# imuncle/TSCM_Calib

Measured on AMD Instinct MI355X. Metric: LM iterations/sec at 4 cams x 10k views (joint intrinsics+extrinsics, fp64), higher is better.
Workload: dtype f64

## Files before the change

include/tscm/tscm.h:

```cpp
#ifndef TSCM_H
#define TSCM_H

#include <stddef.h>

#ifdef __cplusplus
extern "C" {
#endif

#define TSCM_ABI_VERSION 6

enum {
    TSCM_OK = 0,
    TSCM_E_INVALID = -1,
    TSCM_E_NO_DEVICE = -2,
    TSCM_E_HIP = -3,
    TSCM_E_RCCL = -4,
    TSCM_E_UNSUPPORTED = -5,
    TSCM_E_NOMEM = -6,
    TSCM_E_PEER = -7
};

enum { TSCM_CONVERGENCE = 0, TSCM_NO_CONVERGENCE = 1, TSCM_FAILURE = 2 };

#define TSCM_MAX_ITERATIONS 255

typedef struct tscm_problem {
    int n_cameras;
    int n_boards;
    int n_points;
    int n_views;
    const double *board_xy;
    const int *view_camera;
    const int *view_board;
    const int *view_offset;
    const int *view_count;
    const double *obs_u;
    const double *obs_v;
    double *cam_rt;
    double *intr;
    double *board_rt;
    const unsigned char *cam_pose_constant;
    int mono;
    const unsigned char *board_pose_constant;
} tscm_problem;

typedef struct tscm_options {
    size_t struct_size;
    int max_num_iterations;
    double function_tolerance;
    double gradient_tolerance;
    double parameter_tolerance;
    double initial_trust_region_radius;
    double max_trust_region_radius;
    double min_trust_region_radius;
    double min_relative_decrease;
    double min_lm_diagonal;
    double max_lm_diagonal;
    int max_num_consecutive_invalid_steps;
    int jacobi_scaling;
    int check_every;
    int jacobian_fp32;
    int exec_flags;
} tscm_options;

enum {
    TSCM_EXEC_SEPARATE_T_REDUCE = 1,
    TSCM_EXEC_KEEP_SINGLE_RANK_COMM = 2,
    TSCM_EXEC_GRAM_16X16 = 4,
    TSCM_EXEC_SEPARATE_BACKSUB = 8,
    TSCM_EXEC_SEPARATE_CONTROL = 16,
    TSCM_EXEC_DENSE_REDUCED_ORDER = 32,
    TSCM_EXEC_GRAPH_REDUCED_ORDER = 64,
    TSCM_EXEC_SEPARATE_STATS = 128,
    TSCM_EXEC_ALL = 255
};

typedef struct tscm_iteration {
    int iteration;
    int step_is_valid;
    int step_is_successful;
    double cost;
    double cost_change;
    double gradient_max_norm;
    double gradient_norm;
    double step_norm;
    double relative_decrease;
    double trust_region_radius;
} tscm_iteration;

typedef struct tscm_summary {
    int termination_type;
    int num_iterations;
    int num_successful_steps;
    int num_unsuccessful_steps;
    double initial_cost;
    double final_cost;
    int n_residual_blocks;
    int lm_iterations;
    tscm_iteration iterations[TSCM_MAX_ITERATIONS + 1];
    char message[128];
    double seconds_solve;
    double seconds_total;
    double rmse;
} tscm_summary;

typedef struct tscm_solver tscm_solver;
typedef struct tscm_comm tscm_comm;

int tscm_abi_version(void);
const char *tscm_last_error(void);
int tscm_device_count(void);
int tscm_device_synchronize(int device);
int tscm_device_peak_fp64(int device, double *mfma_tflops, double *valu_tflops);
int tscm_device_peak_fp64_ex(int device, double peaks[3]);
int tscm_device_peak_fp32_mfma(int device, double *tflops);

void tscm_default_options(tscm_options *opt, int mono);

int tscm_solver_create(const tscm_problem *problem, int device, tscm_solver **out);
int tscm_solver_set_comm(tscm_solver *s, tscm_comm *comm);
int tscm_solver_debug_withhold_handoff(tscm_solver *s, int on);
int tscm_solver_reruns(const tscm_solver *s);
int tscm_solver_solve(tscm_solver *s, const tscm_options *opt, tscm_summary *summary);
int tscm_solver_upload_params(tscm_solver *s, const double *cam_rt, const double *intr, const double *board_rt);
int tscm_solver_solve_resident(tscm_solver *s, const tscm_options *opt, tscm_summary *summary, int reset);
int tscm_solver_download_params(tscm_solver *s, double *cam_rt, double *intr, double *board_rt);
void tscm_solver_destroy(tscm_solver *s);
int tscm_solver_kernel_time(tscm_solver *s, int enable, int *launches, double *total_ms);
int tscm_solver_exchange_time(tscm_solver *s, int *n_T, double *ms_T, int *n_H, double *ms_H);

int tscm_solve_multi(const tscm_problem *problem, const tscm_options *opt, tscm_summary *summary);
int tscm_solve_mono(const tscm_problem *problem, const tscm_options *opt, tscm_summary *summary);

int tscm_eval_functor(const tscm_problem *problem, int device, double *residuals,
                      double *J_cam, double *J_board, double *J_intr, double *cost);

int tscm_eval_normal_equations(const tscm_problem *problem, int device, double *board_gram,
                               double *board_grad, double *view_cross, double *cam_gram,
                               double *cam_grad, double *cost);

int tscm_eval_normal_equations_ex(const tscm_problem *problem, int device, const tscm_options *opt,
                                  double *board_gram, double *board_grad, double *view_cross,
                                  double *cam_gram, double *cam_grad, double *cost);

int tscm_eval_step_ex(const tscm_problem *problem, int device, const tscm_options *opt,
                      double *cam_rt, double *intr, double *board_rt, int *valid,
                      tscm_summary *summary);

enum { TSCM_LOSS_NONE = 0, TSCM_LOSS_HUBER = 1, TSCM_LOSS_SOFT_L1 = 2, TSCM_LOSS_CAUCHY = 3 };
int tscm_solver_set_loss(tscm_solver *s, int kind, double scale);
int tscm_solve_robust(const tscm_problem *problem, const tscm_options *opt, int kind, double scale, tscm_summary *summary);
int tscm_eval_normal_equations_robust(const tscm_problem *problem, int device, const tscm_options *opt, int kind, double scale,
                                      double *board_gram, double *board_grad, double *view_cross,
                                      double *cam_gram, double *cam_grad, double *cost);
int tscm_eval_step_robust(const tscm_problem *problem, int device, const tscm_options *opt, int kind, double scale,
                          double *cam_rt, double *intr, double *board_rt, int *valid, tscm_summary *summary);

enum {
    TSCM_FIX_FX = 1, TSCM_FIX_FY = 2, TSCM_FIX_CX = 4, TSCM_FIX_CY = 8, TSCM_FIX_XI = 16, TSCM_FIX_LAMBDA = 32,
    TSCM_FIX_ALPHA = 64, TSCM_FIX_B = 128, TSCM_FIX_C = 256,
    TSCM_FIX_INTRINSICS = 127, TSCM_FIX_ALL = 511,
    TSCM_MODEL_DS = TSCM_FIX_LAMBDA, TSCM_MODEL_UCM = TSCM_FIX_XI | TSCM_FIX_LAMBDA
};
int tscm_solver_set_fixed_intrinsics(tscm_solver *s, const unsigned short *fixed);
int tscm_solve_fixed(const tscm_problem *problem, const tscm_options *opt, const unsigned short *fixed, int kind, double scale,
                     tscm_summary *summary);
int tscm_eval_step_fixed(const tscm_problem *problem, int device, const tscm_options *opt, const unsigned short *fixed, int kind,
                         double scale, double *cam_rt, double *intr, double *board_rt, int *valid, tscm_summary *summary);

int tscm_solve_mono_batch(const tscm_problem *problems, int n_problems, int device, const tscm_options *opt,
                          const unsigned short *fixed , int loss_kind, double loss_scale,
                          tscm_summary *summaries );

int tscm_project_points(const double *intr9, const double *points, int n, int device, double *pixels);
int tscm_unproject_pixels(const double *intr9, const double *pixels, int n, int device, double *rays);
int tscm_reprojection_error(const tscm_problem *problem, int device, double *per_camera_mean,
                            double *global_mean, double *rmse);

#define TSCM_UNIQUE_ID_BYTES 128
int tscm_solver_create_sharded(const tscm_problem *problem, int device, int rank, int world, tscm_solver **out);
int tscm_comm_unique_id(unsigned char id[TSCM_UNIQUE_ID_BYTES]);
int tscm_comm_create(const unsigned char id[TSCM_UNIQUE_ID_BYTES], int rank, int world, int device, tscm_comm **out);
int tscm_comm_create_local(int world, int device, tscm_comm **out );
#define TSCM_IPC_HANDLE_BYTES 80
int tscm_comm_ipc_open(int rank, int world, int device, size_t max_doubles, tscm_comm **out, unsigned char handle[TSCM_IPC_HANDLE_BYTES]);
int tscm_comm_ipc_connect(tscm_comm *c, const unsigned char *handles );
void tscm_comm_destroy(tscm_comm *c);
int tscm_comm_info(const tscm_comm *c, int *rank, int *world, int *backend_ranks);
int tscm_solver_solve_group(tscm_solver **solvers, int n, const tscm_options *opt, tscm_summary *summaries, int reset);
int tscm_solver_gather_boards(tscm_solver *s, double *board_rt);
int tscm_shard_frames(const tscm_problem *problem, int world, int *owner);


typedef struct tscm_rig_input {
    int n_cameras, n_boards, n_points;
    const double *worlds;
    const double *intr;
    const unsigned char *has;
    const double *Rt;
    const double *pix_u, *pix_v;
} tscm_rig_input;

typedef struct tscm_rig_result {
    double *cam_R, *cam_t, *cam_rt;
    double *board_R, *board_t, *board_rt;
    unsigned char *board_initial;
    int *cam_choice;
    double *cam_min_error;
    double seconds_hypotheses;
    double seconds_total;
    long long n_projections;
} tscm_rig_result;

int tscm_rig_init(const tscm_rig_input *in, int device, tscm_rig_result *out);
int tscm_rig_stage_errors(const tscm_rig_input *in, int i, const double *Rp, const double *tp, int ksplit, int device,
                          double *Rs_out, double *ts_out, double *err_out, int *info_out);


int tscm_yaml_format(int n_cameras, const double *intr, const double *cam_R, const double *cam_t,
                     char *buf, size_t buf_size, size_t *needed);
int tscm_yaml_write(const char *path, int n_cameras, const double *intr, const double *cam_R,
                    const double *cam_t);
int tscm_yaml_parse(const char *text, int max_cameras, int *n_cameras, double *intr, double *Twc);
int tscm_yaml_read(const char *path, int max_cameras, int *n_cameras, double *intr, double *Twc);


typedef struct tscm_map_desc {
    double intr[9];
    double R[9];
    double fx, fy, cx, cy;
    double offset_x, offset_y;
    int width, height;
    int out_stride;
    int check_w2;
    long long out_offset;
    double w2;
} tscm_map_desc;

int tscm_build_maps(const tscm_map_desc *maps, int n_maps, int device, int exact, float *mapx,
                    float *mapy, size_t n_elems, double *seconds_kernel);

enum { TSCM_PROJ_PERSPECTIVE = 0, TSCM_PROJ_LONGLAT = 1, TSCM_PROJ_CYLINDRICAL = 2,
       TSCM_PROJ_STEREOGRAPHIC = 3, TSCM_PROJ_EQUIRECT = 4 };

int tscm_build_maps_ex(const tscm_map_desc *maps, const int *projection ,
                       int n_maps, int device, int exact, float *mapx, float *mapy, size_t n_elems,
                       double *seconds_kernel);

int tscm_build_sweep_maps(const tscm_map_desc *maps , const int *projection , int n_cameras,
                          const double *centers , const double *inv_distance , int D,
                          int device_index, int exact, float *mapx, float *mapy ,
                          size_t n_elems, double *seconds_kernel);

int tscm_rectify_points(const tscm_map_desc *map, int projection, const double *pixels ,
                        int n, int device, double *out , unsigned char *valid );


int tscm_estimate_focal(const double *pix_u, const double *pix_v, const int *count, int n_views,
                        int board_w, int board_h, double cx, double cy, int device, double *focal,
                        int *n_used);
int tscm_poses_from_r1r2t(const double *Rt, const unsigned char *has, int n, double *rt);
int tscm_estimate_extrinsic(const double *intr9, const double *pix_u, const double *pix_v, const int *count,
                            int n_views, const double *worlds, int n_points, int board_w, int device,
                            double *Rt, int *n_estimated);
#define TSCM_EXTRINSIC_NO_BOARD 1
#define TSCM_EXTRINSIC_DEGENERATE_BOARD 2
#define TSCM_EXTRINSIC_DLT_FAILED 3
#define TSCM_EXTRINSIC_ZERO_COLUMN 4
#define TSCM_EXTRINSIC_CONVERGED 5
#define TSCM_EXTRINSIC_ITERATION_CAP 6
#define TSCM_EXTRINSIC_GN_CHOLESKY 7
int tscm_estimate_focal_rows(const double *pix_u, const double *pix_v, const int *count, int n_views,
                             int board_w, int board_h, double cx, double cy, int device, double *gamma);
int tscm_estimate_extrinsic_stages(const double *intr9, const double *pix_u, const double *pix_v,
                                   const int *count, int n_views, const double *worlds, int n_points,
                                   int board_w, int device, double *Rt, int *n_estimated, double *T,
                                   double *H, double *pose0, double *pose, int *steps, int *exit_code);


typedef struct tscm_corner_set {
    int n_cameras, n_boards, board_cols, board_rows;
    double pitch;
    int image_width, image_height;
    unsigned char *has;
    double *pix_u, *pix_v;
} tscm_corner_set;

int tscm_corners_write(const char *path, const tscm_corner_set *set);
int tscm_corners_read(const char *path, tscm_corner_set *set);
void tscm_corners_free(tscm_corner_set *set);

int tscm_remap(const unsigned char *src, int width, int height, int stride, int channels, const float *mapx, const float *mapy, int map_width,
               int map_height, int map_stride, int to_gray, int device, unsigned char *dst, int dst_stride);

typedef struct tscm_corner_candidates {
    int n;
    int n_maxima;
    double *x, *y;
    double *v1, *v2;
    double *score;
    double *sub;
    double seconds;
} tscm_corner_candidates;

int tscm_detect_corners(const unsigned char *gray, int width, int height, int stride, int sigma, double min_score, int device,
                        tscm_corner_candidates *out);
int tscm_detect_corners_batch(const unsigned char *const *images, int n_images, int width, int height, int stride, int sigma, double min_score,
                              int device, tscm_corner_candidates *out);
void tscm_corner_candidates_free(tscm_corner_candidates *c);
// ... 222 lines not shown
```

tscm_calib_amd/api.py:

```python
from __future__ import annotations

import ctypes as C

import numpy as np

from . import lib as _l
from .problem import Problem


class Solver:

    def __init__(self, problem: Problem, device: int = 0, rank: int = 0, world: int = 1):
        self.problem = problem.normalised() if not _is_normalised(problem) else problem
        self.problem.validate()
        self._cp = _l.c_problem(self.problem)
        self._h = C.c_void_p()
        self.rank, self.world = rank, world
        _l.check(_l.lib().tscm_solver_create_sharded(C.byref(self._cp), device, rank, world, C.byref(self._h)))
        self._comm = None

    def close(self):
        if getattr(self, "_h", None) is not None and self._h.value:
            _l.lib().tscm_solver_destroy(self._h)
            self._h = C.c_void_p()
# ... 114 lines not shown
        _l.check(_l.lib().tscm_comm_unique_id(buf))
        return bytes(buf)

    def close(self):
        if getattr(self, "_h", None) is not None and self._h.value:
            _l.lib().tscm_comm_destroy(self._h)
            self._h = C.c_void_p()

    __del__ = close


class Group:

    def __init__(self, problem: Problem, world: int, device: int = 0, *, loss=None, fixed=None):
        self.problem = problem.normalised() if not _is_normalised(problem) else problem
        self.world = world
        self.comms = Comm.local_group(world, device)
        self.solvers = [Solver(self.problem, device, r, world) for r in range(world)]
        for s, c in zip(self.solvers, self.comms):
            s.set_comm(c)
        if loss is not None:
            k, a = _l.loss_args(loss)
            for s in self.solvers:
                _l.check(_l.lib().tscm_solver_set_loss(s._h, k, a))
        if fixed is not None:
            for s in self.solvers:
                s.set_fixed_intrinsics(fixed)

    def solve(self, **options) -> "list[dict]":
        for s in self.solvers:
            s.upload_params()
        out = self.solve_resident(reset=True, **options)
        p = self.problem
        cam, intr, _ = self.solvers[0].download_params()
        if not p.mono:
            p.cam_rt[:] = cam
        p.intr[:] = intr
        for s in self.solvers:
            _l.check(_l.lib().tscm_solver_download_params(s._h, None, None, _l.dptr(p.board_rt)))
        return out

    def solve_resident(self, reset: bool = True, **options) -> "list[dict]":
        o = _l.default_options(self.problem.mono, **options)
        hs = (C.c_void_p * self.world)(*[s._h for s in self.solvers])
        sums = (_l.CSummary * self.world)()
        _l.check(_l.lib().tscm_solver_solve_group(hs, self.world, C.byref(o), sums, 1 if reset else 0))
        return [_l.summary_dict(sums[r]) for r in range(self.world)]

    def close(self):
        for s in self.solvers:
            s.close()
        for c in self.comms:
            c.close()
        self.solvers, self.comms = [], []

    def __enter__(self):
        return self

    def __exit__(self, *a):
        self.close()


def _is_normalised(p: Problem) -> bool:
    ok = lambda a, dt: isinstance(a, np.ndarray) and a.dtype == dt and a.flags["C_CONTIGUOUS"]
    return (all(ok(getattr(p, n), np.float64) for n in ("board_xy", "obs_u", "obs_v", "cam_rt", "intr", "board_rt"))
            and all(ok(getattr(p, n), np.int32) for n in ("view_camera", "view_board", "view_offset", "view_count"))
            and ok(p.cam_pose_constant, np.uint8)
            and (p.board_pose_constant is None or ok(p.board_pose_constant, np.uint8)))


def calibrate(problem: Problem, device: int = 0, *, loss=None, fixed=None, **options) -> dict:
    if problem.mono:
        raise ValueError("calibrate() is the multi-camera solve; use refinement() for a mono problem")
    assert _is_normalised(problem), "use Problem.normalised()"
    o = _l.default_options(False, **options)
    s = _l.CSummary()
    cp = _l.c_problem(problem)
    _select(device)
    _solve_one_shot(cp, o, s, loss, fixed, problem.n_cameras, _l.lib().tscm_solve_multi)
    return _l.summary_dict(s)


def refinement(problem: Problem, device: int = 0, *, loss=None, fixed=None, **options):
    if not problem.mono:
        raise ValueError("refinement() is the mono solve")
    assert _is_normalised(problem), "use Problem.normalised()"
    o = _l.default_options(True, **options)
    s = _l.CSummary()
    cp = _l.c_problem(problem)
    _select(device)
    _solve_one_shot(cp, o, s, loss, fixed, problem.n_cameras, _l.lib().tscm_solve_mono)
    d = _l.summary_dict(s)
    return d["termination_type"] == 0, d


def refinement_batch(problems, device: int = 0, *, loss=None, fixed=None, **options):
    problems = list(problems)
    if not problems:
        raise ValueError("refinement_batch() needs at least one problem")
    for p in problems:
        if not p.mono:
            raise ValueError("refinement_batch() takes mono problems only")
        assert _is_normalised(p), "use Problem.normalised()"
    n = len(problems)
    o = _l.default_options(True, **options)
    cps = (_l.CProblem * n)(*[_l.c_problem(p) for p in problems])
    sums = (_l.CSummary * n)()
    if fixed is None:
        w = None
    else:
        if len(fixed) != n:
            raise ValueError("fixed: one mask per problem")
        w = np.array([_l.fixed_masks(f, 1)[0] for f in fixed], dtype=np.uint16)
    k, a = _l.loss_args(loss)
    _l.check(_l.lib().tscm_solve_mono_batch(cps, n, device, C.byref(o), _l.ushort_ptr(w) if w is not None else None, k, a, sums))
    out = []
    for i in range(n):
        d = _l.summary_dict(sums[i])
        out.append((d["termination_type"] == 0, d))
    return out


def _solve_one_shot(cp, o, s, loss, fixed, n_cameras, plain):
    if fixed is not None:
        w = _l.fixed_masks(fixed, n_cameras)
        k, a = _l.loss_args(loss)
        _l.check(_l.lib().tscm_solve_fixed(C.byref(cp), C.byref(o), _l.ushort_ptr(w), k, a, C.byref(s)))
    elif loss is None:
        _l.check(plain(C.byref(cp), C.byref(o), C.byref(s)))
    else:
        k, a = _l.loss_args(loss)
        _l.check(_l.lib().tscm_solve_robust(C.byref(cp), C.byref(o), k, a, C.byref(s)))


def _select(device: int):
    if device != 0:
        raise ValueError("one-shot calibrate()/refinement() use the current device; use Solver(problem, device)")


def evaluate_functor(problem: Problem, device: int = 0, jacobians: bool = True):
    assert _is_normalised(problem)
    N = problem.n_corners
    res = np.zeros((N, 2))
    cost = C.c_double(0.0)
    cp = _l.c_problem(problem)
    if jacobians:
        Jc, Jb, Ji = np.zeros((N, 2, 6)), np.zeros((N, 2, 6)), np.zeros((N, 2, 9))
        _l.check(_l.lib().tscm_eval_functor(C.byref(cp), device, _l.dptr(res), _l.dptr(Jc), _l.dptr(Jb), _l.dptr(Ji), C.byref(cost)))
        return cost.value, res, Jc, Jb, Ji
    _l.check(_l.lib().tscm_eval_functor(C.byref(cp), device, _l.dptr(res), None, None, None, C.byref(cost)))
    return cost.value, res


def normal_equations(problem: Problem, device: int = 0, *, jacobian_fp32: int = 0, exec_flags: int = 0, loss=None) -> dict:
    assert _is_normalised(problem)
    Cn, B, V = problem.n_cameras, problem.n_boards, problem.n_views
    out = dict(board_gram=np.zeros((B, 6, 6)), board_grad=np.zeros((B, 6)), view_cross=np.zeros((V, 6, 15)),
               cam_gram=np.zeros((Cn, 15, 15)), cam_grad=np.zeros((Cn, 15)))
    cost = C.c_double(0.0)
    cp = _l.c_problem(problem)
    o = _l.default_options(problem.mono, jacobian_fp32=jacobian_fp32, exec_flags=exec_flags)
    outs = (_l.dptr(out["board_gram"]), _l.dptr(out["board_grad"]), _l.dptr(out["view_cross"]),
            _l.dptr(out["cam_gram"]), _l.dptr(out["cam_grad"]), C.byref(cost))
    if loss is None:
        _l.check(_l.lib().tscm_eval_normal_equations_ex(C.byref(cp), device, C.byref(o), *outs))
    else:
        k, a = _l.loss_args(loss)
        _l.check(_l.lib().tscm_eval_normal_equations_robust(C.byref(cp), device, C.byref(o), k, a, *outs))
    out["cost"] = cost.value
    return out


def step(problem: Problem, device: int = 0, *, loss=None, fixed=None, **options) -> dict:
    assert _is_normalised(problem)
    cam, intr, board = np.zeros_like(problem.cam_rt), np.zeros_like(problem.intr), np.zeros_like(problem.board_rt)
    valid = C.c_int(0)
    s = _l.CSummary()
    cp = _l.c_problem(problem)
    o = _l.default_options(problem.mono, **options)
    outs = (_l.dptr(cam), _l.dptr(intr), _l.dptr(board), C.byref(valid), C.byref(s))
    if fixed is not None:
        w = _l.fixed_masks(fixed, problem.n_cameras)
        k, a = _l.loss_args(loss)
        _l.check(_l.lib().tscm_eval_step_fixed(C.byref(cp), device, C.byref(o), _l.ushort_ptr(w), k, a, *outs))
    elif loss is None:
        _l.check(_l.lib().tscm_eval_step_ex(C.byref(cp), device, C.byref(o), *outs))
    else:
        k, a = _l.loss_args(loss)
        _l.check(_l.lib().tscm_eval_step_robust(C.byref(cp), device, C.byref(o), k, a, *outs))
    return dict(cam_rt=cam, intr=intr, board_rt=board, valid=bool(valid.value), summary=_l.summary_dict(s))


def project(intr, points, device: int = 0) -> np.ndarray:
    intr = np.ascontiguousarray(intr, dtype=np.float64).reshape(9)
    pts = np.ascontiguousarray(points, dtype=np.float64).reshape(-1, 3)
    out = np.zeros((pts.shape[0], 2))
    _l.check(_l.lib().tscm_project_points(_l.dptr(intr), _l.dptr(pts), pts.shape[0], device, _l.dptr(out)))
    return out


def unproject(intr, pixels, device: int = 0) -> np.ndarray:
    intr = np.ascontiguousarray(intr, dtype=np.float64).reshape(9)
    px = np.ascontiguousarray(pixels, dtype=np.float64).reshape(-1, 2)
    out = np.zeros((px.shape[0], 3))
    _l.check(_l.lib().tscm_unproject_pixels(_l.dptr(intr), _l.dptr(px), px.shape[0], device, _l.dptr(out)))
    return out


def reprojection_error(problem: Problem, device: int = 0):
    assert _is_normalised(problem)
    per = np.zeros(problem.n_cameras)
    g, r = C.c_double(0.0), C.c_double(0.0)
    cp = _l.c_problem(problem)
    _l.check(_l.lib().tscm_reprojection_error(C.byref(cp), device, _l.dptr(per), C.byref(g), C.byref(r)))
    return per, g.value, r.value


def shard_owner(problem: Problem, world: int) -> np.ndarray:
    assert _is_normalised(problem)
    owner = np.zeros(problem.n_boards, dtype=np.int32)
    cp = _l.c_problem(problem)
    _l.check(_l.lib().tscm_shard_frames(C.byref(cp), world, owner.ctypes.data_as(C.POINTER(C.c_int))))
    return owner
```

tscm_calib_amd/csrc/tscm_dev.h:

```cpp
#pragma once

static_assert(kColFree == kFA && kColGrad == kFR, "tscm_columns.h plans the columns of tscm_math.h's camera tile");
constexpr int kWcolTc = 3;
constexpr int kFac = 56;
constexpr int kFacM = 0;
constexpr int kFacC = 15;
constexpr int kFacL = 21;
constexpr int kFacI = 36;
constexpr int kFacZ = 42;
constexpr int kFacD = 48;
constexpr int kTcols = 15;
constexpr int kTcWb = 0, kTcWc = 4, kTcF = 8, kTcOne = 9, kTcXi = 10, kTcLam = 12, kTcAl = 13, kTcR = 14;
__host__ __device__ constexpr int tc_tc(int j) { return 3 + 4 * j; }
constexpr int kVConst = 27;
constexpr int kCConst = 48;
constexpr int kCStride = 72;
constexpr int kCst = 80;
constexpr int kScal = 8;
constexpr int kStStride = 16;

constexpr int kVStride = 48;
constexpr int kVFloatOff = 32;

__device__ __forceinline__ void wave_lds_fence()
{
    __builtin_amdgcn_fence(__ATOMIC_RELEASE, "wavefront");
    __builtin_amdgcn_wave_barrier();
    __builtin_amdgcn_fence(__ATOMIC_ACQUIRE, "wavefront");
}

typedef int v2i __attribute__((ext_vector_type(2)));
__device__ __forceinline__ __amdgpu_buffer_rsrc_t make_rsrc(const void *p, size_t bytes)
{
    return __builtin_amdgcn_make_buffer_rsrc(const_cast<void *>(p), 0, (int)(bytes > 0xffffffffull ? 0xffffffffu : (unsigned)bytes), 0x00020000);
}
__device__ __forceinline__ double buf_load_f64(__amdgpu_buffer_rsrc_t r, unsigned voff, unsigned soff)
{
    return __builtin_bit_cast(double, __builtin_amdgcn_raw_buffer_load_b64(r, (int)voff, (int)soff, 0));
}
__device__ __forceinline__ void buf_store_f64(__amdgpu_buffer_rsrc_t r, unsigned voff, unsigned soff, double v)
{
    __builtin_amdgcn_raw_buffer_store_b64(__builtin_bit_cast(v2i, v), r, (int)voff, (int)soff, 0);
}

typedef double d4 __attribute__((ext_vector_type(4)));
typedef double d2 __attribute__((ext_vector_type(2)));
typedef int v4i __attribute__((ext_vector_type(4)));
__device__ __forceinline__ d2 buf_load_2f64(__amdgpu_buffer_rsrc_t r, unsigned voff, unsigned soff)
{
    return __builtin_bit_cast(d2, __builtin_amdgcn_raw_buffer_load_b128(r, (int)voff, (int)soff, 0));
}
__device__ __forceinline__ void buf_store_2f64(__amdgpu_buffer_rsrc_t r, unsigned voff, double a, double b)
{
    const d2 v = { a, b };
    __builtin_amdgcn_raw_buffer_store_b128(__builtin_bit_cast(v4i, v), r, (int)voff, 0, 0);
}

__device__ __forceinline__ void set_prio(int p)
{
    switch (p & 3) {
    case 0: __builtin_amdgcn_s_setprio(0); break;
    case 1: __builtin_amdgcn_s_setprio(1); break;
    case 2: __builtin_amdgcn_s_setprio(2); break;
    default: __builtin_amdgcn_s_setprio(3); break;
    }
}

__device__ __forceinline__ const double *rec_w(const double *rec, int slot) { return rec + (size_t)kRecW * slot; }
__device__ __forceinline__ const double *rec_e(const double *rec, int V, int slot) { return rec + (size_t)kRecW * V + (size_t)kRecE * slot; }
__device__ __forceinline__ const double *rec_g(const double *rec, int V, int slot) { return rec + (size_t)(kRecW + kRecE) * V + (size_t)kRecG * slot; }

struct Ctrl : CtrlHead {
    IterLog log[kMaxLog];
};

struct DevProblem {
    int C, B, n_points, V, N, n_pad;
    int n_chunks, n_pchunks, n_bids;
    int rp, half;
    int lds_wave;
    const double *board_xy;
    const int *view_cam, *view_board, *view_obs, *view_count;
    const double *obs_u, *obs_v;
    const int *chunk_vb, *chunk_ve, *chunk_cam, *cam_chunk_ptr;
    const int4 *chunk_desc;
    const int *bv_ptr;
    const int *view_slot, *slot_cam;
    const int *slot_view, *slot_board;
    const int *slow_boards;
    int n_slow;
    const int *pair_i, *pair_j;
    const int *pc_begin, *pc_end, *pc_tile;
    const int *bid_part_ptr;
    const int *pair_board;
    const int *bc_tile;
    const int4 *bc_desc;
    int n_bchunks, n_tiles;
    const unsigned char *col_ctl;
    const unsigned char *board_const;
    const unsigned char *col_active;
    const int *act_map;
    int n_act;
    int cam_pre[9];
    unsigned short cam_free[8];
    unsigned long long pair_mask;
    const int4 *solve_map;
    int cam_wg[9];
    int rank, world;
    const short *bid_lut;
    int bid_part_small[kSmallBids + 1];
    int g4_per;
};

struct DevState {
    double *cam_rt[2], *intr[2], *board_rt[2];
    double *board_pc, *cam_pc;
    double *vconst;
    double *cconst[2];
    double *rec[2];
    double *campart, *campart2;
    double *H[2], *H_stage;
    double *s_b, *s_c;
    double *fac;
    double *pairpart, *T;
    int *t_count;
    int *fac_fail;
    int *y_flag;
    double *yhat;
    double *Abig;
    double *bs_part, *st_part;
    int n_bs_blocks, n_st_blocks;
    Ctrl *ctrl;
    CtrlHead *ctrl_snap;
    int *stats_count, *stats_flag;
    struct CtlPub *ctl_pub;
};
struct CtlPub { int epoch, cur, done, pad; double radius; };

template <int CTRL>
__device__ __forceinline__ double dpp_f64(double v)
{
    const int lo = __builtin_amdgcn_update_dpp(0, __double2loint(v), CTRL, 0xF, 0xF, true);
    const int hi = __builtin_amdgcn_update_dpp(0, __double2hiint(v), CTRL, 0xF, 0xF, true);
    return __hiloint2double(hi, lo);
}
__device__ __forceinline__ double row16_allsum(double v)
{
    v += dpp_f64<0xB1>(v); v += dpp_f64<0x4E>(v); v += dpp_f64<0x141>(v); v += dpp_f64<0x140>(v);
    return v;
}
__device__ __forceinline__ double row16_allmax(double v)
{
    v = fmax(v, dpp_f64<0xB1>(v)); v = fmax(v, dpp_f64<0x4E>(v)); v = fmax(v, dpp_f64<0x141>(v)); v = fmax(v, dpp_f64<0x140>(v));
    return v;
}

#if defined(__HIP_DEVICE_COMPILE__) && !defined(__gfx950__) && !defined(__gfx942__)
#error "the in-launch hand-offs (handoff_store / handoff_load) rely on gfx942 / gfx950 sc1 write-through semantics: re-derive them for this target"
#endif
constexpr long long kHandoffTimeoutTicks = 50 * 1000 * 1000;
__device__ __forceinline__ void handoff_store(double *p, double v) { __hip_atomic_store(p, v, __ATOMIC_RELAXED, __HIP_MEMORY_SCOPE_AGENT); }
__device__ __forceinline__ double handoff_load(const double *p) { return __hip_atomic_load(p, __ATOMIC_RELAXED, __HIP_MEMORY_SCOPE_AGENT); }
```

tscm_calib_amd/csrc/tscm_eval_f32.h:

```cpp
#pragma once

template <int KS> struct F32Tile {
    static constexpr int KB = KS + (KS & 1);
    static constexpr int P2 = 4 * KB + 2;
    static constexpr int kDoubles = 16 * P2 > 512 ? 16 * P2 : 512;
    static_assert(4 * KB <= P2 && (2 * P2) % 8 == 4 && (KB * 8) % 16 == 0, "block starts are 16-byte aligned, columns 4 * odd dwords apart");
};

typedef float f2 __attribute__((ext_vector_type(2)));
typedef float f4 __attribute__((ext_vector_type(4)));

__host__ __device__ inline int eval_f32_lds_doubles(int n_points, int ks)
{
    const int kb = ks + (ks & 1), tile = 16 * (4 * kb + 2);
    return 4 * (tile > 512 ? tile : 512) + 2 * n_points;
}

template <int KS, bool MULTI, bool ROBUST = false>
__global__ __launch_bounds__(256, 4) void k_eval_gram_f32(DevProblem P, DevState S, int cand, LossArg L)
{
    static_assert(KS >= 1 && KS <= kG4MaxKS, "a pass holds at most 56 rows");
    const int ctrl_done = S.ctrl->done, ctrl_cur = S.ctrl->cur;
    extern __shared__ __attribute__((aligned(16))) double lds_all[];
    const int wave = __builtin_amdgcn_readfirstlane(threadIdx.x >> 6);
    constexpr int kP2 = F32Tile<KS>::P2, KB = F32Tile<KS>::KB, kTile32 = F32Tile<KS>::kDoubles;
    constexpr int lds_wave = kTile32;
    double *lds = lds_all + (size_t)wave * lds_wave;
    f2 *T2 = reinterpret_cast<f2 *>(lds);
    double *bxy = lds_all + 4 * kTile32;
    const int lane = threadIdx.x & 63;
    const int chunk = blockIdx.x * 4 + wave;
    const v4i cd = *(const v4i __attribute__((address_space(4))) *)(const void *)(P.chunk_desc + chunk);
    const int cam = cd[0], vb = cd[1], ve = cd[2];
    const int n2 = 2 * P.n_points;
    const double bx0 = P.board_xy[min(lane, n2 - 1)], bx1 = P.board_xy[min(lane + 64, n2 - 1)];
    typedef const float __attribute__((address_space(4))) *fptr4;
    double *const cc_buf[2] = { S.cconst[0], S.cconst[1] };
    double *const rec_buf[2] = { S.rec[0], S.rec[1] };
    const int col = lane & 15, kq = lane >> 4;
    d4 camU = { 0.0, 0.0, 0.0, 0.0 }, camV = { 0.0, 0.0, 0.0, 0.0 };
    double rr = 0.0;
    for (int i = lane; i < kTile32; i += 64) lds[i] = 0.0;
    int prev_nv = 0;
    double pf_u = 0.0, pf_v = 0.0;
    int warm = 0;
    constexpr int K = KS;
    const int per = MULTI ? P.g4_per : 4 * KS;
    f2 *fw = T2 + (KB == KS ? lane : KB * (lane / K) + lane % K);
    typedef const f4 __attribute__((address_space(3))) *lds_f4;
    const lds_f4 pB = (lds_f4)(T2 + col * kP2 + KB * kq);
    const lds_f4 pA = (lds_f4)(T2 + ((col >> 2) + 4 * (col & 3)) * kP2 + KB * kq);
    if (ctrl_done) return;
    const int tgt = cand ? (ctrl_cur ^ 1) : ctrl_cur;
    const __amdgpu_buffer_rsrc_t r_rec = make_rsrc(tgt ? rec_buf[1] : rec_buf[0], sizeof(double) * (size_t)kRec * P.V);
    const cptr4 cc = (cptr4)((tgt ? cc_buf[1] : cc_buf[0]) + kCStride * cam);
    const fptr4 cf = (fptr4)((tgt ? cc_buf[1] : cc_buf[0]) + kCStride * cam + kCConst);
    const RecLane rl = rec_lane(lane, (unsigned)P.V);
    const __amdgpu_buffer_rsrc_t r_vc = make_rsrc(S.vconst, sizeof(double) * (size_t)kVStride * P.V);
    const __amdgpu_buffer_rsrc_t r_u = make_rsrc(P.obs_u, sizeof(double) * (size_t)P.N), r_v = make_rsrc(P.obs_v, sizeof(double) * (size_t)P.N);
    int off_next = cd[3];
    int m_cnt0 = 0, m_slot0 = 0;
    if (vb + lane < min(ve, vb + 64)) { m_cnt0 = P.view_count[vb + lane]; m_slot0 = P.view_slot[vb + lane]; }
    if (vb < ve) { pf_u = buf_load_f64(r_u, 8u * lane, 8u * (unsigned)off_next); pf_v = buf_load_f64(r_v, 8u * lane, 8u * (unsigned)off_next); }
    {
        typedef const int __attribute__((address_space(4))) *cptr4i;
        const cptr4i v0 = (cptr4i)(S.vconst + (size_t)kVStride * min(vb, P.V - 1)), c0 = (cptr4i)cc;
        const int k0 = v0[0], k1 = v0[16], k2 = v0[32], k3 = v0[48], k4 = v0[64], k5 = v0[80], k6 = c0[16], k7 = c0[48], k8 = c0[80], k9 = c0[112], k10 = c0[128];
        asm volatile("" :: "s"(k0), "s"(k1), "s"(k2), "s"(k3), "s"(k4), "s"(k5), "s"(k6), "s"(k7), "s"(k8), "s"(k9), "s"(k10));
    }
    if (lane < n2) bxy[lane] = bx0;
    if (lane + 64 < n2) bxy[lane + 64] = bx1;
    for (int i = lane + 128; i < n2; i += 64) bxy[i] = P.board_xy[i];
    for (int vbase = vb; vbase < ve; vbase += 64) {
    const int vend = min(ve, vbase + 64);
    int m_cnt = 0, m_slot = 0;
    if (vbase == vb) { m_cnt = m_cnt0; m_slot = m_slot0; }
    else {
        if (vbase + lane < vend) { m_cnt = P.view_count[vbase + lane]; m_slot = P.view_slot[vbase + lane]; }
        pf_u = buf_load_f64(r_u, 8u * lane, 8u * (unsigned)off_next); pf_v = buf_load_f64(r_v, 8u * lane, 8u * (unsigned)off_next);
    }
    asm volatile("" : "+v"(m_cnt), "+v"(m_slot));
    for (int view = vbase; view < vend; ++view) {
        const int cnt = __builtin_amdgcn_readlane(m_cnt, view - vbase);
        const int off = off_next;
        off_next = off + cnt;
        wave_lds_fence();
        set_prio(3 - min(3, 8 * (view - vb) / max(1, ve - vb) % 4));
        const cptr4 cst = (cptr4)(S.vconst + (size_t)kVStride * view);
        const fptr4 cs = (fptr4)(S.vconst + (size_t)kVStride * view + kVFloatOff);
        d4 accU = { 0.0, 0.0, 0.0, 0.0 }, accV = { 0.0, 0.0, 0.0, 0.0 };
        for (int c0 = 0; c0 < cnt; c0 += per) {
            const int j = c0 + lane;
            const bool valid = lane < (MULTI ? min(per, cnt - c0) : cnt);
            float wf = 1.f;
            auto PUT = [&](int c, float u, float v) {
                if constexpr (ROBUST) { u *= wf; v *= wf; }
                fw[c * kP2] = f2{ u, v };
            };
            if (valid) {
                const double x = bxy[2 * j], y = bxy[2 * j + 1];
                const double ou = pf_u, ov = pf_v;
                const double X = fma(x, cst[0], fma(y, cst[3], cst[6]));
                const double Y = fma(x, cst[1], fma(y, cst[4], cst[7]));
                const double Z = fma(x, cst[2], fma(y, cst[5], cst[8]));
                const double rho2 = X * X + Y * Y;
                const double s1 = rho2 + Z * Z;
                const double id1 = fast_rsqrt(s1), d1 = s1 * id1;
                const double z1 = Z + cc[43] * d1;
                const double s2 = rho2 + z1 * z1;
                const double id2 = fast_rsqrt(s2), d2 = s2 * id2;
                const double z2 = z1 + cc[44] * d2;
                const double s3 = rho2 + z2 * z2;
                const double id3 = fast_rsqrt(s3), d3 = s3 * id3;
                const double ik = fast_rcp(z2 + cc[45] * d3);
                const double mx = X * ik, my = Y * ik;
                const double ru = ou - (cc[39] * mx + cc[41]);
                const double rv = ov - (cc[40] * my + cc[42]);
                double w = 1.0;
                if constexpr (ROBUST) {
                    double rho;
                    robust_rho(L, ru * ru + rv * rv, rho, w);
                    rr += rho;
                    wf = (float)w;
                } else {
                    rr += ru * ru + rv * rv;
                }
                const float xf = (float)x, yf = (float)y;
                const float Xf = (float)X, Yf = (float)Y, Zf = (float)Z, z1f = (float)z1, z2f = (float)z2;
                const float i1 = (float)id1, i2 = (float)id2, i3 = (float)id3, ikf = (float)ik;
                const float e1 = (float)d1, e2 = (float)d2, e3 = (float)d3;
                const float mxf = (float)mx, myf = (float)my;
                float Q0 = (float)(X - cc[9]), Q1 = (float)(Y - cc[10]), Q2 = (float)(Z - cc[11]);
                if (cc[24] != 0.0) {
                    const float w0 = cf[21], w1 = cf[22], w2 = cf[23];
                    const float s0 = w1 * Q2 - w2 * Q1, s1 = w2 * Q0 - w0 * Q2, s2 = w0 * Q1 - w1 * Q0;
                    Q0 -= s0; Q1 -= s1; Q2 -= s2;
                }
                const float xi = cf[43], lam = cf[44], beta = cf[45];
                const float c1 = 1.f + xi * Zf * i1;
                const float c2 = 1.f + lam * z1f * i2;
                const float c3 = 1.f + beta * z2f * i3;
                const float q = beta * i3 + c3 * (lam * i2 + c2 * xi * i1);
                const float kz = c1 * c2 * c3;
                const f2 fk = { cf[39] * ikf, cf[40] * ikf };
                const f2 HM = { fk.x * mxf, fk.y * myf };
                const f2 N0 = HM * (Xf * q) - (f2){ fk.x, 0.f };
                const f2 N1 = HM * (Yf * q) - (f2){ 0.f, fk.y };
                const f2 N2 = HM * kz;
                PUT(tc_tc(0), N0.x, N0.y);
                PUT(tc_tc(1), N1.x, N1.y);
                PUT(tc_tc(2), N2.x, N2.y);
#pragma unroll
                for (int kk = 0; kk < 3; ++kk) {
                    const float h0 = xf * cs[9 + 6 * kk] + yf * cs[12 + 6 * kk];
                    const float h1 = xf * cs[10 + 6 * kk] + yf * cs[13 + 6 * kk];
                    const float h2 = xf * cs[11 + 6 * kk] + yf * cs[14 + 6 * kk];
                    const f2 w = N0 * h0 + N1 * h1 + N2 * h2;
                    PUT((kTcWb + kk), w.x, w.y);
                }
                {
                    const f2 c0 = N2 * Q1 - N1 * Q2, c1 = N0 * Q2 - N2 * Q0, c2 = N1 * Q0 - N0 * Q1;
#pragma unroll
                    for (int kk = 0; kk < 3; ++kk) {
                        const f2 w = c0 * cf[12 + 3 * kk] + c1 * cf[13 + 3 * kk] + c2 * cf[14 + 3 * kk];
                        PUT((kTcWc + kk), w.x, w.y);
                    }
                }
                PUT(kTcF, -mxf, -myf);
                PUT(kTcOne, -1.f, -1.f);
                const float kxi = c3 * c2 * e1, klam = c3 * e2, kal = e3 * cf[46];
                const f2 a = HM * kxi, b = HM * klam, c = HM * kal;
                PUT(kTcXi, a.x, a.y);
                PUT(kTcLam, b.x, b.y);
                PUT(kTcAl, c.x, c.y);
                if constexpr (ROBUST) fw[kTcR * kP2] = f2{ (float)(w * ru), (float)(w * rv) };
                else PUT(kTcR, (float)ru, (float)rv);
            } else if (lane < prev_nv) {
#pragma unroll
                for (int c = 0; c < kTcols; ++c) PUT(c, 0.f, 0.f);
            }
            {
                const int vn = min(view + 1, vend - 1);
                const int cn = view + 1 < vend ? __builtin_amdgcn_readlane(m_cnt, vn - vbase) : 0;
                if (!MULTI || c0 == 0) warm = __builtin_amdgcn_raw_buffer_load_b32(r_vc, lane < 6 ? 64 * lane : (int)0xffffe000u, (int)(8u * (unsigned)kVStride * (unsigned)vn), 0);
                const bool more = MULTI && c0 + per < cnt;
                const int ncnt = MULTI ? (more ? min(per, cnt - c0 - per) : min(per, cn)) : cn;
// ... 57 lines not shown
```

tscm_calib_amd/csrc/tscm_eval_gram4.h:

```cpp
#pragma once

constexpr int kG4Stride = 68;
__host__ __device__ constexpr int g4_tile_doubles(int ks) { return ks * kG4Stride > 512 ? ks * kG4Stride : 512; }
__host__ __device__ inline int eval_gram4_lds_doubles(int n_points, int ks) { return g4_tile_doubles(ks) + 2 * n_points; }

constexpr int kG4Wb = 0, kG4R = 3, kG4Tc = 4, kG4Al = 7, kG4Wc = 8, kG4F = 11, kG4One = 12, kG4Xi = 13, kG4Lam = 14;
__device__ __forceinline__ constexpr int g4_old_col(int c)
{
    return c < 3 ? kTcWb + c : c == 3 ? kTcR : c < 7 ? tc_tc(c - 4) : c == 7 ? kTcAl : c < 11 ? kTcWc + (c - 8) : c == 11 ? kTcF
         : c == 12 ? kTcOne : c == 13 ? kTcXi : c == 14 ? kTcLam : 15;
}
__device__ __forceinline__ constexpr int g4_wcol(int c)
{
    return c < 3 ? -1 : c == 3 ? kFR : c < 7 ? kWcolTc + (c - 4) : c == 7 ? 12 : c < 11 ? c - 8 : c == 11 ? 6 : c == 12 ? 8 : c == 13 ? 10 : c == 14 ? 11 : -1;
}
__device__ __forceinline__ constexpr int g4_cgroup(int b, int q) { return q == 0 ? b : q == 1 ? ((b + 1) & 3) : (b == 0 ? 2 : b == 1 ? 3 : 1); }
__device__ __forceinline__ int g4_elem(int c, int k) { return 4 * c + (k ^ ((c >> 3) << 1)); }

template <int KS, int D, bool ACC, int T = 0>
__device__ __forceinline__ void gram4_steps(unsigned aN, unsigned aR, unsigned aB, double (&n)[KS], double (&r)[KS], double (&b)[KS], double (&acc)[3])
{
    if constexpr (T < KS) {
        if constexpr (T + D < KS) {
            n[T + D] = ds_read_f64<8 * kG4Stride * (T + D)>(aN);
            r[T + D] = ds_read_f64<8 * kG4Stride * (T + D)>(aR);
            b[T + D] = ds_read_f64<8 * kG4Stride * (T + D)>(aB);
        }
        constexpr int newer = 3 * (KS - 1 - T < D ? KS - 1 - T : D);
        lgkm_wait<newer + 2>(n[T]);
        if constexpr (T == 0 && !ACC) acc[0] = __builtin_amdgcn_mfma_f64_4x4x4f64(n[T], n[T], 0.0, 0, 0, 0);
        else acc[0] = __builtin_amdgcn_mfma_f64_4x4x4f64(n[T], n[T], acc[0], 0, 0, 0);
        lgkm_wait<newer + 1>(r[T]);
        if constexpr (T == 0 && !ACC) acc[1] = __builtin_amdgcn_mfma_f64_4x4x4f64(n[T], r[T], 0.0, 0, 0, 0);
        else acc[1] = __builtin_amdgcn_mfma_f64_4x4x4f64(n[T], r[T], acc[1], 0, 0, 0);
        lgkm_wait<newer>(b[T]);
        if constexpr (T == 0 && !ACC) acc[2] = __builtin_amdgcn_mfma_f64_4x4x4f64(n[T], b[T], 0.0, 0, 0, 0);
        else acc[2] = __builtin_amdgcn_mfma_f64_4x4x4f64(n[T], b[T], acc[2], 0, 0, 0);
        gram4_steps<KS, D, ACC, T + 1>(aN, aR, aB, n, r, b, acc);
    }
}
template <int KS, int D, int T = 0>
__device__ __forceinline__ void gram4_prime(unsigned aN, unsigned aR, unsigned aB, double (&n)[KS], double (&r)[KS], double (&b)[KS])
{
    if constexpr (T < D && T < KS) {
        n[T] = ds_read_f64<8 * kG4Stride * T>(aN);
        r[T] = ds_read_f64<8 * kG4Stride * T>(aR);
        b[T] = ds_read_f64<8 * kG4Stride * T>(aB);
        gram4_prime<KS, D, T + 1>(aN, aR, aB, n, r, b);
    }
}
template <int KS, bool ACC>
__device__ __forceinline__ void gram4_full(unsigned aN, unsigned aR, unsigned aB, double (&acc)[3])
{
    constexpr int D = KS < 2 ? KS : 2;
    double n[KS], r[KS], b[KS];
    gram4_prime<KS, D>(aN, aR, aB, n, r, b);
    gram4_steps<KS, D, ACC>(aN, aR, aB, n, r, b, acc);
}

__device__ __forceinline__ double quad_tb(double x, double c0, double c1, double c2)
{
    const double x0 = dpp_f64<0x00>(x), x1 = dpp_f64<0x55>(x), x2 = dpp_f64<0xAA>(x);
    return fma(c2, x2, fma(c0, x0, c1 * x1));
}

template <int ROW, int BANK>
__device__ __forceinline__ double lane_pick(double keep, double take)
{
    const int lo = __builtin_amdgcn_update_dpp(__double2loint(keep), __double2loint(take), 0xE4, ROW, BANK, false);
    const int hi = __builtin_amdgcn_update_dpp(__double2hiint(keep), __double2hiint(take), 0xE4, ROW, BANK, false);
    return __hiloint2double(hi, lo);
}

template <int KS, bool MULTI, bool ROBUST = false>
__global__ __launch_bounds__(256, 4) void k_eval_gram4(DevProblem P, DevState S, int cand, LossArg L)
{
    static_assert(KS >= 1 && KS <= kG4MaxKS, "a pass holds at most 56 rows");
    constexpr int kTile = g4_tile_doubles(KS);
    KTL(0);
    const int ctrl_done = S.ctrl->done, ctrl_cur = S.ctrl->cur;
#ifdef TSCM_WAVE_TIMELINE
    const long long tl_t0 = wall_clock64();
    const int tl_iter = S.ctrl->iteration;
    long long tl_ph[5] = { 0, 0, 0, 0, 0 };
    long long tl_w[4] = { 0, 0, 0, 0 };
    int tl_nv = 0;
#define TL_STAMP(var) const long long var = (long long)__builtin_readcyclecounter()
#define TL_ADD(k, a, b) tl_ph[k] += (b) - (a)
#else
#define TL_STAMP(var)
#define TL_ADD(k, a, b)
#endif
    extern __shared__ __attribute__((aligned(16))) double lds_all[];
    const int wave = __builtin_amdgcn_readfirstlane(threadIdx.x >> 6);
    const int lds_wave = eval_gram4_lds_doubles(P.n_points, KS);
    double *lds = lds_all + (size_t)wave * lds_wave;
    double *Fl = lds;
    double *bxy = lds + kTile;
    const int lane = threadIdx.x & 63;
    const int chunk = blockIdx.x * 4 + wave;
    const v4i cd = *(const v4i __attribute__((address_space(4))) *)(const void *)(P.chunk_desc + chunk);
    const int cam = cd[0], vb = cd[1], ve = cd[2];
    const d2 my_xy = *reinterpret_cast<const d2 *>(P.board_xy + 2 * min(lane, P.n_points - 1));
    double *const cc_buf[2] = { S.cconst[0], S.cconst[1] };
    double *const rec_buf[2] = { S.rec[0], S.rec[1] };
    double camU[3] = { 0.0, 0.0, 0.0 }, camV[3] = { 0.0, 0.0, 0.0 };
    for (int i = lane; i < KS * kG4Stride; i += 64) Fl[i] = 0.0;
    int prev_nv = 0;
    double pf_u = 0.0, pf_v = 0.0;
    int warm = 0;
    double rho_sum = 0.0;
    if (ctrl_done) return;
    const int tgt = cand ? (ctrl_cur ^ 1) : ctrl_cur;
    const __amdgpu_buffer_rsrc_t r_rec = make_rsrc(tgt ? rec_buf[1] : rec_buf[0], sizeof(double) * (size_t)kRec * P.V);
    const cptr4 ccs = (cptr4)((tgt ? cc_buf[1] : cc_buf[0]) + kCStride * cam);
    auto CC = [&](int k) { return ccs[k]; };
    const __amdgpu_buffer_rsrc_t r_vc = make_rsrc(S.vconst, sizeof(double) * (size_t)kVStride * P.V);
    const __amdgpu_buffer_rsrc_t r_u = make_rsrc(P.obs_u, sizeof(double) * (size_t)P.N), r_v = make_rsrc(P.obs_v, sizeof(double) * (size_t)P.N);
    int off_next = cd[3];
    int m_cnt0 = 0, m_slot0 = 0;
    if (vb + lane < min(ve, vb + 64)) { m_cnt0 = P.view_count[vb + lane]; m_slot0 = P.view_slot[vb + lane]; }
    if (vb < ve) { pf_u = buf_load_f64(r_u, 8u * ((unsigned)off_next + lane), 0); pf_v = buf_load_f64(r_v, 8u * ((unsigned)off_next + lane), 0); }
    typedef const int __attribute__((address_space(4))) *cptr4i;
    const cptr4i vc0 = (cptr4i)(S.vconst + (size_t)kVStride * min(vb, P.V - 1)), cc0 = (cptr4i)ccs;
    const int kw0 = vc0[0], kw1 = vc0[16], kw2 = vc0[32], kw3 = vc0[48], kw4 = cc0[16], kw5 = cc0[32], kw6 = cc0[48], kw7 = cc0[64], kw8 = cc0[80];
    double *fu_lo = Fl + (lane >> 2) * kG4Stride + (lane & 3), *fu_hi = Fl + (lane >> 2) * kG4Stride + ((lane & 3) ^ 2);
    const int li = lane >> 4, c16 = lane & 15, lb = c16 >> 2, lj = c16 & 3;
    const unsigned lds0 = lds_addr(Fl);
    const unsigned aN = lds0 + 8u * (unsigned)g4_elem(c16, li);
    const unsigned aR = lds0 + 8u * (unsigned)g4_elem((c16 + 4) & 15, li);
    const unsigned aB = lds0 + 8u * (unsigned)g4_elem(4 * g4_cgroup(lb, 2) + lj, li);
    const double rc0 = lj == 0 ? ccs[0] : lj == 1 ? ccs[1] : ccs[2];
    const double rc1 = lj == 0 ? ccs[3] : lj == 1 ? ccs[4] : ccs[5];
    const double rc2 = lj == 0 ? ccs[6] : lj == 1 ? ccs[7] : ccs[8];
    constexpr unsigned BAD = 0xffffe000u;
    unsigned o1e = BAD, o1w = BAD, o2 = BAD, o3e = BAD, o4 = BAD, o5 = BAD, o6 = BAD, o7a = BAD, o7b = BAD;
    {
        const int b = lb, j = lj, i = li;
        auto W = [](int wcol, int row) { return 8u * (unsigned)(6 * wcol + row); };
        const int f1 = g4_wcol(4 + i), f1j = g4_wcol(4 + j), f2 = g4_wcol(8 + i), f2j = g4_wcol(8 + j), f3 = g4_wcol(12 + i);
        if (b == 0 && j < 3 && i < 3) { o1e = 8u * (unsigned)(6 * j + i); o3e = 8u * (unsigned)(6 * i + 3 + j); }
        if (b == 0 && j == 3 && i < 3) { o1w = W(kFR, i); o7a = 8u * (unsigned)i; }
        if (b == 1 && j < 3) o1w = W(f1, 3 + j);
        if (b == 0 && i < 3) o2 = W(f1j, i);
        if (b == 0 && i == 3 && j < 3) { o2 = W(kFR, 3 + j); o7b = 8u * (unsigned)(3 + j); }
        if (b == 3 && j < 3 && i < 3) o2 = W(f3, j);
        if (b == 0 && i < 3) o4 = W(f2j, i);
        if (b == 2 && j < 3) o4 = W(f2, 3 + j);
        if (b == 3 && j < 3 && i < 3) o4 = W(f3, 3 + j);
        if (b == 3 && i == 0 && j < 3) { o5 = W(9, j); o6 = W(9, 3 + j); }
        if (b == 0 && j == 3 && i < 3) o6 = W(7, i);
        if (b == 2 && i == 3 && j < 3) o6 = W(7, 3 + j);
    }
    if (lane < P.n_points) *reinterpret_cast<d2 *>(bxy + 2 * lane) = my_xy;
    if constexpr (MULTI) {
        for (int j = lane + 64; j < P.n_points; j += 64) *reinterpret_cast<d2 *>(bxy + 2 * j) = *reinterpret_cast<const d2 *>(P.board_xy + 2 * j);
    }
    const int per = MULTI ? P.g4_per : 4 * KS;
    asm volatile("" :: "s"(kw0), "s"(kw1), "s"(kw2), "s"(kw3), "s"(kw4), "s"(kw5), "s"(kw6), "s"(kw7), "s"(kw8));
#ifdef TSCM_WAVE_TIMELINE
    tl_w[0] = wall_clock64();
    const bool tl_on = lane == 0 && tl_iter == 5 && cand && chunk < kTimelineWaves;
#endif
    const int prio_n = max(1, ve - vb);
    int prio_q = 0, prio_rem = 0;
    for (int vbase = vb; vbase < ve; vbase += 64) {
    const int vend = min(ve, vbase + 64);
    int m_cnt = 0, m_slot = 0;
    if (vbase == vb) { m_cnt = m_cnt0; m_slot = m_slot0; }
    else {
        if (vbase + lane < vend) { m_cnt = P.view_count[vbase + lane]; m_slot = P.view_slot[vbase + lane]; }
        pf_u = buf_load_f64(r_u, 8u * ((unsigned)off_next + lane), 0); pf_v = buf_load_f64(r_v, 8u * ((unsigned)off_next + lane), 0);
    }
    asm volatile("" : "+v"(m_cnt), "+v"(m_slot));
    for (int view = vbase; view < vend; ++view) {
        const int cnt = __builtin_amdgcn_readlane(m_cnt, view - vbase);
        const int off = off_next;
        off_next += cnt;
        wave_lds_fence();
        const int left = ve - 1 - view;
        const bool tail_steps = left <= 2 && ve - vb <= 16;
        set_prio(tail_steps ? left + 1 : 3 - (prio_q & 3));
        for (prio_rem += 8; prio_rem >= prio_n; prio_rem -= prio_n) { ++prio_q; asm volatile("" : "+s"(prio_q)); }
#ifdef TSCM_WAVE_TIMELINE
        if (tl_on && tl_nv < kTlViews) g_tlv[(size_t)(4 + kTlViews) * chunk + 4 + tl_nv] = wall_clock64();
        ++tl_nv;
#endif
        const cptr4 vcs = (cptr4)(S.vconst + (size_t)kVStride * view);
        auto VC = [&](int k) { return vcs[k]; };
        double accU[3] = { 0.0, 0.0, 0.0 }, accV[3] = { 0.0, 0.0, 0.0 };
        int pbv = 0;
        do {
        const int pb = MULTI ? pbv : 0;
        TL_STAMP(ts0);
        if constexpr (MULTI) { if (pb) wave_lds_fence(); }
        const int nv = MULTI ? min(per, cnt - pb) : cnt;
        const bool valid = lane < nv;
        double fv[16];
        auto PUT = [&](int c, double u, double v) { (c < 8 ? fu_lo : fu_hi)[4 * c] = u; fv[c] = v; };
        if (valid) {
            const double x = bxy[2 * (pb + lane)], y = bxy[2 * (pb + lane) + 1];
            constexpr int tcol[15] = { kG4Wb, kG4Wb + 1, kG4Wb + 2, kG4Tc, kG4Tc + 1, kG4Tc + 2, kG4Wc, kG4Wc + 1, kG4Wc + 2,
                                       kG4F, kG4One, kG4Xi, kG4Lam, kG4Al, kG4R };
            if constexpr (ROBUST) {
                double ru, rv, rho, w;
                corner_residual(x, y, pf_u, pf_v, VC, CC, ru, rv);
                robust_rho(L, ru * ru + rv * rv, rho, w);
                rho_sum += rho;
                corner_geometry(x, y, pf_u, pf_v, VC, CC, [&](int gc, double u, double v) { PUT(tcol[gc], w * u, w * v); });
            } else {
                corner_geometry(x, y, pf_u, pf_v, VC, CC, [&](int gc, double u, double v) { PUT(tcol[gc], u, v); });
            }
        }
        if (nv < prev_nv) {
            if (!valid && lane < prev_nv) {
#pragma unroll
                for (int c = 0; c < kTcols; ++c) (c < 8 ? fu_lo : fu_hi)[4 * c] = 0.0;
            }
        }
        {
            const int vn = min(view + 1, vend - 1);
            if (!MULTI || pb == 0) warm = __builtin_amdgcn_raw_buffer_load_b32(r_vc, lane < 4 ? 64 * lane : (int)0xffffe000u, (int)(8u * (unsigned)kVStride * (unsigned)vn), 0);
            const bool more = MULTI && pb + per < cnt;
            const unsigned noff = more ? (unsigned)(off + pb + per) : (unsigned)off_next;
            pf_u = buf_load_f64(r_u, 8u * (noff + lane), 0);
            pf_v = buf_load_f64(r_v, 8u * (noff + lane), 0);
        }
        prev_nv = MULTI ? min(per, max(cnt - pb, 0)) : cnt;
        wave_lds_fence();
        if (tail_steps && left == 0) set_prio(0);
        TL_STAMP(ts1);
#ifdef TSCM_WAVE_TIMELINE
        if (tl_nv == 1) tl_w[1] = wall_clock64();
#endif
        gram4_full<KS, MULTI>(aN, aR, aB, accU);
        wave_lds_fence();
        TL_STAMP(ts2);
        if (valid) {
#pragma unroll
            for (int c = 0; c < kTcols; ++c) (c < 8 ? fu_lo : fu_hi)[4 * c] = fv[c];
        }
        wave_lds_fence();
        TL_STAMP(ts3);
        gram4_full<KS, MULTI>(aN, aR, aB, accV);
        TL_STAMP(ts4);
        TL_ADD(0, ts0, ts1); TL_ADD(1, ts1, ts2); TL_ADD(2, ts2, ts3); TL_ADD(3, ts3, ts4);
        pbv += per;
        } while (MULTI && pbv < cnt);
        TL_STAMP(ts4e);
        asm volatile("" :: "v"(warm));
#pragma unroll
        for (int q = 0; q < 3; ++q) { camU[q] += accU[q]; camV[q] += accV[q]; }
        {
            const unsigned slot = (unsigned)__builtin_amdgcn_readlane(m_slot, view - vbase);
            const unsigned offW = 8u * (unsigned)kRecW * slot, offE = 8u * ((unsigned)kRecW * (unsigned)P.V + (unsigned)kRecE * slot);
            const double T0 = accU[0] + accV[0], T1 = accU[1] + accV[1], T2 = accU[2] + accV[2];
            const double X = lane_pick<0xF, 0x1>(lane_pick<0xF, 0x2>(T2, T0), T1);
            const double tbX = quad_tb(X, rc0, rc1, rc2), tbU2 = quad_tb(accU[2], rc0, rc1, rc2);
            const unsigned offG = 8u * ((unsigned)(kRecW + kRecE) * (unsigned)P.V + (unsigned)kRecG * slot);
            buf_store_f64(r_rec, o1e, offE, T0);
            buf_store_f64(r_rec, o7a, offG, T0);
            buf_store_f64(r_rec, o1w, offW, lane_pick<0xF, 0x2>(T0, tbX));
            buf_store_f64(r_rec, o5, offW, T1 - accU[1]);
            buf_store_f64(r_rec, o2, offW, lane_pick<0x1, 0x8>(lane_pick<0x8, 0xF>(T1, tbX), accU[1]));
            buf_store_f64(r_rec, o3e, offE, tbX);
            buf_store_f64(r_rec, o7b, offG, tbX);
            const double a4 = lane_pick<0xF, 0xE>(T2, tbX), u4 = lane_pick<0xF, 0x1>(tbU2, accU[2]);
            buf_store_f64(r_rec, o4, offW, (int)o6 >= 0 ? u4 : a4);
            buf_store_f64(r_rec, o6, offW, a4 - u4);
        }
#ifdef TSCM_WAVE_TIMELINE
        { TL_STAMP(ts5); TL_ADD(4, ts4e, ts5); }
        if (view + 1 == ve) tl_w[3] = wall_clock64();
#endif
    }
    }
#ifdef TSCM_WAVE_TIMELINE
    if (lane == 0 && tl_iter == 5 && cand && chunk < kTimelineWaves) {
        g_timeline[4 * chunk] = (long long)__builtin_amdgcn_s_getreg(63492);
        g_timeline[4 * chunk + 1] = (long long)__builtin_amdgcn_s_getreg(6164);
        g_timeline[4 * chunk + 2] = tl_t0;
        g_timeline[4 * chunk + 3] = wall_clock64();
        for (int k = 0; k < 5; ++k) g_phase[5 * chunk + k] = tl_ph[k];
        for (int k = 0; k < 4; ++k) g_tlv[(size_t)(4 + kTlViews) * chunk + k] = tl_w[k];
    }
#endif
    if constexpr (ROBUST) {
#pragma unroll
        for (int o = 32; o > 0; o >>= 1) rho_sum += __shfl_xor(rho_sum, o);
        if (lane == 16 * kG4R + kG4R) { camU[0] = rho_sum; camV[0] = 0.0; }
    }
    wave_lds_fence();
#pragma unroll
    for (int q = 0; q < 3; ++q) {
        const int r = g4_old_col(4 * lb + li), c = g4_old_col(4 * g4_cgroup(lb, q) + lj);
        lds[16 * r + c] = camU[q]; lds[16 * c + r] = camU[q];
        lds[256 + 16 * r + c] = camV[q]; lds[256 + 16 * c + r] = camV[q];
    }
    __syncthreads();
    {
        const int t = threadIdx.x;
        const size_t st = lds_wave;
        double *part = S.campart + (size_t)512 * blockIdx.x;
        part[t] = (lds_all[t] + lds_all[st + t]) + (lds_all[2 * st + t] + lds_all[3 * st + t]);
        part[256 + t] = (lds_all[256 + t] + lds_all[st + 256 + t]) + (lds_all[2 * st + 256 + t] + lds_all[3 * st + 256 + t]);
    }
#ifdef TSCM_WAVE_TIMELINE
    if (lane == 0 && tl_iter == 5 && cand && chunk < kTimelineWaves) g_tlv[(size_t)(4 + kTlViews) * chunk + 2] = wall_clock64();
#endif
}
```

tscm_calib_amd/csrc/tscm_exec_plan.h:

```cpp
#ifndef TSCM_EXEC_PLAN_H
#define TSCM_EXEC_PLAN_H

#include "tscm_layout.h"

#include <algorithm>
#include <string>

#ifdef __HIPCC__
#define TSCM_PLAN_FN __host__ __device__ inline
#else
#define TSCM_PLAN_FN inline
#endif

namespace tscm {

constexpr int kCamSl = 16;
constexpr int kTSlices = 16;
constexpr int kTEntries = 64;
constexpr int kFusedEntries = 256 / kTSlices;
constexpr int kVPrepThreads = 128;
constexpr int kDense4Cams = 4;

constexpr int kCtlOneGpu = 1;
constexpr int kCtlComm = 2;
constexpr int kCtlInit = 4;
constexpr int kCtlRide = 8;
constexpr int kCtlWithhold = 16;

enum CommKind { kCommNone, kCommOneRank, kCommShared };
inline bool uses_comm(int kind, int exec_flags) { return kind == kCommShared || (kind == kCommOneRank && (exec_flags & TSCM_EXEC_KEEP_SINGLE_RANK_COMM)); }

enum class Gram { G4, F32, G16, G16Pitch58 };
enum class EvalTail {
    ReduceControl,
    StatsThenHead,
    Ride,
    Exchange,
};
enum class Solver { Empty, Dense4, Nd, Big };

struct ExecDevice {
    int schur_resident[4] = {}, schur_resident_ride[4] = {};
    int dense4_resident = 0;
    int nd_resident[2] = {}, nd_tpt[2] = { 1, 1 };
};

struct ExecPlan {
    bool comm = false;
    Gram gram = Gram::G4;
    bool robust = false;
    EvalTail tail = EvalTail::ReduceControl;
    bool ctl_in_schur = false;
    bool stats_ride = false;
    bool t_in_solve = false;
    Solver solver = Solver::Empty;
    int nd = 0, tpt = 1;
    int n_prod = 0, n_bs = 0;
    int bs_threads = 0;
    bool f32() const { return gram == Gram::F32; }
};

inline int reduction_blocks(const Layout &L, int C) { return C * kCamSl + (L.B + 255) / 256; }

inline Gram plan_gram(int exec_flags, int jacobian_fp32, int rp)
{
    if (jacobian_fp32) return Gram::F32;
    if (!(exec_flags & TSCM_EXEC_GRAM_16X16)) return Gram::G4;
    return rp == 58 ? Gram::G16Pitch58 : Gram::G16;
}

constexpr int kG4MaxKS = 14;
struct G4Plan { int passes, per, ks; };
TSCM_PLAN_FN G4Plan g4_plan(int n_points)
{
    G4Plan g;
    g.passes = (n_points + 4 * kG4MaxKS - 1) / (4 * kG4MaxKS);
    if (g.passes < 1) g.passes = 1;
    g.ks = ((n_points + g.passes - 1) / g.passes + 3) / 4;
    if (g.ks < 1) g.ks = 1;
    g.per = 4 * g.ks;
    return g;
}

inline ExecPlan plan_exec(const Layout &L, int C, int n_act, int comm_kind, int exec_flags, int jacobian_fp32, int loss_kind, int rp,
                          const ExecDevice &dev)
{
    ExecPlan p;
    p.comm = uses_comm(comm_kind, exec_flags);
    p.gram = plan_gram(exec_flags, jacobian_fp32, rp);
    p.robust = loss_kind != TSCM_LOSS_NONE;
    const int n_variants = (L.nv_chunks[1] ? 1 : 0) + (L.nv_chunks[2] ? 1 : 0) + (L.nv_chunks[3] ? 1 : 0);
    const bool small = C <= kMaxCamLds;
    p.ctl_in_schur = (p.comm || small) && L.slow_boards.empty() && L.pc_begin.empty() && n_variants == 1 &&
                     !(exec_flags & TSCM_EXEC_SEPARATE_CONTROL);
    const int nv = L.nv_chunks[1] ? 1 : L.nv_chunks[2] ? 2 : 3;
    p.stats_ride = p.ctl_in_schur && !p.comm && small && !(exec_flags & TSCM_EXEC_SEPARATE_STATS) &&
                   std::max(reduction_blocks(L, C), L.nv_chunks[nv]) + 1 <= dev.schur_resident_ride[nv];
    p.tail = p.comm || !small ? EvalTail::Exchange : !p.ctl_in_schur ? EvalTail::ReduceControl : p.stats_ride ? EvalTail::Ride : EvalTail::StatsThenHead;
    p.t_in_solve = !(exec_flags & TSCM_EXEC_SEPARATE_T_REDUCE) && small && !p.comm && L.n_bids > 0 && L.n_bids <= kSmallBids && n_act > 0;
    p.n_prod = p.t_in_solve ? L.n_bids * (256 / kFusedEntries) : 0;
    p.nd = (exec_flags & TSCM_EXEC_DENSE_REDUCED_ORDER) ? 1 : 0;
    const bool graph_order = (exec_flags & TSCM_EXEC_GRAPH_REDUCED_ORDER) || p.nd;
    p.solver = n_act == 0 ? Solver::Empty : C <= kDense4Cams && !graph_order ? Solver::Dense4 : small ? Solver::Nd : Solver::Big;
    if (p.solver != Solver::Nd) p.nd = 0;
    p.tpt = p.solver == Solver::Nd ? dev.nd_tpt[p.nd] : 1;
    if (p.solver == Solver::Dense4 || p.solver == Solver::Nd) {
        const int resident = p.solver == Solver::Dense4 ? dev.dense4_resident : dev.nd_resident[p.nd];
        if (!(exec_flags & TSCM_EXEC_SEPARATE_BACKSUB) && L.bs_threads == 256 && L.n_bs_blocks <= resident - 1 - p.n_prod) p.n_bs = L.n_bs_blocks;
    }
    p.bs_threads = !p.n_bs && L.n_bs_blocks ? L.bs_threads : 0;
    return p;
}

inline int check_exec_options(const tscm_options &o, int loss_kind, std::string &err)
{
    if (o.max_num_iterations < 0 || o.max_num_iterations > TSCM_MAX_ITERATIONS) return layout_fail(err, TSCM_E_INVALID, "max_num_iterations must be in [0, 255]");
    if (o.exec_flags & ~TSCM_EXEC_ALL) return layout_fail(err, TSCM_E_INVALID, "unknown bits in tscm_options.exec_flags (an options struct of an older ABI?)");
    if (loss_kind != TSCM_LOSS_NONE && (o.exec_flags & TSCM_EXEC_GRAM_16X16)) return layout_fail(err, TSCM_E_UNSUPPORTED, "TSCM_EXEC_GRAM_16X16 has no robust-loss kernel");
    return 0;
}

}

#endif
```

tscm_calib_amd/csrc/tscm_geometry.h:

```cpp
#pragma once

__host__ __device__ __forceinline__ constexpr int f_tile(int f)
{
    return f < 3 ? kTcWc + f : f < 6 ? tc_tc(f - 3) : f < 8 ? kTcF : f < 10 ? kTcOne : f == 10 ? kTcXi : f == 11 ? kTcLam : f == 12 ? kTcAl : kTcR;
}
__device__ __forceinline__ int f_mask(int f) { return (f >= 6 && f < 10) ? (1 << ((f - 6) & 1)) : 3; }

typedef const double __attribute__((address_space(4))) *cptr4;

struct RecLane { unsigned off, stride, goff, gstride; };
__device__ __forceinline__ RecLane rec_lane(int lane, unsigned V)
{
    const int col = lane & 15, kq = lane >> 4;
    RecLane r;
    r.goff = col == kTcR ? 8u * ((unsigned)(kRecW + kRecE) * V + (unsigned)kq) : 0xffffe000u; r.gstride = col == kTcR ? 8u * kRecG : 0u;
    if (col < 3) { r.off = 8u * ((unsigned)kRecW * V + 6u * (unsigned)col + (unsigned)kq); r.stride = 8u * kRecE; }
    else if (col == 15) { r.off = 0xffffe000u; r.stride = 0u; }
    else {
        const int f = (col & 3) == 3 ? kWcolTc + (col >> 2) : col < 8 ? col - kTcWc : col == kTcF ? 6 : col == kTcOne ? 8 : col == kTcXi ? 10 : col - 1;
        r.off = 8u * (6u * (unsigned)f + (unsigned)kq); r.stride = 8u * kRecW;
    }
    return r;
}

template <typename PW, typename PR>
__host__ __device__ __forceinline__ double tb_tb(PW W, PR Rc, int l, int lp)
{
    double t = Rc[3 + lp] * W[6 * (kWcolTc + 1) + 3 + l];
    t = fma(Rc[lp], W[6 * kWcolTc + 3 + l], t);
    return fma(Rc[6 + lp], W[6 * (kWcolTc + 2) + 3 + l], t);
}

__device__ __forceinline__ void store_view_record(__amdgpu_buffer_rsrc_t r_rec, int lane, const d4 &accU, const d4 &accV, cptr4 cc, unsigned slot, RecLane rl)
{
    int le = lane;
    asm volatile("" : "+v"(le));
    const int col = le & 15;
    const bool k3 = le >= 48, split = col == kTcF || col == kTcOne;
    constexpr unsigned BAD = 0xffffe000u;
    const unsigned off = rl.off + __umul24(slot, rl.stride);
    const double t0 = accU[0] + accV[0], t1 = accU[1] + accV[1], t2 = accU[2] + accV[2];
    double tbT[3], tbU[3];
#pragma unroll
    for (int l = 0; l < 3; ++l) {
        tbT[l] = fma(cc[6 + l], t2, fma(cc[l], t0, cc[3 + l] * t1));
        tbU[l] = fma(cc[6 + l], accU[2], fma(cc[l], accU[0], cc[3 + l] * accU[1]));
    }
    const double selT = k3 ? tbT[0] : t0, selU = k3 ? tbU[0] : accU[0];
    buf_store_f64(r_rec, off, 0u, split ? selU : selT);
    buf_store_2f64(r_rec, (k3 ? off : BAD) + 8u, split ? tbU[1] : tbT[1], split ? tbU[2] : tbT[2]);
    buf_store_f64(r_rec, (split ? off : BAD) + 48u, 0u, selT - selU);
    buf_store_2f64(r_rec, (split && k3 ? off : BAD) + 56u, tbT[1] - tbU[1], tbT[2] - tbU[2]);
    const unsigned og = rl.goff + __umul24(slot, rl.gstride);
    buf_store_f64(r_rec, og, 0u, selT);
    buf_store_2f64(r_rec, (k3 ? og : BAD) + 8u, tbT[1], tbT[2]);
}

enum GCol { gcWb0 = 0, gcWb1, gcWb2, gcTc0, gcTc1, gcTc2, gcWc0, gcWc1, gcWc2, gcF, gcOne, gcXi, gcLam, gcAl, gcR };

template <typename FV, typename FC, typename FP>
__device__ __forceinline__ void corner_geometry(double x, double y, double ou, double ov, FV VC, FC CC, FP PUT)
{
    const double X = fma(x, VC(0), fma(y, VC(3), VC(6)));
    const double Y = fma(x, VC(1), fma(y, VC(4), VC(7)));
    const double Z = fma(x, VC(2), fma(y, VC(5), VC(8)));
    const double fx = CC(39), fy = CC(40), xi = CC(43), lam = CC(44), beta = CC(45);
    const double rho2 = X * X + Y * Y;
    double d1, id1, d2, id2, d3, id3;
    sqrt_and_inverse(rho2 + Z * Z, d1, id1);
    const double z1 = Z + xi * d1;
    sqrt_and_inverse(rho2 + z1 * z1, d2, id2);
    const double z2 = z1 + lam * d2;
    sqrt_and_inverse(rho2 + z2 * z2, d3, id3);
    const double k = z2 + beta * d3;
    const double ik = fast_rcp(k);
    const double mx = X * ik, my = Y * ik;
    const double c1 = 1.0 + xi * Z * id1;
    const double c2 = 1.0 + lam * z1 * id2;
    const double c3 = 1.0 + beta * z2 * id3;
    const double q = beta * id3 + c3 * (lam * id2 + c2 * xi * id1);
    const double kz = c1 * c2 * c3;
    const double fxk = fx * ik, fyk = fy * ik;
    const double n00 = -fxk * (1.0 - X * mx * q), n01 = fxk * mx * Y * q, n02 = fxk * mx * kz;
    const double n10 = fyk * my * X * q, n11 = -fyk * (1.0 - Y * my * q), n12 = fyk * my * kz;
    PUT(gcTc0, n00, n10);
    PUT(gcTc1, n01, n11);
    PUT(gcTc2, n02, n12);
#pragma unroll
    for (int kk = 0; kk < 3; ++kk) {
        const double h0 = x * VC(9 + 6 * kk) + y * VC(12 + 6 * kk);
        const double h1 = x * VC(10 + 6 * kk) + y * VC(13 + 6 * kk);
        const double h2 = x * VC(11 + 6 * kk) + y * VC(14 + 6 * kk);
        PUT(gcWb0 + kk, n00 * h0 + n01 * h1 + n02 * h2, n10 * h0 + n11 * h1 + n12 * h2);
    }
    {
        double Q0 = X - CC(9), Q1 = Y - CC(10), Q2 = Z - CC(11);
        if (CC(24) != 0.0) {
            const double w0 = CC(21), w1 = CC(22), w2 = CC(23);
            const double s0 = w1 * Q2 - w2 * Q1, s1 = w2 * Q0 - w0 * Q2, s2 = w0 * Q1 - w1 * Q0;
            Q0 -= s0; Q1 -= s1; Q2 -= s2;
        }
        const double cu0 = Q1 * n02 - Q2 * n01, cu1 = Q2 * n00 - Q0 * n02, cu2 = Q0 * n01 - Q1 * n00;
        const double cv0 = Q1 * n12 - Q2 * n11, cv1 = Q2 * n10 - Q0 * n12, cv2 = Q0 * n11 - Q1 * n10;
#pragma unroll
        for (int kk = 0; kk < 3; ++kk)
            PUT(gcWc0 + kk, CC(12 + 3 * kk) * cu0 + CC(13 + 3 * kk) * cu1 + CC(14 + 3 * kk) * cu2,
                            CC(12 + 3 * kk) * cv0 + CC(13 + 3 * kk) * cv1 + CC(14 + 3 * kk) * cv2);
    }
    PUT(gcF, -mx, -my);
    PUT(gcOne, -1.0, -1.0);
    const double hu = fxk * mx, hv = fyk * my;
    const double kxi = c3 * c2 * d1, klam = c3 * d2, kal = d3 * CC(46);
    PUT(gcXi, hu * kxi, hv * kxi);
    PUT(gcLam, hu * klam, hv * klam);
    PUT(gcAl, hu * kal, hv * kal);
    PUT(gcR, ou - (fx * mx + CC(41)), ov - (fy * my + CC(42)));
}

template <typename FV, typename FC>
__device__ __forceinline__ void corner_residual(double x, double y, double ou, double ov, FV VC, FC CC, double &ru, double &rv)
{
    const double X = fma(x, VC(0), fma(y, VC(3), VC(6)));
    const double Y = fma(x, VC(1), fma(y, VC(4), VC(7)));
    const double Z = fma(x, VC(2), fma(y, VC(5), VC(8)));
    const double xi = CC(43), lam = CC(44), beta = CC(45);
    const double rho2 = X * X + Y * Y;
    double d1, id1, d2, id2, d3, id3;
    sqrt_and_inverse(rho2 + Z * Z, d1, id1);
    const double z1 = Z + xi * d1;
    sqrt_and_inverse(rho2 + z1 * z1, d2, id2);
    const double z2 = z1 + lam * d2;
    sqrt_and_inverse(rho2 + z2 * z2, d3, id3);
    const double k = z2 + beta * d3;
    const double ik = fast_rcp(k);
    const double mx = X * ik, my = Y * ik;
    ru = ou - (CC(39) * mx + CC(41));
    rv = ov - (CC(40) * my + CC(42));
}

enum { kLossNone = 0, kLossHuber = 1, kLossSoftL1 = 2, kLossCauchy = 3 };
struct LossArg { double a, b, c; int kind, pad; };
__device__ __forceinline__ void robust_rho(const LossArg &L, double s, double &rho, double &w)
{
    constexpr double kMin = 2.2250738585072014e-308;
    double r1;
    if (L.kind == kLossHuber) {
        if (s > L.b) { const double r = sqrt(s); rho = 2.0 * L.a * r - L.b; r1 = fmax(kMin, L.a / r); }
        else { rho = s; r1 = 1.0; }
    } else if (L.kind == kLossSoftL1) {
        const double sum = 1.0 + s * L.c, tmp = sqrt(sum);
        rho = 2.0 * L.b * (tmp - 1.0); r1 = fmax(kMin, 1.0 / tmp);
    } else {
        const double sum = 1.0 + s * L.c, inv = 1.0 / sum;
        rho = L.b * log(sum); r1 = fmax(kMin, inv);
    }
    w = sqrt(r1);
}
```

tscm_calib_amd/csrc/tscm_solver.hip:

```cpp
#include "tscm/tscm.h"
#include "tscm_host.h"
#include "tscm_kernels.h"
#include "tscm_launch_seq.h"
#include "tscm_mono_batch.h"

#include <hip/hip_runtime.h>
#include <hip/hip_ext.h>
#include <rccl/rccl.h>

#include <algorithm>
#include <chrono>
#include <cstdio>
#include <cstdlib>
#include <cmath>
#include <cstring>
#include <memory>
#include <numeric>
#include <string>
#include <thread>
#include <vector>

using namespace tscm;

static thread_local std::string g_err;
static int fail(int code, const std::string &msg) { g_err = msg; return code; }
int tscm_set_error(int code, const std::string &msg) { return fail(code, msg); }

#define NCCL_TRY(expr)                                                                                 \
    do {                                                                                               \
        ncclResult_t r_ = (expr);                                                                      \
        if (r_ != ncclSuccess)                                                                         \
            return fail(TSCM_E_RCCL, std::string(#expr) + ": " + ncclGetErrorString(r_));             \
    } while (0)

static double wall() { return std::chrono::duration<double>(std::chrono::steady_clock::now().time_since_epoch()).count(); }

struct tscm_local_group {
    int world = 0, device = 0, refs = 0;
    hipStream_t stream = nullptr;
    double **d_ptrs = nullptr;
    DeviceMem mem;
    ~tscm_local_group() { if (stream) (void)hipStreamDestroy(stream); }
};
constexpr int kIpcMaxWorld = 16;
struct IpcPeers { double *base[kIpcMaxWorld]; };
struct tscm_ipc {
    int world = 0, rank = 0;
    size_t max_doubles = 0;
    DeviceMem mem;
    void *mapped[kIpcMaxWorld] = {};
    bool connected = false;
    long long count = 0;
    int *d_fault = nullptr;
    bool fine = false;
    bool dead = false;
    size_t slot_doubles() const { return max_doubles; }
    size_t flags_offset() const { return 2 * (size_t)world * max_doubles; }
    size_t total_bytes() const { return 8 * (flags_offset() + 2 * (size_t)world); }
};
struct tscm_comm {
    ncclComm_t comm = nullptr;
    tscm_local_group *group = nullptr;
    tscm_ipc *ipc = nullptr;
    int rank = 0, world = 1, device = 0;
};

typedef void (*EvalKernel)(DevProblem, DevState, int, LossArg);
template <bool ROBUST>
static EvalKernel g4_kernel_of(int ks, bool multi)
{
    static const EvalKernel single[kG4MaxKS] = {
        k_eval_gram4<1, false, ROBUST>, k_eval_gram4<2, false, ROBUST>, k_eval_gram4<3, false, ROBUST>, k_eval_gram4<4, false, ROBUST>,
        k_eval_gram4<5, false, ROBUST>, k_eval_gram4<6, false, ROBUST>, k_eval_gram4<7, false, ROBUST>, k_eval_gram4<8, false, ROBUST>,
        k_eval_gram4<9, false, ROBUST>, k_eval_gram4<10, false, ROBUST>, k_eval_gram4<11, false, ROBUST>, k_eval_gram4<12, false, ROBUST>,
        k_eval_gram4<13, false, ROBUST>, k_eval_gram4<14, false, ROBUST> };
    static const EvalKernel passes[kG4MaxKS] = {
        nullptr, nullptr, nullptr, nullptr, nullptr, nullptr, nullptr, k_eval_gram4<8, true, ROBUST>, k_eval_gram4<9, true, ROBUST>,
        k_eval_gram4<10, true, ROBUST>, k_eval_gram4<11, true, ROBUST>, k_eval_gram4<12, true, ROBUST>, k_eval_gram4<13, true, ROBUST>,
        k_eval_gram4<14, true, ROBUST> };
    return (multi ? passes : single)[ks - 1];
}
static EvalKernel g4_kernel(int ks, bool multi, bool robust) { return robust ? g4_kernel_of<true>(ks, multi) : g4_kernel_of<false>(ks, multi); }
template <bool ROBUST>
static EvalKernel f32_kernel_of(int ks, bool multi)
{
    static const EvalKernel single[kG4MaxKS] = {
        k_eval_gram_f32<1, false, ROBUST>, k_eval_gram_f32<2, false, ROBUST>, k_eval_gram_f32<3, false, ROBUST>, k_eval_gram_f32<4, false, ROBUST>,
        k_eval_gram_f32<5, false, ROBUST>, k_eval_gram_f32<6, false, ROBUST>, k_eval_gram_f32<7, false, ROBUST>, k_eval_gram_f32<8, false, ROBUST>,
        k_eval_gram_f32<9, false, ROBUST>, k_eval_gram_f32<10, false, ROBUST>, k_eval_gram_f32<11, false, ROBUST>, k_eval_gram_f32<12, false, ROBUST>,
        k_eval_gram_f32<13, false, ROBUST>, k_eval_gram_f32<14, false, ROBUST> };
    static const EvalKernel passes[kG4MaxKS] = {
        nullptr, nullptr, nullptr, nullptr, nullptr, nullptr, nullptr, k_eval_gram_f32<8, true, ROBUST>, k_eval_gram_f32<9, true, ROBUST>,
        k_eval_gram_f32<10, true, ROBUST>, k_eval_gram_f32<11, true, ROBUST>, k_eval_gram_f32<12, true, ROBUST>, k_eval_gram_f32<13, true, ROBUST>,
        k_eval_gram_f32<14, true, ROBUST> };
    return (multi ? passes : single)[ks - 1];
}
static EvalKernel f32_kernel(int ks, bool multi, bool robust) { return robust ? f32_kernel_of<true>(ks, multi) : f32_kernel_of<false>(ks, multi); }

struct tscm_solver {
    int device = 0;
    hipStream_t stream = nullptr;
    DevProblem P{};
    DevState S{};
    DeviceMem mem;
    tscm_comm *comm = nullptr;
    Layout L;
    int C = 0, B = 0, V = 0, N = 0, n_points = 0, n_pad = 0;
    int rank = 0, world = 1;
    hipStream_t own_stream = nullptr;
    bool mono = false;
    double *h_cam_rt = nullptr, *h_intr = nullptr, *h_board_rt = nullptr;
    double *d_init_cam = nullptr, *d_init_intr = nullptr, *d_init_board = nullptr;
    double *d_start_cam = nullptr, *d_start_intr = nullptr, *d_start_board = nullptr;
    bool have_init = false;
    Ctrl *h_ctrl = nullptr;
    Ctrl *d_h_ctrl = nullptr;
    size_t lds_eval = 0, lds_eval32 = 0, lds_solve = 0, lds_bs = 0;
    ExecDevice dev;
    ExecPlan xp;
    CtrlHead head;
    int withhold = 0, withhold_next = 0;
    int n_reruns = 0;
    bool no_rerun = false, no_rerun_next = false;
    tscm_comm *comm_reg = nullptr;
    NdPlan plan[2];
    const int4 *d_nd_map[2] = { nullptr, nullptr };
    const int *d_nd_tab[2] = { nullptr, nullptr }, *d_nd_bs[2] = { nullptr, nullptr };
    size_t lds_nd[2] = { 0, 0 }, lds_dense4 = 0;
    size_t lds_eval4 = 0;
    EvalKernel eval4 = nullptr, eval32 = nullptr;
    EvalKernel eval4r = nullptr, eval32r = nullptr;
    LossArg loss{};
    std::vector<unsigned short> fixed;
    int n_cu = 1;
    double *d_view_sq = nullptr;
    int timing = 0;
    unsigned ev_count[3] = { 0, 0, 0 };
    std::vector<std::pair<hipEvent_t, hipEvent_t>> ev;
    std::vector<int> ev_kind;
    size_t ev_used = 0;
    int t_launches[3] = { 0, 0, 0 };
    double t_ms[3] = { 0.0, 0.0, 0.0 };
};

struct SolverDelete { void operator()(tscm_solver *s) const { tscm_solver_destroy(s); } };
using SolverPtr = std::unique_ptr<tscm_solver, SolverDelete>;

static int create_scoped(const tscm_problem *p, int device, SolverPtr &sp)
{
    tscm_solver *s = nullptr;
    if (int rc = tscm_solver_create(p, device, &s)) return rc;
    sp.reset(s);
    return 0;
}

extern "C" int tscm_abi_version(void) { return TSCM_ABI_VERSION; }
extern "C" const char *tscm_last_error(void) { return g_err.c_str(); }

extern "C" int tscm_device_count(void)
{
    int n = 0;
    if (hipGetDeviceCount(&n) != hipSuccess) return 0;
    return n;
}

extern "C" int tscm_device_synchronize(int device)
{
    if (int rc = select_device(device, "tscm_device_synchronize")) return rc;
    HIP_TRY(hipDeviceSynchronize());
    return 0;
}

extern "C" void tscm_default_options(tscm_options *o, int mono)
{
    o->struct_size = sizeof(tscm_options);
    o->max_num_iterations = mono ? 100 : 50;
    o->function_tolerance = 1e-6;
    o->gradient_tolerance = 1e-10;
    o->parameter_tolerance = 1e-8;
    o->initial_trust_region_radius = 1e4;
    o->max_trust_region_radius = 1e16;
    o->min_trust_region_radius = 1e-32;
    o->min_relative_decrease = 1e-3;
    o->min_lm_diagonal = 1e-6;
    o->max_lm_diagonal = 1e32;
    o->max_num_consecutive_invalid_steps = 5;
    o->jacobi_scaling = 1;
    o->check_every = 4;
    o->jacobian_fp32 = 0;
    o->exec_flags = 0;
}

static int validate(const tscm_problem *p)
{
    std::string err;
    if (int rc = tscm::validate(p, err)) return fail(rc, err);
    return 0;
}

static int make_loss(int kind, double scale, LossArg &L)
{
    L = LossArg{};
    if (kind < TSCM_LOSS_NONE || kind > TSCM_LOSS_CAUCHY) return fail(TSCM_E_INVALID, "unknown loss kind");
    if (kind == TSCM_LOSS_NONE) return 0;
    if (!std::isfinite(scale) || !(scale > 0.0)) return fail(TSCM_E_INVALID, "the scale of a loss must be finite and > 0");
    L.kind = kind; L.a = scale; L.b = scale * scale; L.c = 1.0 / L.b;
    return 0;
}
static bool same_loss(const LossArg &x, const LossArg &y) { return x.kind == y.kind && (x.kind == TSCM_LOSS_NONE || x.a == y.a); }

extern "C" int tscm_solver_set_loss(tscm_solver *s, int kind, double scale)
{
    LossArg L;
    if (int rc = make_loss(kind, scale, L)) return rc;
    if (!s) return fail(TSCM_E_INVALID, "solver is NULL");
    s->loss = L;
    return 0;
}

extern "C" void tscm_solver_destroy(tscm_solver *s)
{
    if (!s) return;
    (void)hipSetDevice(s->device);
    s->stream = s->own_stream;
    if (s->stream) (void)hipStreamSynchronize(s->stream);
    for (auto &e : s->ev) { (void)hipEventDestroy(e.first); (void)hipEventDestroy(e.second); }
    if (s->h_ctrl) (void)hipHostFree(s->h_ctrl);
    if (s->stream) (void)hipStreamDestroy(s->stream);
    delete s;
}

static int apply_columns(tscm_solver *s, const ColumnPlan &c)
{
    DevProblem &P = s->P;
    HIP_TRY(hipSetDevice(s->device));
    HIP_TRY(hipStreamSynchronize(s->stream));
    HIP_TRY(hipMemcpy(const_cast<unsigned char *>(P.col_active), c.col_active.data(), c.col_active.size(), hipMemcpyHostToDevice));
    HIP_TRY(hipMemcpy(const_cast<unsigned char *>(P.col_ctl), c.col_ctl.data(), c.col_ctl.size(), hipMemcpyHostToDevice));
    HIP_TRY(hipMemcpy(const_cast<int *>(P.act_map), c.act_map.data(), sizeof(int) * c.act_map.size(), hipMemcpyHostToDevice));
    P.n_act = c.n_act;
    std::copy(std::begin(c.cam_pre), std::end(c.cam_pre), P.cam_pre);
    std::copy(std::begin(c.cam_free), std::end(c.cam_free), P.cam_free);
    static_assert(sizeof(Int4) == sizeof(int4), "the operand map is uploaded as it is");
    if (!c.solve_map.empty()) HIP_TRY(hipMemcpy(const_cast<int4 *>(P.solve_map), c.solve_map.data(), sizeof(Int4) * c.solve_map.size(), hipMemcpyHostToDevice));
    if (c.has_nd) {
        for (int v = 0; v < 2; ++v) {
            const NdPlan &pl = c.nd[v];
            s->mem.release(s->d_nd_map[v]); s->mem.release(s->d_nd_tab[v]); s->mem.release(s->d_nd_bs[v]);
            s->d_nd_map[v] = nullptr; s->d_nd_tab[v] = nullptr; s->d_nd_bs[v] = nullptr;
            HIP_TRY(s->mem.upload(&s->d_nd_map[v], reinterpret_cast<const int4 *>(pl.map.data()), pl.map.size() / 4));
            HIP_TRY(s->mem.upload(&s->d_nd_tab[v], pl.tab));
            HIP_TRY(s->mem.upload(&s->d_nd_bs[v], pl.bs_tab));
            s->lds_nd[v] = sizeof(double) * pl.lds_doubles;
            s->plan[v] = pl;
        }
        {
            const size_t lds_max = std::max(std::max(s->lds_nd[0], s->lds_nd[1]), s->lds_bs);
            if (lds_max > 64 * 1024)
                for (const void *k : { reinterpret_cast<const void *>(k_solve_nd<1, true>), reinterpret_cast<const void *>(k_solve_nd<2, true>),
                                       reinterpret_cast<const void *>(k_solve_nd<1, false>), reinterpret_cast<const void *>(k_solve_nd<2, false>) })
                    HIP_TRY(hipFuncSetAttribute(k, hipFuncAttributeMaxDynamicSharedMemorySize, (int)lds_max));
        }
        for (int v = 0; v < 2; ++v) {
            const size_t lds = std::max(s->lds_nd[v], s->lds_bs);
            int per_cu = 0;
            if (s->plan[v].tpt == 1) HIP_TRY(hipOccupancyMaxActiveBlocksPerMultiprocessor(&per_cu, reinterpret_cast<const void *>(k_solve_nd<1, true>), kNdThreads, lds));
            else HIP_TRY(hipOccupancyMaxActiveBlocksPerMultiprocessor(&per_cu, reinterpret_cast<const void *>(k_solve_nd<2, true>), kNdThreads, lds));
            s->dev.nd_resident[v] = per_cu * s->n_cu;
            s->dev.nd_tpt[v] = s->plan[v].tpt;
        }
        s->lds_solve = std::max(s->lds_nd[0], s->lds_nd[1]);
    }
    if (s->C > kMaxCamLds) s->lds_solve = solve_big_lds_bytes((c.n_act + 15) & ~15, s->n_pad);
    return 0;
}

static int check_fixed(const unsigned short *fixed, int C)
{
    if (fixed) for (int m = 0; m < C; ++m) if (fixed[m] & ~TSCM_FIX_ALL) return fail(TSCM_E_INVALID, "unknown bits in a fixed-intrinsics mask (bits 0-8 only)");
    return 0;
}

extern "C" int tscm_solver_set_fixed_intrinsics(tscm_solver *s, const unsigned short *fixed)
{
    if (!s) return fail(TSCM_E_INVALID, "solver is NULL");
    if (int rc = check_fixed(fixed, s->C)) return rc;
    std::vector<unsigned short> f(s->C, 0);
    if (fixed) f.assign(fixed, fixed + s->C);
    if (f == s->fixed) return 0;
    ColumnPlan c;
    std::string err;
    if (int rc = plan_columns(s->L, s->C, f.data(), c, err)) return fail(rc, err);
    if (int rc = apply_columns(s, c)) return rc;
    s->fixed = f;
    return 0;
}

extern "C" int tscm_solver_create_sharded(const tscm_problem *p, int device, int rank, int world, tscm_solver **out)
{
    if (!out) return fail(TSCM_E_INVALID, "out is NULL");
    *out = nullptr;
    if (int rc = validate(p)) return rc;
    if (world < 1 || rank < 0 || rank >= world) return fail(TSCM_E_INVALID, "rank / world out of range");
    if (int rc = select_device(device, "the TSCM solver")) return rc;

    SolverPtr sp(new tscm_solver);
    tscm_solver *s = sp.get();
    s->device = device;
    s->rank = rank; s->world = world;
    s->C = p->n_cameras; s->n_points = p->n_points; s->mono = p->mono != 0;
    s->n_pad = 16 * s->C;
    s->h_cam_rt = p->cam_rt; s->h_intr = p->intr; s->h_board_rt = p->board_rt;
    HIP_TRY(hipStreamCreateWithFlags(&s->stream, hipStreamNonBlocking));
    s->own_stream = s->stream;
    const int C = s->C;

    const int half_rows = 8 * ((std::min(64, p->n_points) + 7) / 8);
    const int rp = half_rows + 2;
    const size_t lds_eval_bytes = sizeof(double) * (std::max<size_t>((size_t)16 * rp, 512) + kCst + 2 * (size_t)p->n_points);
    if (4 * lds_eval_bytes > 64 * 1024) HIP_TRY(hipFuncSetAttribute(reinterpret_cast<const void *>(k_eval_gram<0>), hipFuncAttributeMaxDynamicSharedMemorySize, (int)(4 * lds_eval_bytes)));
    const G4Plan g4 = g4_plan(p->n_points);
    const EvalKernel eval4 = g4_kernel(g4.ks, g4.passes > 1, false), eval4r = g4_kernel(g4.ks, g4.passes > 1, true);
    const size_t lds_eval4 = 4 * sizeof(double) * (size_t)eval_gram4_lds_doubles(p->n_points, g4.ks);
    if (lds_eval4 > 160 * 1024) return fail(TSCM_E_UNSUPPORTED, "board with too many corners for the Gram kernel's LDS (more than about 2,000)");
    if (lds_eval4 > 64 * 1024)
        for (EvalKernel k : { eval4, eval4r }) HIP_TRY(hipFuncSetAttribute(reinterpret_cast<const void *>(k), hipFuncAttributeMaxDynamicSharedMemorySize, (int)lds_eval4));
    int wgs_per_cu = 0;
    HIP_TRY(hipOccupancyMaxActiveBlocksPerMultiprocessor(&wgs_per_cu, reinterpret_cast<const void *>(eval4), 256, lds_eval4));
    const int waves_per_cu = 4 * std::max(1, std::min(4, wgs_per_cu));
    hipDeviceProp_t prop;
    HIP_TRY(hipGetDeviceProperties(&prop, device));
    const void *schur[4][2] = { {}, { reinterpret_cast<const void *>(k_schur_gram<1>), reinterpret_cast<const void *>(k_schur_gram<1, true>) },
                                { reinterpret_cast<const void *>(k_schur_gram<2>), reinterpret_cast<const void *>(k_schur_gram<2, true>) },
                                { reinterpret_cast<const void *>(k_schur_gram<3>), reinterpret_cast<const void *>(k_schur_gram<3, true>) } };
    for (int nv = 1; nv <= 3; ++nv) {
        HIP_TRY(hipOccupancyMaxActiveBlocksPerMultiprocessor(&s->dev.schur_resident[nv], schur[nv][0], 256, 0));
        HIP_TRY(hipOccupancyMaxActiveBlocksPerMultiprocessor(&s->dev.schur_resident_ride[nv], schur[nv][1], 256, 0));
        s->dev.schur_resident[nv] *= prop.multiProcessorCount; s->dev.schur_resident_ride[nv] *= prop.multiProcessorCount;
    }
    s->n_cu = std::max(1, prop.multiProcessorCount);

    const Layout &L = s->L;
    {
        LayoutDevice dev;
        dev.n_cu = prop.multiProcessorCount; dev.waves_per_cu = waves_per_cu;
        std::string err;
        if (int rc = plan_layout(p, rank, world, dev, s->L, err)) return fail(rc, err);
    }
    s->B = L.B; s->V = L.V; s->N = L.N;
    const int B = L.B, V = L.V, N = L.N;
    s->lds_bs = sizeof(double) * (size_t)(L.bs_threads == 256 ? BsGeom<256>::kLds : BsGeom<128>::kLds);
    for (const void *k : { reinterpret_cast<const void *>(k_backsub_prep<128>), reinterpret_cast<const void *>(k_backsub_prep<256>) })
        HIP_TRY(hipFuncSetAttribute(k, hipFuncAttributeMaxDynamicSharedMemorySize, (int)s->lds_bs));

    std::vector<double> u((size_t)N), w((size_t)N);
    for (int i = 0; i < V; ++i) {
        const int v = L.dev2orig[i];
        std::memcpy(u.data() + L.view_obs[i], p->obs_u + p->view_offset[v], sizeof(double) * L.view_count[i]);
        std::memcpy(w.data() + L.view_obs[i], p->obs_v + p->view_offset[v], sizeof(double) * L.view_count[i]);
    }
    const std::vector<double> bxy(p->board_xy, p->board_xy + 2 * (size_t)p->n_points);
    auto int4s = [](const std::vector<Int4> &h) {
        std::vector<int4> d(h.size());
        for (size_t i = 0; i < h.size(); ++i) d[i] = make_int4(h[i].x, h[i].y, h[i].z, h[i].w);
        return d;
    };
    const std::vector<int4> chunk_desc = int4s(L.chunk_desc), bc_desc = int4s(L.bc_desc);
    const std::vector<short> bid_lut(L.bid_of.begin(), L.bid_of.end());
    DevProblem &P = s->P;
    DevState &S = s->S;
    P.C = C; P.B = B; P.n_points = p->n_points; P.V = V; P.N = N; P.n_pad = s->n_pad;
    P.rank = rank; P.world = world;
    P.rp = rp; P.half = half_rows; P.lds_wave = (int)(lds_eval_bytes / sizeof(double)); P.g4_per = g4.per;
    P.n_chunks = (int)L.chunk_vb.size(); P.n_pchunks = (int)L.pc_begin.size(); P.n_bids = L.n_bids;
    P.n_bchunks = (int)L.bc_desc.size(); P.n_tiles = L.n_tiles; P.n_slow = (int)L.slow_boards.size();
    std::copy(std::begin(L.cam_wg), std::end(L.cam_wg), P.cam_wg);
    std::copy(std::begin(L.bid_part_small), std::end(L.bid_part_small), P.bid_part_small);
    P.pair_mask = L.pair_mask;
    hipError_t he = hipSuccess;
    auto up = [&](auto **dst, const auto &h) { if (he == hipSuccess) he = s->mem.upload(dst, h); };
    auto al = [&](auto **dst, size_t n) { if (he == hipSuccess) he = s->mem.alloc(dst, n); };
    up(&P.board_xy, bxy);
    up(&P.view_cam, L.view_cam); up(&P.view_board, L.view_board); up(&P.view_obs, L.view_obs); up(&P.view_count, L.view_count);
    up(&P.obs_u, u); up(&P.obs_v, w);
    up(&P.chunk_vb, L.chunk_vb); up(&P.chunk_ve, L.chunk_ve); up(&P.chunk_cam, L.chunk_cam); up(&P.chunk_desc, chunk_desc);
    up(&P.cam_chunk_ptr, L.cam_chunk_ptr);
    up(&P.bv_ptr, L.bv_ptr); up(&P.view_slot, L.view_slot); up(&P.slot_cam, L.slot_cam); up(&P.slot_view, L.slot_view); up(&P.slot_board, L.slot_board);
    up(&P.slow_boards, L.slow_boards);
    up(&P.pair_i, L.pair_i); up(&P.pair_j, L.pair_j); up(&P.pc_begin, L.pc_begin); up(&P.pc_end, L.pc_end); up(&P.pc_tile, L.pc_tile);
    up(&P.bid_part_ptr, L.bid_part_ptr); up(&P.pair_board, L.pair_board); up(&P.bc_tile, L.bc_tile); up(&P.bc_desc, bc_desc);
    up(&P.bid_lut, bid_lut); up(&P.board_const, L.board_const);
    s->fixed.assign(C, 0);
    al(&P.col_active, s->n_pad); al(&P.col_ctl, (size_t)16 * kMaxCam); al(&P.act_map, s->n_pad);

    for (int k = 0; k < 2; ++k) {
        al(&S.cam_rt[k], 6 * (size_t)C); al(&S.intr[k], 9 * (size_t)C); al(&S.board_rt[k], 6 * (size_t)B);
        al(&S.rec[k], (size_t)kRec * V); al(&S.H[k], 256 * (size_t)C);
    }
    al(&s->d_init_cam, 6 * (size_t)C); al(&s->d_init_intr, 9 * (size_t)C); al(&s->d_init_board, 6 * (size_t)B);
    al(&s->d_start_cam, 6 * (size_t)C); al(&s->d_start_intr, 9 * (size_t)C); al(&s->d_start_board, 6 * (size_t)B);
    al(&S.board_pc, (size_t)kBoardConst * B); al(&S.cam_pc, (size_t)kCamConst * C); al(&S.vconst, (size_t)kVStride * V);
    al(&S.cconst[0], (size_t)kCStride * C); al(&S.cconst[1], (size_t)kCStride * C);
    al(&S.campart, 512 * (size_t)(P.n_chunks / 4)); al(&S.campart2, 512 * (size_t)C);
    al(&S.H_stage, 256 * (size_t)C + kScal + world);
    al(&S.s_b, 6 * (size_t)B); al(&S.s_c, s->n_pad); al(&S.fac, (size_t)kFac * B);
    al(&S.pairpart, 256 * (size_t)P.n_tiles); al(&S.T, 256 * (size_t)L.n_bids);
    al(&S.t_count, 1); al(&S.y_flag, 1); al(&S.fac_fail, 1);
    al(&S.yhat, s->n_pad);
    S.n_st_blocks = (B + 255) / 256;
    al(&S.bs_part, 2 * (size_t)((B + 15) / 16));
    al(&S.st_part, kStStride * (size_t)S.n_st_blocks);
    S.n_bs_blocks = L.n_bs_blocks;
    al(&S.ctrl, 1); al(&S.ctrl_snap, 1); al(&S.ctl_pub, 1);
    al(&S.stats_count, 64); al(&S.stats_flag, 64);
    HIP_TRY(he);
    for (int *flag : { S.t_count, S.y_flag, S.fac_fail }) HIP_TRY(hipMemset(flag, 0, sizeof(int)));
    HIP_TRY(hipMemset(S.stats_count, 0, 256)); HIP_TRY(hipMemset(S.stats_flag, 0, 256));
    HIP_TRY(hipMemset(S.ctl_pub, 0, sizeof(CtlPub)));
    HIP_TRY(hipMemset(S.T, 0, sizeof(double) * 256 * (size_t)L.n_bids));
    HIP_TRY(hipMemset(S.H_stage, 0, sizeof(double) * (256 * (size_t)C + kScal + world)));
    HIP_TRY(hipMemset(S.campart2, 0, sizeof(double) * 512 * (size_t)C));
    HIP_TRY(hipMemset(S.ctrl, 0, sizeof(Ctrl)));
    HIP_TRY(hipMemset(S.ctrl_snap, 0, sizeof(CtrlHead)));
    HIP_TRY(hipHostMalloc(reinterpret_cast<void **>(&s->h_ctrl), sizeof(Ctrl)));
    HIP_TRY(hipHostGetDevicePointer(reinterpret_cast<void **>(&s->d_h_ctrl), s->h_ctrl, 0));

    s->lds_eval = 4 * lds_eval_bytes;
    s->lds_eval32 = sizeof(double) * (size_t)eval_f32_lds_doubles(p->n_points, g4.ks);
    s->lds_eval4 = lds_eval4; s->eval4 = eval4; s->eval4r = eval4r;
    s->eval32 = f32_kernel(g4.ks, g4.passes > 1, false); s->eval32r = f32_kernel(g4.ks, g4.passes > 1, true);
    if (s->lds_eval32 > 64 * 1024)
        for (EvalKernel k : { s->eval32, s->eval32r }) HIP_TRY(hipFuncSetAttribute(reinterpret_cast<const void *>(k), hipFuncAttributeMaxDynamicSharedMemorySize, (int)s->lds_eval32));
    ColumnPlan cols;
    {
        std::string err;
        if (int rc = plan_columns(L, C, nullptr, cols, err)) return fail(rc, err);
    }
    if (C <= kDense4Cams) {
        int4 *map = nullptr;
        HIP_TRY(s->mem.alloc(&map, (size_t)(kSolveMapSlots / 4) * kSolveMapThreads));
        P.solve_map = map;
        const size_t NN = 64, TT = 4, NPD = 64;
        s->lds_dense4 = sizeof(double) * (NN * (NN + 2) + 2 * (NN / TT) * (TT * TT + 2) + 2 * NN + 3 * NPD);
        int per_cu = 0;
        HIP_TRY(hipOccupancyMaxActiveBlocksPerMultiprocessor(&per_cu, reinterpret_cast<const void *>(k_solve_reduced<4, 16, 64, true>), 256, std::max(s->lds_dense4, s->lds_bs)));
        s->dev.dense4_resident = per_cu * prop.multiProcessorCount;
    }
    if (C > kMaxCamLds) {
        const int NN = (cols.n_act + 15) & ~15;
        const size_t lds_max = solve_big_lds_bytes(NN, s->n_pad);
        HIP_TRY(s->mem.alloc(&S.Abig, (size_t)256 * (NN / 16 + 1) * (NN / 16 + 2) / 2));
        if (lds_max > 64 * 1024) HIP_TRY(hipFuncSetAttribute(reinterpret_cast<const void *>(k_solve_reduced_big), hipFuncAttributeMaxDynamicSharedMemorySize, (int)lds_max));
    }
    if (int rc = apply_columns(s, cols)) return rc;
    if (s->lds_eval > 160 * 1024) return fail(TSCM_E_UNSUPPORTED, "board has too many corners for the LDS board-point tile");
    HIP_TRY(hipDeviceSynchronize());
    *out = sp.release();
    return 0;
}

extern "C" int tscm_solver_create(const tscm_problem *p, int device, tscm_solver **out)
{
    return tscm_solver_create_sharded(p, device, 0, 1, out);
}

static CommKind comm_kind(const tscm_comm *c) { return !c ? kCommNone : c->world > 1 || c->group ? kCommShared : kCommOneRank; }

extern "C" int tscm_solver_debug_withhold_handoff(tscm_solver *s, int on)
{
    if (!s) return fail(TSCM_E_INVALID, "solver is NULL");
    s->withhold_next = on == 3 ? kWithholdStats : on ? kWithholdProducer : 0;
    s->no_rerun_next = on == 2;
    return 0;
}

extern "C" int tscm_solver_reruns(const tscm_solver *s)
{
    if (!s) return fail(TSCM_E_INVALID, "solver is NULL");
    return s->n_reruns;
}

extern "C" int tscm_solver_set_comm(tscm_solver *s, tscm_comm *comm)
{
    if (!s) return fail(TSCM_E_INVALID, "solver is NULL");
    if (comm && comm->device != s->device) return fail(TSCM_E_INVALID, "communicator and solver live on different devices");
    if (comm && (comm->world != s->world || comm->rank != s->rank))
        return fail(TSCM_E_INVALID, "communicator rank / world differ from the solver's shard (tscm_solver_create_sharded)");
    s->comm_reg = comm;
    s->comm = uses_comm(comm_kind(comm), 0) ? comm : nullptr;
    return 0;
}

extern "C" int tscm_solver_upload_params(tscm_solver *s, const double *cam_rt, const double *intr, const double *board_rt)
{
    if (!s || !intr || (!board_rt && s->L.B_total)) return fail(TSCM_E_INVALID, "NULL argument");
    HIP_TRY(hipSetDevice(s->device));
    std::vector<double> zero(6 * (size_t)s->C, 0.0);
    const double *c = (s->mono || !cam_rt) ? zero.data() : cam_rt;
    HIP_TRY(hipMemcpyAsync(s->d_init_cam, c, sizeof(double) * 6 * s->C, hipMemcpyHostToDevice, s->stream));
    HIP_TRY(hipMemcpyAsync(s->d_init_intr, intr, sizeof(double) * 9 * s->C, hipMemcpyHostToDevice, s->stream));
    std::vector<double> brd(6 * (size_t)s->B);
    for (int i = 0; i < s->B; ++i) std::memcpy(brd.data() + 6 * (size_t)i, board_rt + 6 * ((size_t)s->L.b0 + s->L.board_perm[i]), 6 * sizeof(double));
    if (s->B) HIP_TRY(hipMemcpyAsync(s->d_init_board, brd.data(), sizeof(double) * 6 * s->B, hipMemcpyHostToDevice, s->stream));
    HIP_TRY(hipStreamSynchronize(s->stream));
    s->have_init = true;
    return 0;
}

static int timed_pair(tscm_solver *s, int kind, hipEvent_t *e0, hipEvent_t *e1)
{
    *e0 = *e1 = nullptr;
    if (!(s->timing > 0 && (s->ev_count[kind]++ % (unsigned)s->timing) == 0)) return 0;
    if (s->ev_used == s->ev.size()) {
        hipEvent_t a, b;
        HIP_TRY(hipEventCreate(&a)); HIP_TRY(hipEventCreate(&b));
        s->ev.emplace_back(a, b);
        s->ev_kind.push_back(0);
    }
    s->ev_kind[s->ev_used] = kind;
    *e0 = s->ev[s->ev_used].first;
    *e1 = s->ev[s->ev_used].second;
    ++s->ev_used;
    return 0;
}

static int timed_begin(tscm_solver *s, int kind, hipStream_t stream, hipEvent_t *e1)
{
    hipEvent_t e0 = nullptr;
    if (int rc = timed_pair(s, kind, &e0, e1)) return rc;
    if (e0) HIP_TRY(hipEventRecord(e0, stream));
    return 0;
}

template <typename K, typename... A>
static void launch_eval_kernel(K kernel, dim3 grid, size_t lds, tscm_solver *s, hipEvent_t e0, hipEvent_t e1, int cand, A... extra)
{
    if (e0) hipExtLaunchKernelGGL(kernel, grid, dim3(256), (std::uint32_t)lds, s->stream, e0, e1, 0, s->P, s->S, cand, extra...);
    else hipLaunchKernelGGL(kernel, grid, dim3(256), lds, s->stream, s->P, s->S, cand, extra...);
}

static int launch_eval(tscm_solver *s, int cand)
{
    const DevProblem &P = s->P;
    if (P.n_chunks == 0) return 0;
    hipEvent_t e0 = nullptr, e1 = nullptr;
    if (int rc = timed_pair(s, 0, &e0, &e1)) return rc;
    const dim3 grid(P.n_chunks / 4);
    const bool robust = s->xp.robust;
    if (s->xp.gram == Gram::F32) launch_eval_kernel(robust ? s->eval32r : s->eval32, grid, s->lds_eval32, s, e0, e1, cand, s->loss);
    else if (s->xp.gram == Gram::G4) launch_eval_kernel(robust ? s->eval4r : s->eval4, grid, s->lds_eval4, s, e0, e1, cand, s->loss);
    else if (s->xp.gram == Gram::G16Pitch58) launch_eval_kernel(k_eval_gram<58>, grid, s->lds_eval, s, e0, e1, cand);
    else launch_eval_kernel(k_eval_gram<0>, grid, s->lds_eval, s, e0, e1, cand);
    return 0;
}

static int collect_timing(tscm_solver *s)
{
    for (size_t i = 0; i < s->ev_used; ++i) {
        float ms = 0.f;
        HIP_TRY(hipEventElapsedTime(&ms, s->ev[i].first, s->ev[i].second));
        const int k = s->ev_kind[i];
        s->t_ms[k] += ms; s->t_launches[k] += 1;
    }
    s->ev_used = 0;
    return 0;
}

extern "C" int tscm_solver_kernel_time(tscm_solver *s, int enable, int *launches, double *total_ms)
{
    if (!s) return fail(TSCM_E_INVALID, "solver is NULL");
    if (launches) *launches = s->t_launches[0];
    if (total_ms) *total_ms = s->t_ms[0];
    s->t_launches[0] = 0; s->t_ms[0] = 0.0;
    s->timing = enable < 0 ? 0 : enable;
    s->ev_count[0] = s->ev_count[1] = s->ev_count[2] = 0;
    return 0;
}

extern "C" int tscm_solver_exchange_time(tscm_solver *s, int *n_T, double *ms_T, int *n_H, double *ms_H)
{
    if (!s) return fail(TSCM_E_INVALID, "solver is NULL");
    if (n_T) *n_T = s->t_launches[1];
    if (ms_T) *ms_T = s->t_ms[1];
    if (n_H) *n_H = s->t_launches[2];
    if (ms_H) *ms_H = s->t_ms[2];
    s->t_launches[1] = s->t_launches[2] = 0; s->t_ms[1] = s->t_ms[2] = 0.0;
    return 0;
}

__global__ void k_xchg_sum(double *const *bufs, int world, size_t n)
{
    const size_t i = (size_t)blockIdx.x * blockDim.x + threadIdx.x;
    if (i >= n) return;
    double a = 0.0;
    for (int r = 0; r < world; ++r) a += bufs[r][i];
    for (int r = 0; r < world; ++r) bufs[r][i] = a;
}

constexpr long long kIpcTimeoutTicks = 1000000000;
__global__ __launch_bounds__(1024) void k_ipc_allreduce(double *buf, size_t n, IpcPeers peers, int rank, int world, size_t max_doubles, long long epoch, int *fault)
{
    if (__hip_atomic_load(fault, __ATOMIC_RELAXED, __HIP_MEMORY_SCOPE_AGENT)) return;
    const int parity = (int)(epoch & 1);
    const size_t slot = ((size_t)parity * world + rank) * max_doubles, flags = 2 * (size_t)world * max_doubles;
    for (int p = 0; p < world; ++p) {
        double *dst = peers.base[p] + slot;
        for (size_t i = threadIdx.x; i < n; i += 1024) __builtin_nontemporal_store(buf[i], dst + i);
    }
    __builtin_amdgcn_fence(__ATOMIC_RELEASE, "");
    __syncthreads();
    if ((int)threadIdx.x < world) {
        long long *f = reinterpret_cast<long long *>(peers.base[threadIdx.x] + flags) + (size_t)parity * world + rank;
        __hip_atomic_store(f, epoch, __ATOMIC_RELEASE, __HIP_MEMORY_SCOPE_SYSTEM);
    }
    __shared__ int s_late;
    if (threadIdx.x == 0) s_late = 0;
    __syncthreads();
    if ((int)threadIdx.x < world) {
        const long long *f = reinterpret_cast<const long long *>(peers.base[rank] + flags) + (size_t)parity * world + threadIdx.x;
        const long long t0 = wall_clock64();
        while (__hip_atomic_load(f, __ATOMIC_ACQUIRE, __HIP_MEMORY_SCOPE_SYSTEM) < epoch) {
            __builtin_amdgcn_s_sleep(8);
            if (wall_clock64() - t0 > kIpcTimeoutTicks) { s_late = 1; break; }
        }
    }
    __syncthreads();
    __builtin_amdgcn_fence(__ATOMIC_ACQUIRE, "");
    if (s_late) { if (threadIdx.x == 0) __hip_atomic_store(fault, 1, __ATOMIC_RELAXED, __HIP_MEMORY_SCOPE_SYSTEM); return; }
    const double *mine = peers.base[rank] + (size_t)parity * world * max_doubles;
    for (size_t i = threadIdx.x; i < n; i += 1024) {
        double a = 0.0;
        for (int r = 0; r < world; ++r) a += __builtin_nontemporal_load(mine + (size_t)r * max_doubles + i);
        buf[i] = a;
    }
}

static int comm_allreduce(tscm_comm *c, double *buf, size_t n, hipStream_t stream)
{
    if (c->ipc) {
        tscm_ipc *x = c->ipc;
        if (!x->connected) return fail(TSCM_E_INVALID, "tscm_comm_ipc_connect has not been called");
        if (x->dead) return fail(TSCM_E_PEER, "the IPC communicator is unusable after an earlier failure (a peer that did not arrive, or a failed solve)");
        IpcPeers peers{};
        for (int r = 0; r < x->world; ++r) peers.base[r] = static_cast<double *>(x->mapped[r]);
        for (size_t off = 0; off < n; off += x->max_doubles) {
            const size_t m = std::min(x->max_doubles, n - off);
            hipLaunchKernelGGL(k_ipc_allreduce, dim3(1), dim3(1024), 0, stream, buf + off, m, peers, x->rank, x->world, x->max_doubles, ++x->count, x->d_fault);
        }
        return 0;
    }
    NCCL_TRY(ncclAllReduce(buf, buf, n, ncclDouble, ncclSum, c->comm, stream));
    return 0;
}
static int comm_check(tscm_comm *c)
{
    if (!c || !c->ipc) return 0;
    int f = 0;
    HIP_TRY(hipMemcpy(&f, c->ipc->d_fault, sizeof(int), hipMemcpyDeviceToHost));
    if (f) { c->ipc->dead = true; return fail(TSCM_E_PEER, "IPC exchange: a peer rank did not arrive within the bound (failed or gone); the communicator is unusable from here on"); }
    return 0;
}

struct LmSeq {
    SeqState st;
    LaunchList todo;
    int at = 0;
};
struct LmRun {
    std::vector<tscm_solver *> m;
    std::vector<LmSeq> seq;
};

static int exchange(LmRun &run, bool t_buffer)
{
    tscm_solver *s0 = run.m[0];
    if (!s0->comm) return 0;
    const size_t n = t_buffer ? 256 * (size_t)s0->P.n_bids : 256 * (size_t)s0->P.C + kScal + s0->P.world;
    if (n == 0) return 0;
    hipEvent_t e1 = nullptr;
    if (s0->comm->group) {
        tscm_local_group *g = s0->comm->group;
        if (int rc = timed_begin(s0, t_buffer ? 1 : 2, g->stream, &e1)) return rc;
        hipLaunchKernelGGL(k_xchg_sum, dim3((unsigned)((n + 255) / 256)), dim3(256), 0, g->stream, g->d_ptrs + (t_buffer ? 0 : g->world), g->world, n);
        if (e1) HIP_TRY(hipEventRecord(e1, g->stream));
        return 0;
    }
    double *buf = t_buffer ? s0->S.T : s0->S.H_stage;
    if (int rc = timed_begin(s0, t_buffer ? 1 : 2, s0->stream, &e1)) return rc;
    if (int rc = comm_allreduce(s0->comm, buf, n, s0->stream)) return rc;
    if (e1) HIP_TRY(hipEventRecord(e1, s0->stream));
    return 0;
}

static int enqueue(tscm_solver *s, const Launch &l)
{
    const DevProblem &P = s->P;
    const DevState &S = s->S;
    hipStream_t st = s->stream;
    const dim3 grid(l.grid);
    auto schur = [&](auto kernel) { hipLaunchKernelGGL(kernel, grid, dim3(256), 0, st, P, S, l.chunk0, l.ctl, l.first_round, l.ce, l.target, l.n_chunks); };
    auto nd = [&](auto kernel) {
        const int v = l.nd;
        hipLaunchKernelGGL(kernel, grid, dim3(kNdThreads), std::max(s->lds_nd[v], l.n_bs ? s->lds_bs : (size_t)0), st, P, S, s->d_nd_map[v], s->d_nd_tab[v], s->d_nd_bs[v],
// ... 363 lines not shown
    sp->loss = loss;
    if (fixed) if (int rc = tscm_solver_set_fixed_intrinsics(sp.get(), fixed)) return rc;
    return tscm_solver_solve(sp.get(), opt, sum);
}

extern "C" int tscm_solve_multi(const tscm_problem *p, const tscm_options *opt, tscm_summary *sum)
{
    if (p && p->mono) return fail(TSCM_E_INVALID, "tscm_solve_multi called with a mono problem");
    return solve_once(p, opt, sum);
}

extern "C" int tscm_solve_mono(const tscm_problem *p, const tscm_options *opt, tscm_summary *sum)
{
    if (p && !p->mono) return fail(TSCM_E_INVALID, "tscm_solve_mono called with a multi-camera problem");
    return solve_once(p, opt, sum);
}

extern "C" int tscm_solve_robust(const tscm_problem *p, const tscm_options *opt, int kind, double scale, tscm_summary *sum)
{
    LossArg L;
    if (int rc = make_loss(kind, scale, L)) return rc;
    if (!p || !sum) return fail(TSCM_E_INVALID, "NULL argument");
    tscm_options o;
    if (int rc = read_options(opt, p->mono, o)) return rc;
    if (int rc = check_options(o, L.kind)) return rc;
    return solve_once(p, opt, sum, L);
}

extern "C" int tscm_solve_fixed(const tscm_problem *p, const tscm_options *opt, const unsigned short *fixed, int kind, double scale, tscm_summary *sum)
{
    LossArg L;
    if (int rc = make_loss(kind, scale, L)) return rc;
    if (!p || !sum) return fail(TSCM_E_INVALID, "NULL argument");
    if (int rc = check_fixed(fixed, p->n_cameras)) return rc;
    tscm_options o;
    if (int rc = read_options(opt, p->mono, o)) return rc;
    if (int rc = check_options(o, L.kind)) return rc;
    return solve_once(p, opt, sum, L, fixed);
}

static int eval_step(const tscm_problem *p, int device, const tscm_options *opt_in, const LossArg &loss, double *cam_rt, double *intr,
                     double *board_rt, int *valid, tscm_summary *summary, const unsigned short *fixed = nullptr)
{
    tscm_options opt;
    int rc = read_options(opt_in, p ? p->mono : 0, opt);
    if (rc) return rc;
    opt.max_num_iterations = 1;
    opt.function_tolerance = opt.gradient_tolerance = opt.parameter_tolerance = 0.0;
    if ((rc = check_options(opt, loss.kind))) return rc;
    if (!p || !intr || !valid || (!cam_rt && !p->mono) || (!board_rt && p->n_boards)) return fail(TSCM_E_INVALID, "NULL argument");
    SolverPtr sp;
    if ((rc = create_scoped(p, device, sp))) return rc;
    tscm_solver *s = sp.get();
    s->loss = loss;
    if (fixed && (rc = tscm_solver_set_fixed_intrinsics(s, fixed))) return rc;
    if ((rc = tscm_solver_upload_params(s, p->cam_rt, p->intr, p->board_rt))) return rc;
    tscm_summary sum;
    if ((rc = tscm_solver_solve_resident(s, &opt, &sum, 1))) return rc;
    if (cam_rt) { if (p->cam_rt) std::memcpy(cam_rt, p->cam_rt, sizeof(double) * 6 * p->n_cameras); else std::memset(cam_rt, 0, sizeof(double) * 6 * p->n_cameras); }
    if (p->n_boards) std::memcpy(board_rt, p->board_rt, sizeof(double) * 6 * p->n_boards);
    if ((rc = download_buffer(s, 1, cam_rt, intr, board_rt))) return rc;
    *valid = sum.num_iterations > 1 && sum.iterations[1].step_is_valid ? 1 : 0;
    if (summary) *summary = sum;
    return 0;
}

extern "C" int tscm_eval_step_ex(const tscm_problem *p, int device, const tscm_options *opt, double *cam_rt, double *intr,
                                 double *board_rt, int *valid, tscm_summary *summary)
{
    return eval_step(p, device, opt, LossArg{}, cam_rt, intr, board_rt, valid, summary);
}

extern "C" int tscm_eval_step_robust(const tscm_problem *p, int device, const tscm_options *opt, int kind, double scale, double *cam_rt,
                                     double *intr, double *board_rt, int *valid, tscm_summary *summary)
{
    LossArg L;
    if (int rc = make_loss(kind, scale, L)) return rc;
    return eval_step(p, device, opt, L, cam_rt, intr, board_rt, valid, summary);
}

extern "C" int tscm_eval_step_fixed(const tscm_problem *p, int device, const tscm_options *opt, const unsigned short *fixed, int kind, double scale,
                                    double *cam_rt, double *intr, double *board_rt, int *valid, tscm_summary *summary)
{
    LossArg L;
    if (int rc = make_loss(kind, scale, L)) return rc;
    if (!p) return fail(TSCM_E_INVALID, "NULL argument");
    if (int rc = check_fixed(fixed, p->n_cameras)) return rc;
    return eval_step(p, device, opt, L, cam_rt, intr, board_rt, valid, summary, fixed);
}

static int prepare_eval(tscm_solver *s, int with_floats = 0)
{
    int rc;
    if ((rc = tscm_solver_upload_params(s, s->h_cam_rt, s->h_intr, s->h_board_rt))) return rc;
    DevState &S = s->S;
    HIP_TRY(hipMemset(S.ctrl, 0, sizeof(Ctrl)));
    HIP_TRY(hipMemcpy(S.cam_rt[0], s->d_init_cam, sizeof(double) * 6 * s->C, hipMemcpyDeviceToDevice));
    HIP_TRY(hipMemcpy(S.intr[0], s->d_init_intr, sizeof(double) * 9 * s->C, hipMemcpyDeviceToDevice));
    if (s->B) HIP_TRY(hipMemcpy(S.board_rt[0], s->d_init_board, sizeof(double) * 6 * s->B, hipMemcpyDeviceToDevice));
    hipLaunchKernelGGL(k_pose_prep, dim3((s->P.B + s->P.C + 255) / 256), dim3(256), 0, s->stream, s->P, S, 0);
    hipLaunchKernelGGL(k_view_prep, dim3((s->P.V + s->P.C + kVPrepThreads - 1) / kVPrepThreads), dim3(kVPrepThreads), 0, s->stream, s->P, S, 0, with_floats);
    HIP_TRY(hipStreamSynchronize(s->stream));
    return 0;
}

extern "C" int tscm_eval_functor(const tscm_problem *p, int device, double *residuals, double *J_cam,
                                 double *J_board, double *J_intr, double *cost)
{
    SolverPtr sp;
    int rc = create_scoped(p, device, sp);
    if (rc) return rc;
    tscm_solver *s = sp.get();
    if ((rc = prepare_eval(s))) return rc;
    const size_t N = (size_t)s->N;
    std::vector<int> corner_view(N);
    for (int v = 0; v < s->V; ++v) for (int j = 0; j < s->L.view_count[v]; ++j) corner_view[s->L.view_obs[v] + j] = v;
    const int *d_cv = nullptr;
    double *d_res = nullptr, *d_Jc = nullptr, *d_Jb = nullptr, *d_Ji = nullptr;
    HIP_TRY(s->mem.upload(&d_cv, corner_view));
    HIP_TRY(s->mem.alloc(&d_res, 2 * N));
    if (J_cam) HIP_TRY(s->mem.alloc(&d_Jc, 12 * N));
    if (J_board) HIP_TRY(s->mem.alloc(&d_Jb, 12 * N));
    if (J_intr) HIP_TRY(s->mem.alloc(&d_Ji, 18 * N));
    if (N) hipLaunchKernelGGL(k_eval_functor, dim3((unsigned)((N + 255) / 256)), dim3(256), 0, s->stream, s->P, s->S, d_cv, d_res, d_Jc, d_Jb, d_Ji);
    HIP_TRY(hipStreamSynchronize(s->stream));
    HIP_TRY(hipGetLastError());
    std::vector<double> h_res(2 * N), h_Jc(d_Jc ? 12 * N : 0), h_Jb(d_Jb ? 12 * N : 0), h_Ji(d_Ji ? 18 * N : 0);
    if (N) HIP_TRY(hipMemcpy(h_res.data(), d_res, sizeof(double) * 2 * N, hipMemcpyDeviceToHost));
    if (d_Jc && N) HIP_TRY(hipMemcpy(h_Jc.data(), d_Jc, sizeof(double) * 12 * N, hipMemcpyDeviceToHost));
    if (d_Jb && N) HIP_TRY(hipMemcpy(h_Jb.data(), d_Jb, sizeof(double) * 12 * N, hipMemcpyDeviceToHost));
    if (d_Ji && N) HIP_TRY(hipMemcpy(h_Ji.data(), d_Ji, sizeof(double) * 18 * N, hipMemcpyDeviceToHost));
    std::vector<long> orig_row(p->n_views, 0);
    { long k = 0; for (int v = 0; v < p->n_views; ++v) { orig_row[v] = k; k += p->view_count[v]; } }
    double c = 0.0;
    for (int dv = 0; dv < s->V; ++dv) {
        const long dst = orig_row[s->L.dev2orig[dv]], src = s->L.view_obs[dv];
        const int cnt = s->L.view_count[dv];
        if (residuals) std::memcpy(residuals + 2 * dst, h_res.data() + 2 * src, sizeof(double) * 2 * cnt);
        if (J_cam) std::memcpy(J_cam + 12 * dst, h_Jc.data() + 12 * src, sizeof(double) * 12 * cnt);
        if (J_board) std::memcpy(J_board + 12 * dst, h_Jb.data() + 12 * src, sizeof(double) * 12 * cnt);
        if (J_intr) std::memcpy(J_intr + 18 * dst, h_Ji.data() + 18 * src, sizeof(double) * 18 * cnt);
    }
    for (size_t k = 0; k < N; ++k) c += 0.5 * (h_res[2 * k] * h_res[2 * k] + h_res[2 * k + 1] * h_res[2 * k + 1]);
    if (cost) *cost = c;
    return 0;
}

extern "C" int tscm_eval_normal_equations(const tscm_problem *p, int device, double *board_gram, double *board_grad,
                                          double *view_cross, double *cam_gram, double *cam_grad, double *cost)
{
    return tscm_eval_normal_equations_ex(p, device, nullptr, board_gram, board_grad, view_cross, cam_gram, cam_grad, cost);
}

static int eval_normal_equations(const tscm_problem *p, int device, const tscm_options *opt_in, const LossArg &loss, double *board_gram,
                                 double *board_grad, double *view_cross, double *cam_gram, double *cam_grad, double *cost)
{
    tscm_options opt;
    int rc = read_options(opt_in, p ? p->mono : 0, opt);
    if (rc) return rc;
    opt.max_num_iterations = 0;
    if ((rc = check_options(opt, loss.kind))) return rc;
    SolverPtr sp;
    if ((rc = create_scoped(p, device, sp))) return rc;
    tscm_solver *s = sp.get();
    s->loss = loss;
    s->xp = plan_exec(s->L, s->C, s->P.n_act, kCommNone, opt.exec_flags, opt.jacobian_fp32, loss.kind, s->P.rp, s->dev);
    if ((rc = prepare_eval(s, s->xp.f32() ? 1 : 0))) return rc;
    const DevProblem &P = s->P;
    DevState &S = s->S;
    if ((rc = launch_eval(s, 0))) return rc;
    hipLaunchKernelGGL(k_reduce_stats, dim3(P.C * kCamSl), dim3(256), 0, s->stream, P, S, 0, 0);
    hipLaunchKernelGGL(k_finalize_eval, dim3(P.C), dim3(256), 0, s->stream, P, S, 0);
    HIP_TRY(hipStreamSynchronize(s->stream));
    HIP_TRY(hipGetLastError());
    std::vector<double> rec((size_t)kRec * s->V), H(256 * (size_t)s->C), cc((size_t)kCStride * s->C);
    if (s->V) HIP_TRY(hipMemcpy(rec.data(), S.rec[0], sizeof(double) * rec.size(), hipMemcpyDeviceToHost));
    HIP_TRY(hipMemcpy(H.data(), S.H_stage, sizeof(double) * H.size(), hipMemcpyDeviceToHost));
    HIP_TRY(hipMemcpy(cc.data(), S.cconst[0], sizeof(double) * cc.size(), hipMemcpyDeviceToHost));
    if (board_gram) std::memset(board_gram, 0, sizeof(double) * 36 * (size_t)s->B);
    if (board_grad) std::memset(board_grad, 0, sizeof(double) * 6 * (size_t)s->B);
    if (view_cross) std::memset(view_cross, 0, sizeof(double) * 90 * (size_t)p->n_views);
    for (int dv = 0; dv < s->V; ++dv) {
        const double *rw = rec.data() + (size_t)kRecW * s->L.view_slot[dv];
        const double *re = rec.data() + (size_t)kRecW * s->V + (size_t)kRecE * s->L.view_slot[dv];
        const double *Rc = cc.data() + (size_t)kCStride * s->L.view_cam[dv];
        const int b = s->L.b0 + s->L.board_perm[s->L.view_board[dv]], ov = s->L.dev2orig[dv];
        for (int i = 0; i < 6; ++i) {
            if (board_gram)
                for (int j = 0; j < 6; ++j) {
                    const int hi = std::max(i, j), lo = std::min(i, j);
                    board_gram[36 * (size_t)b + 6 * i + j] += lo < 3 ? re[6 * lo + hi] : tb_tb(rw, Rc, hi - 3, lo - 3);
                }
            if (board_grad) board_grad[6 * (size_t)b + i] += rw[6 * kFR + i];
            if (view_cross) {
                for (int j = 0; j < 13; ++j) view_cross[90 * (size_t)ov + 15 * i + j] = rw[6 * j + i];
            }
        }
    }
    double c = 0.0;
    for (int m = 0; m < s->C; ++m) {
        const double *h = H.data() + 256 * (size_t)m;
        if (cam_gram) { std::memset(cam_gram + 225 * (size_t)m, 0, sizeof(double) * 225); for (int i = 0; i < 13; ++i) for (int j = 0; j < 13; ++j) cam_gram[225 * (size_t)m + 15 * i + j] = h[16 * i + j]; }
        if (cam_grad) { std::memset(cam_grad + 15 * (size_t)m, 0, sizeof(double) * 15); for (int i = 0; i < 13; ++i) cam_grad[15 * (size_t)m + i] = h[16 * i + kFR]; }
        c += 0.5 * h[16 * kFR + kFR];
    }
    if (cost) *cost = c;
    return 0;
}

extern "C" int tscm_eval_normal_equations_ex(const tscm_problem *p, int device, const tscm_options *opt, double *board_gram,
                                             double *board_grad, double *view_cross, double *cam_gram, double *cam_grad, double *cost)
{
    return eval_normal_equations(p, device, opt, LossArg{}, board_gram, board_grad, view_cross, cam_gram, cam_grad, cost);
}

extern "C" int tscm_eval_normal_equations_robust(const tscm_problem *p, int device, const tscm_options *opt, int kind, double scale,
                                                 double *board_gram, double *board_grad, double *view_cross, double *cam_gram,
                                                 double *cam_grad, double *cost)
{
    LossArg L;
    if (int rc = make_loss(kind, scale, L)) return rc;
    return eval_normal_equations(p, device, opt, L, board_gram, board_grad, view_cross, cam_gram, cam_grad, cost);
}


static int map_rows(void (*kernel)(const double *, const double *, int, double *), const char *who, const double *intr9, const double *in, int w_in,
                    int n, int device, double *out, int w_out)
{
    if (!intr9 || (n > 0 && (!in || !out)) || n < 0) return fail(TSCM_E_INVALID, "NULL argument");
    if (int rc = select_device(device, who)) return rc;
    if (n == 0) return 0;
    DeviceMem mem;
    const double *d_i = nullptr, *d_p = nullptr;
    double *d_o = nullptr;
    HIP_TRY(mem.upload(&d_i, intr9, 9));
    HIP_TRY(mem.upload(&d_p, in, w_in * (size_t)n));
    HIP_TRY(mem.alloc(&d_o, w_out * (size_t)n));
    hipLaunchKernelGGL(kernel, dim3((n + 255) / 256), dim3(256), 0, 0, d_i, d_p, n, d_o);
    HIP_TRY(hipMemcpy(out, d_o, w_out * (size_t)n * sizeof(double), hipMemcpyDeviceToHost));
    return 0;
}

extern "C" int tscm_project_points(const double *intr9, const double *points, int n, int device, double *pixels)
{
    return map_rows(k_project, "tscm_project_points", intr9, points, 3, n, device, pixels, 2);
}

extern "C" int tscm_unproject_pixels(const double *intr9, const double *pixels, int n, int device, double *rays)
{
    return map_rows(k_unproject, "tscm_unproject_pixels", intr9, pixels, 2, n, device, rays, 3);
}

extern "C" int tscm_reprojection_error(const tscm_problem *p, int device, double *per_camera_mean, double *global_mean, double *rmse)
{
    SolverPtr sp;
    int rc = create_scoped(p, device, sp);
    if (rc) return rc;
    tscm_solver *s = sp.get();
    if ((rc = tscm_solver_upload_params(s, s->h_cam_rt, s->h_intr, s->h_board_rt))) return rc;
    double *d_e = nullptr, *d_q = nullptr;
    HIP_TRY(s->mem.alloc(&d_e, (size_t)s->V));
    HIP_TRY(s->mem.alloc(&d_q, (size_t)s->V));
    if (s->V) hipLaunchKernelGGL(k_reproj_error, dim3(s->V), dim3(64), 0, s->stream, s->P, s->d_init_cam, s->d_init_intr, s->d_init_board, d_e, d_q);
    HIP_TRY(hipStreamSynchronize(s->stream));
    HIP_TRY(hipGetLastError());
    std::vector<double> e(s->V), q(s->V);
    if (s->V) { HIP_TRY(hipMemcpy(e.data(), d_e, sizeof(double) * s->V, hipMemcpyDeviceToHost)); HIP_TRY(hipMemcpy(q.data(), d_q, sizeof(double) * s->V, hipMemcpyDeviceToHost)); }
    std::vector<double> err(s->C, 0.0);
    std::vector<long> cnt(s->C, 0);
    double sq = 0.0;
    for (int v = 0; v < s->V; ++v) { err[s->L.view_cam[v]] += e[v]; cnt[s->L.view_cam[v]] += s->L.view_count[v]; sq += q[v]; }
    double tot = 0.0; long n = 0;
    for (int m = 0; m < s->C; ++m) { tot += err[m]; n += cnt[m]; if (per_camera_mean) per_camera_mean[m] = cnt[m] ? err[m] / (double)cnt[m] : 0.0; }
    if (global_mean) *global_mean = n ? tot / (double)n : 0.0;
    if (rmse) *rmse = n ? std::sqrt(sq / (double)n) : 0.0;
    return 0;
}

struct MbStream {
    hipStream_t s = nullptr;
    hipEvent_t e0 = nullptr, e1 = nullptr;
    ~MbStream() { if (e0) (void)hipEventDestroy(e0); if (e1) (void)hipEventDestroy(e1); if (s) (void)hipStreamDestroy(s); }
};

static double mb_pixel_rmse(const tscm_problem &p)
{
    ViewConst vc;
    mono_view_const(p.intr, vc);
    double sq = 0.0;
    long n = 0;
    for (int v = 0; v < p.n_views; ++v) {
        if (p.view_count[v] <= 0) continue;
        const double *rt = p.board_rt + 6 * (size_t)p.view_board[v];
        double bc[kBoardConst];
        board_constants(rt, bc);
        for (int q = 0; q < 3; ++q) { vc.r1[q] = bc[q]; vc.r2[q] = bc[3 + q]; vc.tb[q] = rt[3 + q]; }
        for (int kk = 0; kk < 3; ++kk) for (int q = 0; q < 6; ++q) vc.db[kk][q] = bc[6 + 6 * kk + q];
        for (int j = 0; j < p.view_count[v]; ++j) {
            double r[2], JE[2][kE], JF[2][kFA];
            const int o = p.view_offset[v] + j;
            corner_residual_jacobian(vc, p.board_xy[2 * j], p.board_xy[2 * j + 1], p.obs_u[o], p.obs_v[o], r, JE, JF);
            sq += r[0] * r[0] + r[1] * r[1];
        }
        n += p.view_count[v];
    }
    return n ? std::sqrt(sq / (double)n) : 0.0;
}

extern "C" int tscm_solve_mono_batch(const tscm_problem *problems, int n_problems, int device, const tscm_options *opt_in,
                                     const unsigned short *fixed, int loss_kind, double loss_scale, tscm_summary *summaries)
{
    const double t_call = wall();
    if (!summaries) return fail(TSCM_E_INVALID, "summaries is NULL");
    tscm_options opt;
    if (int rc = read_options(opt_in, 1, opt)) return rc;
    BatchPlan bp;
    {
        std::string err;
        if (int rc = plan_batch(problems, n_problems, opt, fixed, loss_kind, loss_scale, bp, err)) return fail(rc, err);
    }
    LossArg loss;
    if (int rc = make_loss(loss_kind, loss_scale, loss)) return rc;
    if (int rc = select_device(device, "tscm_solve_mono_batch")) return rc;
    for (int i = 0; i < n_problems; ++i) std::memset(&summaries[i], 0, sizeof(tscm_summary));

    const int K = bp.K, nc = (int)bp.chunk.size(), ns = (int)bp.slot_prob.size(), B = bp.B;
    double seconds_solve = 0.0;
    if (K > 0) {
        std::vector<double> ou((size_t)bp.N), ov((size_t)bp.N), intr((size_t)9 * K), board((size_t)6 * B, 0.0);
        for (int s = 0; s < ns; ++s) {
            const tscm_problem &p = problems[bp.dev_prob[bp.slot_prob[s]]];
            const int v = bp.slot_view[s];
            for (int j = 0; j < bp.slot_count[s]; ++j) { ou[bp.slot_obs[s] + j] = p.obs_u[p.view_offset[v] + j]; ov[bp.slot_obs[s] + j] = p.obs_v[p.view_offset[v] + j]; }
        }
        for (int k = 0; k < K; ++k) {
            const tscm_problem &p = problems[bp.dev_prob[k]];
            std::memcpy(&intr[9 * (size_t)k], p.intr, 9 * sizeof(double));
            if (p.n_boards) std::memcpy(&board[6 * (size_t)bp.board_ptr[k]], p.board_rt, 6 * sizeof(double) * p.n_boards);
        }
        std::vector<int4> chunk(nc);
        for (int c = 0; c < nc; ++c) chunk[c] = make_int4(bp.chunk[c].x, bp.chunk[c].y, bp.chunk[c].z, 0);

        DeviceMem A;
        MbDev D{};
        D.K = K; D.n_points = bp.n_points; D.n_chunks = nc; D.n_slots = ns; D.loss = loss;
        char *d_ctrl = nullptr;
        const size_t ctrl_bytes = sizeof(CtrlHead) * (size_t)K + sizeof(IterLog) * (size_t)kMaxLog * K;
        HIP_TRY(A.upload(&D.board_xy, problems[0].board_xy, 2 * (size_t)bp.n_points));
        HIP_TRY(A.upload(&D.obs_u, ou)); HIP_TRY(A.upload(&D.obs_v, ov));
        HIP_TRY(A.upload(&D.chunk, chunk));
        HIP_TRY(A.upload(&D.chunk_ptr, bp.chunk_ptr)); HIP_TRY(A.upload(&D.board_ptr, bp.board_ptr));
        HIP_TRY(A.upload(&D.slot_board, bp.slot_board)); HIP_TRY(A.upload(&D.slot_obs, bp.slot_obs));
        HIP_TRY(A.upload(&D.slot_count, bp.slot_count)); HIP_TRY(A.upload(&D.slot_active, bp.slot_active));
        HIP_TRY(A.upload(&D.mask, bp.mask));
        for (int b = 0; b < 2; ++b) {
            HIP_TRY(A.upload(&D.intr[b], intr)); HIP_TRY(A.upload(&D.board[b], board));
            HIP_TRY(A.alloc(&D.rec[b], (size_t)kMbRec * ns)); HIP_TRY(A.alloc(&D.part[b], (size_t)kMbPart * nc)); HIP_TRY(A.alloc(&D.tot[b], (size_t)kMbTot * K));
        }
        HIP_TRY(A.alloc(&D.schur, (size_t)kMbSp * nc)); HIP_TRY(A.alloc(&D.solvep, 4 * (size_t)nc)); HIP_TRY(A.alloc(&D.cam_mp, 4 * (size_t)K));
        HIP_TRY(A.alloc(&D.s_b, 6 * (size_t)ns)); HIP_TRY(A.alloc(&D.s_f, 7 * (size_t)K));
// ... 282 lines not shown
```

tscm_calib_amd/lib.py:

```python
from __future__ import annotations

import ctypes as C
import os
import subprocess

import numpy as np

_HERE = os.path.dirname(os.path.abspath(__file__))
CSRC = os.path.join(_HERE, "csrc")
LIB_PATH = os.path.join(CSRC, "libtscm_hip.so")
UNIQUE_ID_BYTES = 128
IPC_HANDLE_BYTES = 80
MAX_ITERATIONS = 255
EXEC_SEPARATE_T_REDUCE = 1
EXEC_KEEP_SINGLE_RANK_COMM = 2
EXEC_GRAM_16X16 = 4
EXEC_SEPARATE_BACKSUB = 8
EXEC_SEPARATE_CONTROL = 16
EXEC_DENSE_REDUCED_ORDER = 32
EXEC_GRAPH_REDUCED_ORDER = 64
EXEC_SEPARATE_STATS = 128
LOSS_NONE, LOSS_HUBER, LOSS_SOFT_L1, LOSS_CAUCHY = 0, 1, 2, 3
LOSS_KINDS = {None: LOSS_NONE, "none": LOSS_NONE, "huber": LOSS_HUBER, "soft_l1": LOSS_SOFT_L1, "cauchy": LOSS_CAUCHY}
PROJ_PERSPECTIVE, PROJ_LONGLAT, PROJ_CYLINDRICAL, PROJ_STEREOGRAPHIC, PROJ_EQUIRECT = 0, 1, 2, 3, 4
PROJ_KINDS = {"perspective": PROJ_PERSPECTIVE, "longlat": PROJ_LONGLAT, "cylindrical": PROJ_CYLINDRICAL,
              "stereographic": PROJ_STEREOGRAPHIC, "equirect": PROJ_EQUIRECT}
PANO_SEAM, PANO_FEATHER, PANO_MULTIBAND = 0, 1, 2
FILL_LOWEST, FILL_SECOND_LOWEST, FILL_MEDIAN = 0, 1, 2
PANO_MODES = {"seam": PANO_SEAM, "feather": PANO_FEATHER, "multiband": PANO_MULTIBAND}
INTRINSIC_NAMES = ("fx", "fy", "cx", "cy", "xi", "lambda", "alpha", "b", "c")
FIX = {name: 1 << k for k, name in enumerate(INTRINSIC_NAMES)}
FIX_INTRINSICS, FIX_ALL = 127, 511
MODEL_DS = FIX["lambda"]
MODEL_UCM = FIX["xi"] | FIX["lambda"]

E_NAMES = {0: "TSCM_OK", -1: "TSCM_E_INVALID", -2: "TSCM_E_NO_DEVICE", -3: "TSCM_E_HIP",
           -4: "TSCM_E_RCCL", -5: "TSCM_E_UNSUPPORTED", -6: "TSCM_E_NOMEM", -7: "TSCM_E_PEER"}
TERMINATION = {0: "CONVERGENCE", 1: "NO_CONVERGENCE", 2: "FAILURE"}


class TscmError(RuntimeError):
    def __init__(self, code: int, message: str):
        super().__init__(f"{E_NAMES.get(code, code)}: {message}")
        self.code = code


class CProblem(C.Structure):
    _fields_ = [
        ("n_cameras", C.c_int), ("n_boards", C.c_int), ("n_points", C.c_int), ("n_views", C.c_int),
        ("board_xy", C.c_void_p), ("view_camera", C.c_void_p), ("view_board", C.c_void_p),
        ("view_offset", C.c_void_p), ("view_count", C.c_void_p), ("obs_u", C.c_void_p), ("obs_v", C.c_void_p),
        ("cam_rt", C.c_void_p), ("intr", C.c_void_p), ("board_rt", C.c_void_p),
        ("cam_pose_constant", C.c_void_p), ("mono", C.c_int), ("board_pose_constant", C.c_void_p),
    ]


class COptions(C.Structure):
    _fields_ = [
        ("struct_size", C.c_size_t), ("max_num_iterations", C.c_int), ("function_tolerance", C.c_double), ("gradient_tolerance", C.c_double),
        ("parameter_tolerance", C.c_double), ("initial_trust_region_radius", C.c_double),
        ("max_trust_region_radius", C.c_double), ("min_trust_region_radius", C.c_double),
        ("min_relative_decrease", C.c_double), ("min_lm_diagonal", C.c_double), ("max_lm_diagonal", C.c_double),
        ("max_num_consecutive_invalid_steps", C.c_int), ("jacobi_scaling", C.c_int), ("check_every", C.c_int),
        ("jacobian_fp32", C.c_int), ("exec_flags", C.c_int),
    ]


class CIteration(C.Structure):
    _fields_ = [
        ("iteration", C.c_int), ("step_is_valid", C.c_int), ("step_is_successful", C.c_int),
        ("cost", C.c_double), ("cost_change", C.c_double), ("gradient_max_norm", C.c_double),
        ("gradient_norm", C.c_double), ("step_norm", C.c_double), ("relative_decrease", C.c_double),
        ("trust_region_radius", C.c_double),
    ]


class CSummary(C.Structure):
    _fields_ = [
        ("termination_type", C.c_int), ("num_iterations", C.c_int), ("num_successful_steps", C.c_int),
        ("num_unsuccessful_steps", C.c_int), ("initial_cost", C.c_double), ("final_cost", C.c_double),
        ("n_residual_blocks", C.c_int), ("lm_iterations", C.c_int),
        ("iterations", CIteration * (MAX_ITERATIONS + 1)), ("message", C.c_char * 128),
        ("seconds_solve", C.c_double), ("seconds_total", C.c_double), ("rmse", C.c_double),
    ]


class CRigInput(C.Structure):
    _fields_ = [
        ("n_cameras", C.c_int), ("n_boards", C.c_int), ("n_points", C.c_int),
        ("worlds", C.c_void_p), ("intr", C.c_void_p), ("has", C.c_void_p), ("Rt", C.c_void_p),
        ("pix_u", C.c_void_p), ("pix_v", C.c_void_p),
    ]


class CRigResult(C.Structure):
    _fields_ = [
        ("cam_R", C.c_void_p), ("cam_t", C.c_void_p), ("cam_rt", C.c_void_p),
        ("board_R", C.c_void_p), ("board_t", C.c_void_p), ("board_rt", C.c_void_p),
        ("board_initial", C.c_void_p), ("cam_choice", C.c_void_p), ("cam_min_error", C.c_void_p),
        ("seconds_hypotheses", C.c_double), ("seconds_total", C.c_double), ("n_projections", C.c_longlong),
    ]


class CMapDesc(C.Structure):
    _fields_ = [
        ("intr", C.c_double * 9), ("R", C.c_double * 9), ("fx", C.c_double), ("fy", C.c_double), ("cx", C.c_double),
        ("cy", C.c_double), ("offset_x", C.c_double), ("offset_y", C.c_double), ("width", C.c_int), ("height", C.c_int),
        ("out_stride", C.c_int), ("check_w2", C.c_int), ("out_offset", C.c_longlong), ("w2", C.c_double),
    ]


class CStereoParams(C.Structure):
    _fields_ = [("struct_size", C.c_int), ("min_disparity", C.c_int), ("num_disparities", C.c_int), ("p1", C.c_int), ("p2", C.c_int),
                ("paths", C.c_int), ("uniqueness_ratio", C.c_int), ("disp12_max_diff", C.c_int)]


class CStereoFilterParams(C.Structure):
    _fields_ = [("struct_size", C.c_int), ("min_disparity", C.c_int), ("speckle_window_size", C.c_int), ("speckle_range", C.c_int),
                ("median", C.c_int)]


class CStereoFillParams(C.Structure):
    _fields_ = [("struct_size", C.c_int), ("min_disparity", C.c_int), ("rule", C.c_int), ("paths", C.c_int), ("max_distance", C.c_int),
                ("min_directions", C.c_int), ("wrap_x", C.c_int)]


class CStereoRefineParams(C.Structure):
    _fields_ = [("struct_size", C.c_int), ("min_disparity", C.c_int), ("radius", C.c_int), ("iterations", C.c_int), ("fill_invalid", C.c_int),
                ("wrap_x", C.c_int)]


class CPanoramaParams(C.Structure):
    _fields_ = [("struct_size", C.c_int), ("mode", C.c_int), ("levels", C.c_int), ("wrap_x", C.c_int)]


class CSweepParams(C.Structure):
    _fields_ = [("struct_size", C.c_int), ("num_hypotheses", C.c_int), ("p1", C.c_int), ("p2", C.c_int), ("paths", C.c_int),
                ("uniqueness_ratio", C.c_int), ("wrap_x", C.c_int)]


class CSweepComposeParams(C.Structure):
    _fields_ = [("struct_size", C.c_int), ("mode", C.c_int), ("levels", C.c_int), ("wrap_x", C.c_int), ("fallback_index", C.c_int)]


class CSweepVisibilityParams(C.Structure):
    _fields_ = [("struct_size", C.c_int), ("cell_shift", C.c_int), ("tolerance", C.c_int), ("dilate", C.c_int), ("near_is_high", C.c_int)]


class CCornerSet(C.Structure):
    _fields_ = [
        ("n_cameras", C.c_int), ("n_boards", C.c_int), ("board_cols", C.c_int), ("board_rows", C.c_int), ("pitch", C.c_double),
        ("image_width", C.c_int), ("image_height", C.c_int), ("has", C.c_void_p), ("pix_u", C.c_void_p), ("pix_v", C.c_void_p),
    ]


EXPORTS = [
    "tscm_abi_version", "tscm_last_error", "tscm_device_count", "tscm_device_synchronize", "tscm_device_peak_fp64", "tscm_device_peak_fp64_ex", "tscm_device_peak_fp32_mfma", "tscm_default_options",
    "tscm_solver_create", "tscm_solver_set_comm", "tscm_solver_debug_withhold_handoff", "tscm_solver_reruns", "tscm_solver_solve", "tscm_solver_upload_params",
    "tscm_solver_solve_resident", "tscm_solver_download_params", "tscm_solver_destroy",
    "tscm_solver_kernel_time", "tscm_solver_exchange_time", "tscm_solve_multi", "tscm_solve_mono", "tscm_eval_functor",
    "tscm_eval_normal_equations", "tscm_eval_normal_equations_ex", "tscm_eval_step_ex", "tscm_project_points", "tscm_unproject_pixels",
    "tscm_reprojection_error", "tscm_comm_unique_id", "tscm_comm_create", "tscm_comm_destroy",
    "tscm_shard_frames", "tscm_solver_create_sharded", "tscm_comm_create_local", "tscm_comm_ipc_open", "tscm_comm_ipc_connect", "tscm_solver_solve_group",
    "tscm_solver_gather_boards", "tscm_comm_info", "tscm_rig_init", "tscm_rig_stage_errors", "tscm_yaml_format", "tscm_yaml_write", "tscm_yaml_parse",
    "tscm_yaml_read", "tscm_build_maps", "tscm_estimate_focal", "tscm_poses_from_r1r2t",
    "tscm_estimate_extrinsic", "tscm_estimate_focal_rows", "tscm_estimate_extrinsic_stages", "tscm_corners_write", "tscm_corners_read", "tscm_corners_free",
    "tscm_detect_corners", "tscm_detect_corners_batch", "tscm_corner_planes_batch", "tscm_corner_candidates_free", "tscm_chessboards_from_corners", "tscm_chessboards_free", "tscm_remap",
    "tscm_solver_set_loss", "tscm_solve_robust", "tscm_eval_normal_equations_robust", "tscm_eval_step_robust",
    "tscm_solver_set_fixed_intrinsics", "tscm_solve_fixed", "tscm_eval_step_fixed", "tscm_solve_mono_batch",
    "tscm_build_maps_ex", "tscm_rectify_points",
    "tscm_stereo_default_params", "tscm_stereo_match", "tscm_stereo_stages", "tscm_stereo_stage_times", "tscm_stereo_points",
    "tscm_stereo_filter_default_params", "tscm_stereo_filter", "tscm_stereo_filter_stages",
    "tscm_stereo_fill_default_params", "tscm_stereo_fill", "tscm_stereo_fill_stages",
    "tscm_stereo_refine_default_params", "tscm_stereo_refine_weights", "tscm_stereo_refine", "tscm_stereo_refine_stages",
    "tscm_panorama_default_params", "tscm_panorama_create", "tscm_panorama_compose", "tscm_panorama_stages", "tscm_panorama_overlap", "tscm_panorama_destroy",
    "tscm_build_sweep_maps",
    "tscm_sweep_default_params", "tscm_sweep_create", "tscm_sweep_depth", "tscm_sweep_stages", "tscm_sweep_stage_times", "tscm_sweep_points", "tscm_sweep_destroy",
    "tscm_sweep_compose_default_params", "tscm_sweep_compose", "tscm_sweep_compose_stages",
    "tscm_sweep_visibility_default_params", "tscm_sweep_visibility", "tscm_sweep_visibility_stages", "tscm_sweep_compose_visible", "tscm_sweep_compose_visible_stages",
]


def build(force: bool = False) -> str:
    import glob
    srcs = [f for pat in ("*.hip", "*.cpp", "*.h") for f in glob.glob(os.path.join(CSRC, pat))]
    srcs.append(os.path.join(_HERE, "..", "include", "tscm", "tscm.h"))
    stale = (not os.path.exists(LIB_PATH)) or any(os.path.getmtime(f) > os.path.getmtime(LIB_PATH) for f in srcs)
    if force or stale:
        subprocess.check_call(["make", "-C", CSRC] + (["-B"] if force else []))
    return LIB_PATH


_lib = None


def lib():
    global _lib
    if _lib is not None:
        return _lib
    if not os.path.exists(LIB_PATH):
        raise TscmError(-2, f"{LIB_PATH} is missing: run `python -c 'import __graft_entry__ as g; g.build()'` "
                            "(there is no CPU fallback)")
    L = C.CDLL(LIB_PATH)
    dp, ip, vp = C.POINTER(C.c_double), C.POINTER(C.c_int), C.c_void_p
    L.tscm_abi_version.restype = C.c_int
    L.tscm_last_error.restype = C.c_char_p
    L.tscm_device_count.restype = C.c_int
    L.tscm_device_synchronize.argtypes = [C.c_int]
    L.tscm_device_peak_fp64.argtypes = [C.c_int, dp, dp]
    L.tscm_device_peak_fp64_ex.argtypes = [C.c_int, dp]
    L.tscm_device_peak_fp32_mfma.argtypes = [C.c_int, dp]
    L.tscm_default_options.argtypes = [C.POINTER(COptions), C.c_int]
    L.tscm_default_options.restype = None
    L.tscm_solver_create.argtypes = [C.POINTER(CProblem), C.c_int, C.POINTER(vp)]
    L.tscm_solver_create_sharded.argtypes = [C.POINTER(CProblem), C.c_int, C.c_int, C.c_int, C.POINTER(vp)]
    L.tscm_comm_create_local.argtypes = [C.c_int, C.c_int, C.POINTER(vp)]
    L.tscm_comm_ipc_open.argtypes = [C.c_int, C.c_int, C.c_int, C.c_size_t, C.POINTER(vp), C.POINTER(C.c_ubyte)]
    L.tscm_comm_ipc_connect.argtypes = [vp, C.POINTER(C.c_ubyte)]
    L.tscm_solver_solve_group.argtypes = [C.POINTER(vp), C.c_int, C.POINTER(COptions), C.POINTER(CSummary), C.c_int]
    L.tscm_solver_gather_boards.argtypes = [vp, dp]
    L.tscm_comm_info.argtypes = [vp, ip, ip, ip]
    L.tscm_solver_set_comm.argtypes = [vp, vp]
    L.tscm_solver_debug_withhold_handoff.argtypes = [vp, C.c_int]
    L.tscm_solver_reruns.argtypes = [vp]
    L.tscm_solver_solve.argtypes = [vp, C.POINTER(COptions), C.POINTER(CSummary)]
    L.tscm_solver_upload_params.argtypes = [vp, dp, dp, dp]
    L.tscm_solver_solve_resident.argtypes = [vp, C.POINTER(COptions), C.POINTER(CSummary), C.c_int]
    L.tscm_solver_download_params.argtypes = [vp, dp, dp, dp]
    L.tscm_solver_destroy.argtypes = [vp]
    L.tscm_solver_destroy.restype = None
    L.tscm_solver_kernel_time.argtypes = [vp, C.c_int, ip, dp]
    L.tscm_solver_exchange_time.argtypes = [vp, ip, dp, ip, dp]
    L.tscm_solve_multi.argtypes = [C.POINTER(CProblem), C.POINTER(COptions), C.POINTER(CSummary)]
    L.tscm_solve_mono.argtypes = [C.POINTER(CProblem), C.POINTER(COptions), C.POINTER(CSummary)]
    L.tscm_eval_functor.argtypes = [C.POINTER(CProblem), C.c_int, dp, dp, dp, dp, dp]
    L.tscm_eval_normal_equations.argtypes = [C.POINTER(CProblem), C.c_int, dp, dp, dp, dp, dp, dp]
    L.tscm_eval_normal_equations_ex.argtypes = [C.POINTER(CProblem), C.c_int, C.POINTER(COptions), dp, dp, dp, dp, dp, dp]
    L.tscm_eval_step_ex.argtypes = [C.POINTER(CProblem), C.c_int, C.POINTER(COptions), dp, dp, dp, ip, C.POINTER(CSummary)]
    L.tscm_solver_set_loss.argtypes = [vp, C.c_int, C.c_double]
    L.tscm_solve_robust.argtypes = [C.POINTER(CProblem), C.POINTER(COptions), C.c_int, C.c_double, C.POINTER(CSummary)]
    L.tscm_eval_normal_equations_robust.argtypes = [C.POINTER(CProblem), C.c_int, C.POINTER(COptions), C.c_int, C.c_double, dp, dp, dp, dp, dp, dp]
    L.tscm_eval_step_robust.argtypes = [C.POINTER(CProblem), C.c_int, C.POINTER(COptions), C.c_int, C.c_double, dp, dp, dp, ip, C.POINTER(CSummary)]
    usp = C.POINTER(C.c_ushort)
    L.tscm_solver_set_fixed_intrinsics.argtypes = [vp, usp]
    L.tscm_solve_fixed.argtypes = [C.POINTER(CProblem), C.POINTER(COptions), usp, C.c_int, C.c_double, C.POINTER(CSummary)]
    L.tscm_solve_mono_batch.argtypes = [C.POINTER(CProblem), C.c_int, C.c_int, C.POINTER(COptions), usp, C.c_int, C.c_double,
                                        C.POINTER(CSummary)]
    L.tscm_eval_step_fixed.argtypes = [C.POINTER(CProblem), C.c_int, C.POINTER(COptions), usp, C.c_int, C.c_double, dp, dp, dp, ip, C.POINTER(CSummary)]
    L.tscm_project_points.argtypes = [dp, dp, C.c_int, C.c_int, dp]
    L.tscm_unproject_pixels.argtypes = [dp, dp, C.c_int, C.c_int, dp]
    L.tscm_reprojection_error.argtypes = [C.POINTER(CProblem), C.c_int, dp, dp, dp]
    L.tscm_comm_unique_id.argtypes = [C.POINTER(C.c_ubyte)]
    L.tscm_comm_create.argtypes = [C.POINTER(C.c_ubyte), C.c_int, C.c_int, C.c_int, C.POINTER(vp)]
    L.tscm_comm_destroy.argtypes = [vp]
    L.tscm_comm_destroy.restype = None
    L.tscm_shard_frames.argtypes = [C.POINTER(CProblem), C.c_int, ip]
    L.tscm_rig_init.argtypes = [C.POINTER(CRigInput), C.c_int, C.POINTER(CRigResult)]
    L.tscm_rig_stage_errors.argtypes = [C.POINTER(CRigInput), C.c_int, dp, dp, C.c_int, C.c_int, dp, dp, dp, ip]
    L.tscm_build_maps.argtypes = [C.POINTER(CMapDesc), C.c_int, C.c_int, C.c_int, C.POINTER(C.c_float), C.POINTER(C.c_float),
                                  C.c_size_t, dp]
    L.tscm_build_maps_ex.argtypes = [C.POINTER(CMapDesc), ip, C.c_int, C.c_int, C.c_int, C.POINTER(C.c_float), C.POINTER(C.c_float),
                                     C.c_size_t, dp]
    L.tscm_rectify_points.argtypes = [C.POINTER(CMapDesc), C.c_int, dp, C.c_int, C.c_int, dp, C.POINTER(C.c_ubyte)]
    ubp = C.POINTER(C.c_ubyte)
    L.tscm_stereo_default_params.argtypes = [C.POINTER(CStereoParams)]
    L.tscm_stereo_default_params.restype = None
    L.tscm_stereo_match.argtypes = [ubp, ubp, C.c_int, C.c_int, C.c_int, C.POINTER(CStereoParams), C.c_int, C.POINTER(C.c_short), C.c_int, dp]
    L.tscm_stereo_stages.argtypes = [ubp, ubp, C.c_int, C.c_int, C.c_int, C.POINTER(CStereoParams), C.c_int, C.POINTER(C.c_ulonglong),
                                     C.POINTER(C.c_ulonglong), ubp, usp]
    L.tscm_stereo_stage_times.argtypes = [dp]
    L.tscm_stereo_points.argtypes = [C.POINTER(C.c_short), C.c_int, C.c_int, C.c_int, C.c_int, C.POINTER(CMapDesc), C.c_int, C.c_double, C.c_int,
                                     dp, ubp]
    L.tscm_stereo_filter_default_params.argtypes = [C.POINTER(CStereoFilterParams)]
    L.tscm_stereo_filter_default_params.restype = None
    L.tscm_stereo_filter.argtypes = [C.POINTER(C.c_short), C.c_int, C.c_int, C.c_int, C.POINTER(CStereoFilterParams), C.c_int, C.POINTER(C.c_short), C.c_int, dp]
    L.tscm_stereo_filter_stages.argtypes = [C.POINTER(C.c_short), C.c_int, C.c_int, C.c_int, C.POINTER(CStereoFilterParams), C.c_int, C.POINTER(C.c_int),
                                            C.POINTER(C.c_int), C.POINTER(C.c_short)]
    L.tscm_stereo_fill_default_params.argtypes = [C.POINTER(CStereoFillParams)]
    L.tscm_stereo_fill_default_params.restype = None
    L.tscm_stereo_fill.argtypes = [C.POINTER(C.c_short), C.c_int, C.c_int, C.c_int, C.POINTER(CStereoFillParams), C.c_int, C.POINTER(C.c_short), C.c_int, ubp, dp]
    L.tscm_stereo_fill_stages.argtypes = [C.POINTER(C.c_short), C.c_int, C.c_int, C.c_int, C.POINTER(CStereoFillParams), C.c_int, C.POINTER(C.c_short),
                                          C.POINTER(C.c_short)]
    L.tscm_stereo_refine_default_params.argtypes = [C.POINTER(CStereoRefineParams)]
    L.tscm_stereo_refine_default_params.restype = None
    L.tscm_stereo_refine_weights.argtypes = [C.c_double, ubp]
    L.tscm_stereo_refine_weights.restype = None
    L.tscm_stereo_refine.argtypes = [C.POINTER(C.c_short), C.c_int, C.c_int, C.c_int, ubp, C.c_int, ubp, C.POINTER(CStereoRefineParams), C.c_int,
                                     C.POINTER(C.c_short), C.c_int, dp]
    L.tscm_stereo_refine_stages.argtypes = [C.POINTER(C.c_short), C.c_int, C.c_int, C.c_int, ubp, C.c_int, ubp, C.POINTER(CStereoRefineParams), C.c_int,
                                            C.POINTER(C.c_int), ubp, C.POINTER(C.c_short)]
    fp, shp, llp, vpp = C.POINTER(C.c_float), C.POINTER(C.c_short), C.POINTER(C.c_longlong), C.POINTER(vp)
    L.tscm_panorama_default_params.argtypes = [C.POINTER(CPanoramaParams)]
    L.tscm_panorama_default_params.restype = None
    L.tscm_panorama_create.argtypes = [C.c_int, C.c_int, C.c_int, C.c_int, vpp, fp, fp, C.c_int, C.c_int, C.POINTER(CPanoramaParams), C.c_int, vpp]
    L.tscm_panorama_compose.argtypes = [vp, vpp, C.c_int, usp, ubp, C.c_int, ubp, dp]
    L.tscm_panorama_stages.argtypes = [vp, vpp, C.c_int, usp, ubp, ubp, ubp, ubp, shp, shp]
    L.tscm_panorama_overlap.argtypes = [vp, vpp, C.c_int, llp, llp]
    L.tscm_panorama_destroy.argtypes = [vp]
    L.tscm_panorama_destroy.restype = None
    L.tscm_build_sweep_maps.argtypes = [C.POINTER(CMapDesc), ip, C.c_int, dp, dp, C.c_int, C.c_int, C.c_int, fp, fp, C.c_size_t, dp]
    L.tscm_sweep_default_params.argtypes = [C.POINTER(CSweepParams)]
    L.tscm_sweep_default_params.restype = None
    L.tscm_sweep_create.argtypes = [C.c_int, C.c_int, C.c_int, vpp, fp, fp, C.c_int, C.c_int, C.POINTER(CSweepParams), C.c_int, vpp]
    L.tscm_sweep_depth.argtypes = [vp, vpp, C.c_int, shp, C.c_int, dp]
    L.tscm_sweep_stages.argtypes = [vp, vpp, C.c_int, ubp, ubp, C.POINTER(C.c_ulonglong), ubp, usp]
    L.tscm_sweep_stage_times.argtypes = [dp]
    L.tscm_sweep_points.argtypes = [shp, C.c_int, C.c_int, C.c_int, C.POINTER(CMapDesc), C.c_int, dp, C.c_int, C.c_int, dp, ubp]
    L.tscm_sweep_compose_default_params.argtypes = [C.POINTER(CSweepComposeParams)]
    L.tscm_sweep_compose_default_params.restype = None
    L.tscm_sweep_compose.argtypes = [vp, vpp, C.c_int, C.c_int, shp, C.c_int, C.POINTER(CSweepComposeParams), usp, ubp, C.c_int, ubp, dp]
    L.tscm_sweep_compose_stages.argtypes = [vp, vpp, C.c_int, C.c_int, shp, C.c_int, C.POINTER(CSweepComposeParams), usp, ubp, ubp, ubp, ubp, ubp, shp, shp]
    vis = C.POINTER(CSweepVisibilityParams)
    L.tscm_sweep_visibility_default_params.argtypes = [vis]
    L.tscm_sweep_visibility_default_params.restype = None
    L.tscm_sweep_visibility.argtypes = [vp, shp, C.c_int, vis, ubp, ubp, dp]
    L.tscm_sweep_visibility_stages.argtypes = [vp, shp, C.c_int, vis, ubp, usp, ip, ubp, ubp, ubp]
    L.tscm_sweep_compose_visible.argtypes = [vp, vpp, C.c_int, C.c_int, shp, C.c_int, C.POINTER(CSweepComposeParams), vis, usp, ubp, C.c_int, ubp, dp]
    L.tscm_sweep_compose_visible_stages.argtypes = [vp, vpp, C.c_int, C.c_int, shp, C.c_int, C.POINTER(CSweepComposeParams), vis, usp, ubp, ubp, ubp, ubp, ubp, shp, shp,
                                                    ubp, ubp]
    L.tscm_sweep_destroy.argtypes = [vp]
    L.tscm_sweep_destroy.restype = None
    L.tscm_estimate_focal.argtypes = [dp, dp, ip, C.c_int, C.c_int, C.c_int, C.c_double, C.c_double, C.c_int, dp, ip]
    L.tscm_poses_from_r1r2t.argtypes = [dp, C.c_void_p, C.c_int, dp]
    L.tscm_estimate_extrinsic.argtypes = [dp, dp, dp, ip, C.c_int, dp, C.c_int, C.c_int, C.c_int, dp, ip]
    L.tscm_estimate_focal_rows.argtypes = [dp, dp, ip, C.c_int, C.c_int, C.c_int, C.c_double, C.c_double, C.c_int, dp]
    L.tscm_estimate_extrinsic_stages.argtypes = [dp, dp, dp, ip, C.c_int, dp, C.c_int, C.c_int, C.c_int, dp, ip, dp, dp, dp, dp, ip, ip]
    L.tscm_corners_write.argtypes = [C.c_char_p, C.POINTER(CCornerSet)]
    L.tscm_corners_read.argtypes = [C.c_char_p, C.POINTER(CCornerSet)]
    L.tscm_corners_free.argtypes = [C.POINTER(CCornerSet)]
    L.tscm_corners_free.restype = None
    L.tscm_yaml_format.argtypes = [C.c_int, dp, dp, dp, C.c_char_p, C.c_size_t, C.POINTER(C.c_size_t)]
    L.tscm_yaml_write.argtypes = [C.c_char_p, C.c_int, dp, dp, dp]
    L.tscm_yaml_parse.argtypes = [C.c_char_p, C.c_int, ip, dp, dp]
    L.tscm_yaml_read.argtypes = [C.c_char_p, C.c_int, ip, dp, dp]
    _lib = L
    return L


def loss_args(loss) -> tuple:
    if loss is None:
        return LOSS_NONE, 0.0
    if isinstance(loss, str):
        kind, scale = loss, 1.0
    else:
        kind, scale = loss
    if kind not in LOSS_KINDS:
        raise ValueError(f"unknown loss {kind!r}: one of 'huber', 'soft_l1', 'cauchy' or None")
    return LOSS_KINDS[kind], float(scale)


def fixed_masks(fixed, n_cameras: int) -> np.ndarray:
    C_ = int(n_cameras)
    if fixed is None:
        return np.zeros(C_, np.uint16)
    if isinstance(fixed, str):
        fixed = (fixed,)
    if isinstance(fixed, (int, np.integer)) and not isinstance(fixed, bool):
        words = np.full(C_, int(fixed), np.int64)
    elif isinstance(fixed, (tuple, list)) and all(isinstance(x, str) for x in fixed):
        w = 0
        for name in fixed:
            if name not in FIX:
                raise ValueError(f"unknown intrinsic {name!r}: one of {', '.join(INTRINSIC_NAMES)}")
            w |= FIX[name]
        words = np.full(C_, w, np.int64)
    else:
        a = np.asarray(fixed)
        if a.dtype == np.bool_:
            if a.shape != (C_, 9):
                raise ValueError(f"a bool mask has shape [{C_}, 9], not {list(a.shape)}")
            words = (a.astype(np.int64) << np.arange(9, dtype=np.int64)).sum(axis=1)
        elif np.issubdtype(a.dtype, np.integer):
            if a.shape != (C_,):
                raise ValueError(f"an integer mask has shape [{C_}], not {list(a.shape)}")
            words = a.astype(np.int64)
        else:
            raise ValueError(f"fixed must be None, names, a [C] int array or a [C, 9] bool array, not {a.dtype}")
    if np.any(words < 0) or np.any(words & ~FIX_ALL):
        raise ValueError("unknown bits in a fixed-intrinsics mask (bits 0-8: fx fy cx cy xi lambda alpha b c)")
    return words.astype(np.uint16)


def ushort_ptr(a: np.ndarray):
    assert a.dtype == np.uint16 and a.flags.c_contiguous
    return a.ctypes.data_as(C.POINTER(C.c_ushort))


def check(rc: int) -> None:
    if rc != 0:
        raise TscmError(rc, lib().tscm_last_error().decode(errors="replace"))


def dptr(a):
    return None if a is None else a.ctypes.data_as(C.POINTER(C.c_double))

# ... 54 lines not shown
```

Before: 8911.

## Skip constant camera-pose columns in gram4 eval for fixed-pose cameras

Chunks belonging to cameras whose pose is constant (for example the reference camera) are tagged in the chunk descriptor. The gram4 eval kernel can then take a reduced path that leaves out the camera-pose Jacobian columns and one of the three MFMA accumulations per step, storing a rearranged record layout. A solver-level normal-equations entry point is added so the solved-path output can be checked against the full path. The gain depends on how many chunks have constant pose, and the new layout risks mismatched record indexing.

```diff
diff --git a/include/tscm/tscm.h b/include/tscm/tscm.h
--- a/include/tscm/tscm.h
+++ b/include/tscm/tscm.h
@@ -155,6 +155,9 @@
                                       double *cam_gram, double *cam_grad, double *cost);
 int tscm_eval_step_robust(const tscm_problem *problem, int device, const tscm_options *opt, int kind, double scale,
                           double *cam_rt, double *intr, double *board_rt, int *valid, tscm_summary *summary);
+int tscm_solver_eval_normal_equations(tscm_solver *s, const tscm_options *opt, int as_solved,
+                                      double *board_gram, double *board_grad, double *view_cross,
+                                      double *cam_gram, double *cam_grad, double *cost);
 
 enum {
     TSCM_FIX_FX = 1, TSCM_FIX_FY = 2, TSCM_FIX_CX = 4, TSCM_FIX_CY = 8, TSCM_FIX_XI = 16, TSCM_FIX_LAMBDA = 32,
diff --git a/tscm_calib_amd/api.py b/tscm_calib_amd/api.py
--- a/tscm_calib_amd/api.py
+++ b/tscm_calib_amd/api.py
@@ -290,7 +290,8 @@
     return cost.value, res
 
 
-def normal_equations(problem: Problem, device: int = 0, *, jacobian_fp32: int = 0, exec_flags: int = 0, loss=None) -> dict:
+def normal_equations(problem: Problem, device: int = 0, *, jacobian_fp32: int = 0, exec_flags: int = 0, loss=None,
+                     as_solved: bool = False) -> dict:
     assert _is_normalised(problem)
     Cn, B, V = problem.n_cameras, problem.n_boards, problem.n_views
     out = dict(board_gram=np.zeros((B, 6, 6)), board_grad=np.zeros((B, 6)), view_cross=np.zeros((V, 6, 15)),
@@ -300,7 +301,12 @@
     o = _l.default_options(problem.mono, jacobian_fp32=jacobian_fp32, exec_flags=exec_flags)
     outs = (_l.dptr(out["board_gram"]), _l.dptr(out["board_grad"]), _l.dptr(out["view_cross"]),
             _l.dptr(out["cam_gram"]), _l.dptr(out["cam_grad"]), C.byref(cost))
-    if loss is None:
+    if as_solved:
+        with Solver(problem, device) as s:
+            if loss is not None:
+                s.set_loss(*((loss,) if isinstance(loss, str) else loss))
+            _l.check(_l.lib().tscm_solver_eval_normal_equations(s._h, C.byref(o), 1, *outs))
+    elif loss is None:
         _l.check(_l.lib().tscm_eval_normal_equations_ex(C.byref(cp), device, C.byref(o), *outs))
     else:
         k, a = _l.loss_args(loss)
diff --git a/tscm_calib_amd/csrc/tscm_dev.h b/tscm_calib_amd/csrc/tscm_dev.h
--- a/tscm_calib_amd/csrc/tscm_dev.h
+++ b/tscm_calib_amd/csrc/tscm_dev.h
@@ -12,6 +12,8 @@
 constexpr int kTcols = 15;
 constexpr int kTcWb = 0, kTcWc = 4, kTcF = 8, kTcOne = 9, kTcXi = 10, kTcLam = 12, kTcAl = 13, kTcR = 14;
 __host__ __device__ constexpr int tc_tc(int j) { return 3 + 4 * j; }
+constexpr int kChunkConstPose = 1 << 30, kChunkCamMask = kChunkConstPose - 1;
+constexpr int kEvalCand = 1, kEvalSkipConst = 2;
 constexpr int kVConst = 27;
 constexpr int kCConst = 48;
 constexpr int kCStride = 72;
diff --git a/tscm_calib_amd/csrc/tscm_eval_f32.h b/tscm_calib_amd/csrc/tscm_eval_f32.h
--- a/tscm_calib_amd/csrc/tscm_eval_f32.h
+++ b/tscm_calib_amd/csrc/tscm_eval_f32.h
@@ -31,7 +31,7 @@
     const int lane = threadIdx.x & 63;
     const int chunk = blockIdx.x * 4 + wave;
     const v4i cd = *(const v4i __attribute__((address_space(4))) *)(const void *)(P.chunk_desc + chunk);
-    const int cam = cd[0], vb = cd[1], ve = cd[2];
+    const int cam = cd[0] & kChunkCamMask, vb = cd[1], ve = cd[2];
     const int n2 = 2 * P.n_points;
     const double bx0 = P.board_xy[min(lane, n2 - 1)], bx1 = P.board_xy[min(lane + 64, n2 - 1)];
     typedef const float __attribute__((address_space(4))) *fptr4;
diff --git a/tscm_calib_amd/csrc/tscm_eval_gram4.h b/tscm_calib_amd/csrc/tscm_eval_gram4.h
--- a/tscm_calib_amd/csrc/tscm_eval_gram4.h
+++ b/tscm_calib_amd/csrc/tscm_eval_gram4.h
@@ -17,8 +17,13 @@
 __device__ __forceinline__ constexpr int g4_cgroup(int b, int q) { return q == 0 ? b : q == 1 ? ((b + 1) & 3) : (b == 0 ? 2 : b == 1 ? 3 : 1); }
 __device__ __forceinline__ int g4_elem(int c, int k) { return 4 * c + (k ^ ((c >> 3) << 1)); }
 
-template <int KS, int D, bool ACC, int T = 0>
-__device__ __forceinline__ void gram4_steps(unsigned aN, unsigned aR, unsigned aB, double (&n)[KS], double (&r)[KS], double (&b)[KS], double (&acc)[3])
+constexpr int kG4FCp = 15;
+template <bool CP> __device__ __forceinline__ constexpr bool g4_live(int c) { return CP ? (c < 8 || c >= 12) : c < kTcols; }
+template <bool CP> __device__ __forceinline__ constexpr int g4_old_col_of(int c) { return CP && c == kG4FCp ? kTcF : g4_old_col(c); }
+__device__ __forceinline__ constexpr int g4_wcol_cp(int i) { return i == 0 ? 8 : i == 1 ? 10 : i == 2 ? 11 : 6; }
+
+template <int KS, int D, bool ACC, int NQ, int T = 0>
+__device__ __forceinline__ void gram4_steps(unsigned aN, unsigned aR, unsigned aB, double (&n)[KS], double (&r)[KS], double (&b)[KS], double (&acc)[NQ])
 {
     if constexpr (T < KS) {
         if constexpr (T + D < KS) {
@@ -28,15 +33,17 @@
         }
         constexpr int newer = 3 * (KS - 1 - T < D ? KS - 1 - T : D);
         lgkm_wait<newer + 2>(n[T]);
-        if constexpr (T == 0 && !ACC) acc[0] = __builtin_amdgcn_mfma_f64_4x4x4f64(n[T], n[T], 0.0, 0, 0, 0);
-        else acc[0] = __builtin_amdgcn_mfma_f64_4x4x4f64(n[T], n[T], acc[0], 0, 0, 0);
+        if constexpr (NQ == 3) {
+            if constexpr (T == 0 && !ACC) acc[0] = __builtin_amdgcn_mfma_f64_4x4x4f64(n[T], n[T], 0.0, 0, 0, 0);
+            else acc[0] = __builtin_amdgcn_mfma_f64_4x4x4f64(n[T], n[T], acc[0], 0, 0, 0);
+        }
         lgkm_wait<newer + 1>(r[T]);
-        if constexpr (T == 0 && !ACC) acc[1] = __builtin_amdgcn_mfma_f64_4x4x4f64(n[T], r[T], 0.0, 0, 0, 0);
-        else acc[1] = __builtin_amdgcn_mfma_f64_4x4x4f64(n[T], r[T], acc[1], 0, 0, 0);
+        if constexpr (T == 0 && !ACC) acc[NQ - 2] = __builtin_amdgcn_mfma_f64_4x4x4f64(n[T], r[T], 0.0, 0, 0, 0);
+        else acc[NQ - 2] = __builtin_amdgcn_mfma_f64_4x4x4f64(n[T], r[T], acc[NQ - 2], 0, 0, 0);
         lgkm_wait<newer>(b[T]);
-        if constexpr (T == 0 && !ACC) acc[2] = __builtin_amdgcn_mfma_f64_4x4x4f64(n[T], b[T], 0.0, 0, 0, 0);
-        else acc[2] = __builtin_amdgcn_mfma_f64_4x4x4f64(n[T], b[T], acc[2], 0, 0, 0);
-        gram4_steps<KS, D, ACC, T + 1>(aN, aR, aB, n, r, b, acc);
+        if constexpr (T == 0 && !ACC) acc[NQ - 1] = __builtin_amdgcn_mfma_f64_4x4x4f64(n[T], b[T], 0.0, 0, 0, 0);
+        else acc[NQ - 1] = __builtin_amdgcn_mfma_f64_4x4x4f64(n[T], b[T], acc[NQ - 1], 0, 0, 0);
+        gram4_steps<KS, D, ACC, NQ, T + 1>(aN, aR, aB, n, r, b, acc);
     }
 }
 template <int KS, int D, int T = 0>
@@ -49,13 +56,13 @@
         gram4_prime<KS, D, T + 1>(aN, aR, aB, n, r, b);
     }
 }
-template <int KS, bool ACC>
-__device__ __forceinline__ void gram4_full(unsigned aN, unsigned aR, unsigned aB, double (&acc)[3])
+template <int KS, bool ACC, int NQ>
+__device__ __forceinline__ void gram4_full(unsigned aN, unsigned aR, unsigned aB, double (&acc)[NQ])
 {
     constexpr int D = KS < 2 ? KS : 2;
     double n[KS], r[KS], b[KS];
     gram4_prime<KS, D>(aN, aR, aB, n, r, b);
-    gram4_steps<KS, D, ACC>(aN, aR, aB, n, r, b, acc);
+    gram4_steps<KS, D, ACC, NQ>(aN, aR, aB, n, r, b, acc);
 }
 
 __device__ __forceinline__ double quad_tb(double x, double c0, double c1, double c2)
@@ -72,13 +79,13 @@
     return __hiloint2double(hi, lo);
 }
 
-template <int KS, bool MULTI, bool ROBUST = false>
-__global__ __launch_bounds__(256, 4) void k_eval_gram4(DevProblem P, DevState S, int cand, LossArg L)
+template <int KS, bool MULTI, bool ROBUST, bool CP>
+__device__ __forceinline__ void eval_gram4_wave(const DevProblem &P, const DevState &S, const int cand, const LossArg &L, const v4i cd,
+                                                const int ctrl_done, const int ctrl_cur, const d2 my_xy)
 {
     static_assert(KS >= 1 && KS <= kG4MaxKS, "a pass holds at most 56 rows");
     constexpr int kTile = g4_tile_doubles(KS);
-    KTL(0);
-    const int ctrl_done = S.ctrl->done, ctrl_cur = S.ctrl->cur;
+    constexpr int NQ = CP ? 2 : 3;
 #ifdef TSCM_WAVE_TIMELINE
     const long long tl_t0 = wall_clock64();
     const int tl_iter = S.ctrl->iteration;
@@ -98,13 +105,13 @@
     double *Fl = lds;
     double *bxy = lds + kTile;
     const int lane = threadIdx.x & 63;
+#ifdef TSCM_WAVE_TIMELINE
     const int chunk = blockIdx.x * 4 + wave;
-    const v4i cd = *(const v4i __attribute__((address_space(4))) *)(const void *)(P.chunk_desc + chunk);
-    const int cam = cd[0], vb = cd[1], ve = cd[2];
-    const d2 my_xy = *reinterpret_cast<const d2 *>(P.board_xy + 2 * min(lane, P.n_points - 1));
+#endif
+    const int cam = cd[0] & kChunkCamMask, vb = cd[1], ve = cd[2];
     double *const cc_buf[2] = { S.cconst[0], S.cconst[1] };
     double *const rec_buf[2] = { S.rec[0], S.rec[1] };
-    double camU[3] = { 0.0, 0.0, 0.0 }, camV[3] = { 0.0, 0.0, 0.0 };
+    double camU[NQ] = {}, camV[NQ] = {};
     for (int i = lane; i < KS * kG4Stride; i += 64) Fl[i] = 0.0;
     int prev_nv = 0;
     double pf_u = 0.0, pf_v = 0.0;
@@ -127,9 +134,9 @@
     double *fu_lo = Fl + (lane >> 2) * kG4Stride + (lane & 3), *fu_hi = Fl + (lane >> 2) * kG4Stride + ((lane & 3) ^ 2);
     const int li = lane >> 4, c16 = lane & 15, lb = c16 >> 2, lj = c16 & 3;
     const unsigned lds0 = lds_addr(Fl);
-    const unsigned aN = lds0 + 8u * (unsigned)g4_elem(c16, li);
-    const unsigned aR = lds0 + 8u * (unsigned)g4_elem((c16 + 4) & 15, li);
-    const unsigned aB = lds0 + 8u * (unsigned)g4_elem(4 * g4_cgroup(lb, 2) + lj, li);
+    const unsigned aN = lds0 + 8u * (unsigned)g4_elem(CP && lb == 2 ? 12 + lj : c16, li);
+    const unsigned aR = lds0 + 8u * (unsigned)g4_elem(CP ? (lb == 2 ? lj : c16) : (c16 + 4) & 15, li);
+    const unsigned aB = lds0 + 8u * (unsigned)g4_elem(CP ? 4 + lj : 4 * g4_cgroup(lb, 2) + lj, li);
     const double rc0 = lj == 0 ? ccs[0] : lj == 1 ? ccs[1] : ccs[2];
     const double rc1 = lj == 0 ? ccs[3] : lj == 1 ? ccs[4] : ccs[5];
     const double rc2 = lj == 0 ? ccs[6] : lj == 1 ? ccs[7] : ccs[8];
@@ -144,6 +151,13 @@
         if (b == 1 && j < 3) o1w = W(f1, 3 + j);
         if (b == 0 && i < 3) o2 = W(f1j, i);
         if (b == 0 && i == 3 && j < 3) { o2 = W(kFR, 3 + j); o7b = 8u * (unsigned)(3 + j); }
+        if constexpr (CP) {
+            const int f3c = g4_wcol_cp(i);
+            if (b == 2 && j < 3) o2 = W(f3c, j);
+            if (b == 3 && j < 3) o2 = W(f3c, 3 + j);
+            if (b == 2 && j < 3 && (i == 0 || i == 3)) o4 = W(f3c + 1, j);
+            if (b == 3 && j < 3 && (i == 0 || i == 3)) o4 = W(f3c + 1, 3 + j);
+        } else {
         if (b == 3 && j < 3 && i < 3) o2 = W(f3, j);
         if (b == 0 && i < 3) o4 = W(f2j, i);
         if (b == 2 && j < 3) o4 = W(f2, 3 + j);
@@ -151,6 +165,13 @@
         if (b == 3 && i == 0 && j < 3) { o5 = W(9, j); o6 = W(9, 3 + j); }
         if (b == 0 && j == 3 && i < 3) o6 = W(7, i);
         if (b == 2 && i == 3 && j < 3) o6 = W(7, 3 + j);
+        }
+    }
+    {
+        const unsigned baseE = 8u * (unsigned)kRecW * (unsigned)P.V, baseG = 8u * (unsigned)(kRecW + kRecE) * (unsigned)P.V;
+        if (o1e != BAD) { o1e += baseE; o3e += baseE; }
+        if (o7a != BAD) o7a += baseG;
+        if (o7b != BAD) o7b += baseG;
     }
     if (lane < P.n_points) *reinterpret_cast<d2 *>(bxy + 2 * lane) = my_xy;
     if constexpr (MULTI) {
@@ -188,7 +209,7 @@
 #endif
         const cptr4 vcs = (cptr4)(S.vconst + (size_t)kVStride * view);
         auto VC = [&](int k) { return vcs[k]; };
-        double accU[3] = { 0.0, 0.0, 0.0 }, accV[3] = { 0.0, 0.0, 0.0 };
+        double accU[NQ] = {}, accV[NQ] = {};
         int pbv = 0;
         do {
         const int pb = MULTI ? pbv : 0;
@@ -201,21 +222,21 @@
         if (valid) {
             const double x = bxy[2 * (pb + lane)], y = bxy[2 * (pb + lane) + 1];
             constexpr int tcol[15] = { kG4Wb, kG4Wb + 1, kG4Wb + 2, kG4Tc, kG4Tc + 1, kG4Tc + 2, kG4Wc, kG4Wc + 1, kG4Wc + 2,
-                                       kG4F, kG4One, kG4Xi, kG4Lam, kG4Al, kG4R };
+                                       CP ? kG4FCp : kG4F, kG4One, kG4Xi, kG4Lam, kG4Al, kG4R };
             if constexpr (ROBUST) {
                 double ru, rv, rho, w;
                 corner_residual(x, y, pf_u, pf_v, VC, CC, ru, rv);
                 robust_rho(L, ru * ru + rv * rv, rho, w);
                 rho_sum += rho;
-                corner_geometry(x, y, pf_u, pf_v, VC, CC, [&](int gc, double u, double v) { PUT(tcol[gc], w * u, w * v); });
+                corner_geometry<!CP>(x, y, pf_u, pf_v, VC, CC, [&](int gc, double u, double v) { PUT(tcol[gc], w * u, w * v); });
             } else {
-                corner_geometry(x, y, pf_u, pf_v, VC, CC, [&](int gc, double u, double v) { PUT(tcol[gc], u, v); });
+                corner_geometry<!CP>(x, y, pf_u, pf_v, VC, CC, [&](int gc, double u, double v) { PUT(tcol[gc], u, v); });
             }
         }
         if (nv < prev_nv) {
             if (!valid && lane < prev_nv) {
 #pragma unroll
-                for (int c = 0; c < kTcols; ++c) (c < 8 ? fu_lo : fu_hi)[4 * c] = 0.0;
+                for (int c = 0; c < 16; ++c) if (g4_live<CP>(c)) (c < 8 ? fu_lo : fu_hi)[4 * c] = 0.0;
             }
         }
         {
@@ -233,16 +254,16 @@
 #ifdef TSCM_WAVE_TIMELINE
         if (tl_nv == 1) tl_w[1] = wall_clock64();
 #endif
-        gram4_full<KS, MULTI>(aN, aR, aB, accU);
+        gram4_full<KS, MULTI, NQ>(aN, aR, aB, accU);
         wave_lds_fence();
         TL_STAMP(ts2);
         if (valid) {
 #pragma unroll
-            for (int c = 0; c < kTcols; ++c) (c < 8 ? fu_lo : fu_hi)[4 * c] = fv[c];
+            for (int c = 0; c < 16; ++c) if (g4_live<CP>(c)) (c < 8 ? fu_lo : fu_hi)[4 * c] = fv[c];
         }
         wave_lds_fence();
         TL_STAMP(ts3);
-        gram4_full<KS, MULTI>(aN, aR, aB, accV);
+        gram4_full<KS, MULTI, NQ>(aN, aR, aB, accV);
         TL_STAMP(ts4);
         TL_ADD(0, ts0, ts1); TL_ADD(1, ts1, ts2); TL_ADD(2, ts2, ts3); TL_ADD(3, ts3, ts4);
         pbv += per;
@@ -250,14 +271,26 @@
         TL_STAMP(ts4e);
         asm volatile("" :: "v"(warm));
 #pragma unroll
-        for (int q = 0; q < 3; ++q) { camU[q] += accU[q]; camV[q] += accV[q]; }
+        for (int q = 0; q < NQ; ++q) { camU[q] += accU[q]; camV[q] += accV[q]; }
         {
             const unsigned slot = (unsigned)__builtin_amdgcn_readlane(m_slot, view - vbase);
-            const unsigned offW = 8u * (unsigned)kRecW * slot, offE = 8u * ((unsigned)kRecW * (unsigned)P.V + (unsigned)kRecE * slot);
-            const double T0 = accU[0] + accV[0], T1 = accU[1] + accV[1], T2 = accU[2] + accV[2];
+            const unsigned offW = 8u * (unsigned)kRecW * slot, offE = 8u * (unsigned)kRecE * slot, offG = 8u * (unsigned)kRecG * slot;
+            if constexpr (CP) {
+            const double T0 = accU[0] + accV[0], T1 = accU[1] + accV[1];
+            const double X = lane_pick<0xF, 0x2>(T1, T0);
+            const double tbX = quad_tb(X, rc0, rc1, rc2), tbU1 = quad_tb(accU[1], rc0, rc1, rc2);
+            buf_store_f64(r_rec, o1e, offE, T0);
+            buf_store_f64(r_rec, o7a, offG, T0);
+            const double Z = lane_pick<0xF, 0x9>(T0, tbX), ZU = lane_pick<0xF, 0x8>(accU[0], tbU1);
+            buf_store_f64(r_rec, o4, offW, Z - ZU);
+            buf_store_f64(r_rec, o1w, offW, lane_pick<0xF, 0x2>(T0, tbX));
+            buf_store_f64(r_rec, o2, offW, lane_pick<0x9, 0xC>(lane_pick<0x7, 0x1>(Z, T1), ZU));
+            buf_store_f64(r_rec, o3e, offE, tbX);
+            buf_store_f64(r_rec, o7b, offG, tbX);
+            } else {
+            const double T0 = accU[0] + accV[0], T1 = accU[1] + accV[1], T2 = accU[NQ - 1] + accV[NQ - 1];
             const double X = lane_pick<0xF, 0x1>(lane_pick<0xF, 0x2>(T2, T0), T1);
-            const double tbX = quad_tb(X, rc0, rc1, rc2), tbU2 = quad_tb(accU[2], rc0, rc1, rc2);
-            const unsigned offG = 8u * ((unsigned)(kRecW + kRecE) * (unsigned)P.V + (unsigned)kRecG * slot);
+            const double tbX = quad_tb(X, rc0, rc1, rc2), tbU2 = quad_tb(accU[NQ - 1], rc0, rc1, rc2);
             buf_store_f64(r_rec, o1e, offE, T0);
             buf_store_f64(r_rec, o7a, offG, T0);
             buf_store_f64(r_rec, o1w, offW, lane_pick<0xF, 0x2>(T0, tbX));
@@ -265,9 +298,10 @@
             buf_store_f64(r_rec, o2, offW, lane_pick<0x1, 0x8>(lane_pick<0x8, 0xF>(T1, tbX), accU[1]));
             buf_store_f64(r_rec, o3e, offE, tbX);
             buf_store_f64(r_rec, o7b, offG, tbX);
-            const double a4 = lane_pick<0xF, 0xE>(T2, tbX), u4 = lane_pick<0xF, 0x1>(tbU2, accU[2]);
+            const double a4 = lane_pick<0xF, 0xE>(T2, tbX), u4 = lane_pick<0xF, 0x1>(tbU2, accU[NQ - 1]);
             buf_store_f64(r_rec, o4, offW, (int)o6 >= 0 ? u4 : a4);
             buf_store_f64(r_rec, o6, offW, a4 - u4);
+            }
         }
 #ifdef TSCM_WAVE_TIMELINE
         { TL_STAMP(ts5); TL_ADD(4, ts4e, ts5); }
@@ -291,9 +325,14 @@
         if (lane == 16 * kG4R + kG4R) { camU[0] = rho_sum; camV[0] = 0.0; }
     }
     wave_lds_fence();
-#pragma unroll
-    for (int q = 0; q < 3; ++q) {
-        const int r = g4_old_col(4 * lb + li), c = g4_old_col(4 * g4_cgroup(lb, q) + lj);
+    if constexpr (CP) {
+        for (int i = lane; i < 512; i += 64) lds[i] = 0.0;
+        wave_lds_fence();
+    }
+#pragma unroll
+    for (int q = 0; q < NQ; ++q) {
+        const int rg = CP && lb == 2 ? 3 : lb, cg = !CP ? g4_cgroup(lb, q) : q == 1 ? 1 : lb == 2 ? 0 : lb;
+        const int r = g4_old_col_of<CP>(4 * rg + li), c = g4_old_col_of<CP>(4 * cg + lj);
         lds[16 * r + c] = camU[q]; lds[16 * c + r] = camU[q];
         lds[256 + 16 * r + c] = camV[q]; lds[256 + 16 * c + r] = camV[q];
     }
@@ -309,3 +348,18 @@
     if (lane == 0 && tl_iter == 5 && cand && chunk < kTimelineWaves) g_tlv[(size_t)(4 + kTlViews) * chunk + 2] = wall_clock64();
 #endif
 }
+
+template <int KS, bool MULTI, bool ROBUST = false>
+__global__ __launch_bounds__(256, 4) void k_eval_gram4(DevProblem P, DevState S, int cand, LossArg L)
+{
+    KTL(0);
+    const int ctrl_done = S.ctrl->done, ctrl_cur = S.ctrl->cur;
+    const int chunk = blockIdx.x * 4 + __builtin_amdgcn_readfirstlane(threadIdx.x >> 6);
+    const v4i cd = *(const v4i __attribute__((address_space(4))) *)(const void *)(P.chunk_desc + chunk);
+    const d2 my_xy = *reinterpret_cast<const d2 *>(P.board_xy + 2 * min((int)(threadIdx.x & 63), P.n_points - 1));
+#ifndef TSCM_G4_FULL_PATH
+    if ((cand & kEvalSkipConst) && (cd[0] & kChunkConstPose)) eval_gram4_wave<KS, MULTI, ROBUST, true>(P, S, cand & kEvalCand, L, cd, ctrl_done, ctrl_cur, my_xy);
+    else
+#endif
+        eval_gram4_wave<KS, MULTI, ROBUST, false>(P, S, cand & kEvalCand, L, cd, ctrl_done, ctrl_cur, my_xy);
+}
diff --git a/tscm_calib_amd/csrc/tscm_exec_plan.h b/tscm_calib_amd/csrc/tscm_exec_plan.h
--- a/tscm_calib_amd/csrc/tscm_exec_plan.h
+++ b/tscm_calib_amd/csrc/tscm_exec_plan.h
@@ -49,6 +49,7 @@
     bool comm = false;
     Gram gram = Gram::G4;
     bool robust = false;
+    bool skip_const_pose = false;
     EvalTail tail = EvalTail::ReduceControl;
     bool ctl_in_schur = false;
     bool stats_ride = false;
@@ -83,12 +84,13 @@
 }
 
 inline ExecPlan plan_exec(const Layout &L, int C, int n_act, int comm_kind, int exec_flags, int jacobian_fp32, int loss_kind, int rp,
-                          const ExecDevice &dev)
+                          const ExecDevice &dev, bool inspect = false)
 {
     ExecPlan p;
     p.comm = uses_comm(comm_kind, exec_flags);
     p.gram = plan_gram(exec_flags, jacobian_fp32, rp);
     p.robust = loss_kind != TSCM_LOSS_NONE;
+    p.skip_const_pose = !inspect && p.gram == Gram::G4;
     const int n_variants = (L.nv_chunks[1] ? 1 : 0) + (L.nv_chunks[2] ? 1 : 0) + (L.nv_chunks[3] ? 1 : 0);
     const bool small = C <= kMaxCamLds;
     p.ctl_in_schur = (p.comm || small) && L.slow_boards.empty() && L.pc_begin.empty() && n_variants == 1 &&
diff --git a/tscm_calib_amd/csrc/tscm_geometry.h b/tscm_calib_amd/csrc/tscm_geometry.h
--- a/tscm_calib_amd/csrc/tscm_geometry.h
+++ b/tscm_calib_amd/csrc/tscm_geometry.h
@@ -58,7 +58,7 @@
 
 enum GCol { gcWb0 = 0, gcWb1, gcWb2, gcTc0, gcTc1, gcTc2, gcWc0, gcWc1, gcWc2, gcF, gcOne, gcXi, gcLam, gcAl, gcR };
 
-template <typename FV, typename FC, typename FP>
+template <bool WC = true, typename FV, typename FC, typename FP>
 __device__ __forceinline__ void corner_geometry(double x, double y, double ou, double ov, FV VC, FC CC, FP PUT)
 {
     const double X = fma(x, VC(0), fma(y, VC(3), VC(6)));
@@ -93,7 +93,7 @@
         const double h2 = x * VC(11 + 6 * kk) + y * VC(14 + 6 * kk);
         PUT(gcWb0 + kk, n00 * h0 + n01 * h1 + n02 * h2, n10 * h0 + n11 * h1 + n12 * h2);
     }
-    {
+    if constexpr (WC) {
         double Q0 = X - CC(9), Q1 = Y - CC(10), Q2 = Z - CC(11);
         if (CC(24) != 0.0) {
             const double w0 = CC(21), w1 = CC(22), w2 = CC(23);
diff --git a/tscm_calib_amd/csrc/tscm_solver.hip b/tscm_calib_amd/csrc/tscm_solver.hip
--- a/tscm_calib_amd/csrc/tscm_solver.hip
+++ b/tscm_calib_amd/csrc/tscm_solver.hip
@@ -107,6 +107,7 @@
     Layout L;
     int C = 0, B = 0, V = 0, N = 0, n_points = 0, n_pad = 0;
     int rank = 0, world = 1;
+    int n_views = 0;
     hipStream_t own_stream = nullptr;
     bool mono = false;
     double *h_cam_rt = nullptr, *h_intr = nullptr, *h_board_rt = nullptr;
@@ -308,7 +309,7 @@
     tscm_solver *s = sp.get();
     s->device = device;
     s->rank = rank; s->world = world;
-    s->C = p->n_cameras; s->n_points = p->n_points; s->mono = p->mono != 0;
+    s->C = p->n_cameras; s->n_points = p->n_points; s->mono = p->mono != 0; s->n_views = p->n_views;
     s->n_pad = 16 * s->C;
     s->h_cam_rt = p->cam_rt; s->h_intr = p->intr; s->h_board_rt = p->board_rt;
     HIP_TRY(hipStreamCreateWithFlags(&s->stream, hipStreamNonBlocking));
@@ -365,7 +366,9 @@
         for (size_t i = 0; i < h.size(); ++i) d[i] = make_int4(h[i].x, h[i].y, h[i].z, h[i].w);
         return d;
     };
-    const std::vector<int4> chunk_desc = int4s(L.chunk_desc), bc_desc = int4s(L.bc_desc);
+    std::vector<int4> chunk_desc = int4s(L.chunk_desc);
+    const std::vector<int4> bc_desc = int4s(L.bc_desc);
+    for (int4 &d : chunk_desc) if (L.cam_const[d.x]) d.x |= kChunkConstPose;
     const std::vector<short> bid_lut(L.bid_of.begin(), L.bid_of.end());
     DevProblem &P = s->P;
     DevState &S = s->S;
@@ -415,6 +418,7 @@
     al(&S.stats_count, 64); al(&S.stats_flag, 64);
     HIP_TRY(he);
     for (int *flag : { S.t_count, S.y_flag, S.fac_fail }) HIP_TRY(hipMemset(flag, 0, sizeof(int)));
+    for (int k = 0; k < 2; ++k) if (V) HIP_TRY(hipMemset(S.rec[k], 0, sizeof(double) * (size_t)kRec * V));
     HIP_TRY(hipMemset(S.stats_count, 0, 256)); HIP_TRY(hipMemset(S.stats_flag, 0, 256));
     HIP_TRY(hipMemset(S.ctl_pub, 0, sizeof(CtlPub)));
     HIP_TRY(hipMemset(S.T, 0, sizeof(double) * 256 * (size_t)L.n_bids));
@@ -548,7 +552,8 @@
     const dim3 grid(P.n_chunks / 4);
     const bool robust = s->xp.robust;
     if (s->xp.gram == Gram::F32) launch_eval_kernel(robust ? s->eval32r : s->eval32, grid, s->lds_eval32, s, e0, e1, cand, s->loss);
-    else if (s->xp.gram == Gram::G4) launch_eval_kernel(robust ? s->eval4r : s->eval4, grid, s->lds_eval4, s, e0, e1, cand, s->loss);
+    else if (s->xp.gram == Gram::G4)
+        launch_eval_kernel(robust ? s->eval4r : s->eval4, grid, s->lds_eval4, s, e0, e1, cand | (s->xp.skip_const_pose ? kEvalSkipConst : 0), s->loss);
     else if (s->xp.gram == Gram::G16Pitch58) launch_eval_kernel(k_eval_gram<58>, grid, s->lds_eval, s, e0, e1, cand);
     else launch_eval_kernel(k_eval_gram<0>, grid, s->lds_eval, s, e0, e1, cand);
     return 0;
@@ -1218,19 +1223,11 @@
     return tscm_eval_normal_equations_ex(p, device, nullptr, board_gram, board_grad, view_cross, cam_gram, cam_grad, cost);
 }
 
-static int eval_normal_equations(const tscm_problem *p, int device, const tscm_options *opt_in, const LossArg &loss, double *board_gram,
-                                 double *board_grad, double *view_cross, double *cam_gram, double *cam_grad, double *cost)
-{
-    tscm_options opt;
-    int rc = read_options(opt_in, p ? p->mono : 0, opt);
-    if (rc) return rc;
-    opt.max_num_iterations = 0;
-    if ((rc = check_options(opt, loss.kind))) return rc;
-    SolverPtr sp;
-    if ((rc = create_scoped(p, device, sp))) return rc;
-    tscm_solver *s = sp.get();
-    s->loss = loss;
-    s->xp = plan_exec(s->L, s->C, s->P.n_act, kCommNone, opt.exec_flags, opt.jacobian_fp32, loss.kind, s->P.rp, s->dev);
+static int solver_normal_equations(tscm_solver *s, const tscm_options &opt, bool as_solved, double *board_gram, double *board_grad,
+                                   double *view_cross, double *cam_gram, double *cam_grad, double *cost)
+{
+    int rc;
+    s->xp = plan_exec(s->L, s->C, s->P.n_act, kCommNone, opt.exec_flags, opt.jacobian_fp32, s->loss.kind, s->P.rp, s->dev, !as_solved);
     if ((rc = prepare_eval(s, s->xp.f32() ? 1 : 0))) return rc;
     const DevProblem &P = s->P;
     DevState &S = s->S;
@@ -1245,7 +1242,7 @@
     HIP_TRY(hipMemcpy(cc.data(), S.cconst[0], sizeof(double) * cc.size(), hipMemcpyDeviceToHost));
     if (board_gram) std::memset(board_gram, 0, sizeof(double) * 36 * (size_t)s->B);
     if (board_grad) std::memset(board_grad, 0, sizeof(double) * 6 * (size_t)s->B);
-    if (view_cross) std::memset(view_cross, 0, sizeof(double) * 90 * (size_t)p->n_views);
+    if (view_cross) std::memset(view_cross, 0, sizeof(double) * 90 * (size_t)s->n_views);
     for (int dv = 0; dv < s->V; ++dv) {
         const double *rw = rec.data() + (size_t)kRecW * s->L.view_slot[dv];
         const double *re = rec.data() + (size_t)kRecW * s->V + (size_t)kRecE * s->L.view_slot[dv];
@@ -1272,6 +1269,36 @@
     }
     if (cost) *cost = c;
     return 0;
+}
+
+static int eval_normal_equations(const tscm_problem *p, int device, const tscm_options *opt_in, const LossArg &loss, double *board_gram,
+                                 double *board_grad, double *view_cross, double *cam_gram, double *cam_grad, double *cost)
+{
+    tscm_options opt;
+    int rc = read_options(opt_in, p ? p->mono : 0, opt);
+    if (rc) return rc;
+    opt.max_num_iterations = 0;
+    if ((rc = check_options(opt, loss.kind))) return rc;
+    SolverPtr sp;
+    if ((rc = create_scoped(p, device, sp))) return rc;
+    sp->loss = loss;
+    return solver_normal_equations(sp.get(), opt, false, board_gram, board_grad, view_cross, cam_gram, cam_grad, cost);
+}
+
+extern "C" int tscm_solver_eval_normal_equations(tscm_solver *s, const tscm_options *opt_in, int as_solved, double *board_gram,
+                                                 double *board_grad, double *view_cross, double *cam_gram, double *cam_grad, double *cost)
+{
+    if (!s) return fail(TSCM_E_INVALID, "solver is NULL");
+    if (s->world != 1) return fail(TSCM_E_UNSUPPORTED, "tscm_solver_eval_normal_equations: a sharded solver holds a part of the problem");
+    tscm_options opt;
+    int rc = read_options(opt_in, s->mono ? 1 : 0, opt);
+    if (rc) return rc;
+    opt.max_num_iterations = 0;
+    if ((rc = check_options(opt, s->loss.kind))) return rc;
+    HIP_TRY(hipSetDevice(s->device));
+    rc = solver_normal_equations(s, opt, as_solved != 0, board_gram, board_grad, view_cross, cam_gram, cam_grad, cost);
+    s->xp = ExecPlan{};
+    return rc;
 }
 
 extern "C" int tscm_eval_normal_equations_ex(const tscm_problem *p, int device, const tscm_options *opt, double *board_gram,
diff --git a/tscm_calib_amd/lib.py b/tscm_calib_amd/lib.py
--- a/tscm_calib_amd/lib.py
+++ b/tscm_calib_amd/lib.py
@@ -167,6 +167,7 @@
     "tscm_estimate_extrinsic", "tscm_estimate_focal_rows", "tscm_estimate_extrinsic_stages", "tscm_corners_write", "tscm_corners_read", "tscm_corners_free",
     "tscm_detect_corners", "tscm_detect_corners_batch", "tscm_corner_planes_batch", "tscm_corner_candidates_free", "tscm_chessboards_from_corners", "tscm_chessboards_free", "tscm_remap",
     "tscm_solver_set_loss", "tscm_solve_robust", "tscm_eval_normal_equations_robust", "tscm_eval_step_robust",
+    "tscm_solver_eval_normal_equations",
     "tscm_solver_set_fixed_intrinsics", "tscm_solve_fixed", "tscm_eval_step_fixed", "tscm_solve_mono_batch",
     "tscm_build_maps_ex", "tscm_rectify_points",
     "tscm_stereo_default_params", "tscm_stereo_match", "tscm_stereo_stages", "tscm_stereo_stage_times", "tscm_stereo_points",
@@ -241,6 +242,7 @@
     L.tscm_solve_robust.argtypes = [C.POINTER(CProblem), C.POINTER(COptions), C.c_int, C.c_double, C.POINTER(CSummary)]
     L.tscm_eval_normal_equations_robust.argtypes = [C.POINTER(CProblem), C.c_int, C.POINTER(COptions), C.c_int, C.c_double, dp, dp, dp, dp, dp, dp]
     L.tscm_eval_step_robust.argtypes = [C.POINTER(CProblem), C.c_int, C.POINTER(COptions), C.c_int, C.c_double, dp, dp, dp, ip, C.POINTER(CSummary)]
+    L.tscm_solver_eval_normal_equations.argtypes = [vp, C.POINTER(COptions), C.c_int, dp, dp, dp, dp, dp, dp]
     usp = C.POINTER(C.c_ushort)
     L.tscm_solver_set_fixed_intrinsics.argtypes = [vp, usp]
     L.tscm_solve_fixed.argtypes = [C.POINTER(CProblem), C.POINTER(COptions), usp, C.c_int, C.c_double, C.POINTER(CSummary)]
```

Measured after the change: 9075 (median of 6 runs). 1.8% higher.
